# facebookresearch/PartDistillation

Measured on AMD Instinct MI355X. Metric: images/sec training step, R50 Mask2Former 1024² bs=2/GPU, 1/2/4/8 MI355X, higher is better.
Workload: dtype bf16

## Files before the change

### include/pd_gemm.h

```cpp
#ifndef PD_GEMM_H
#define PD_GEMM_H

#include <stdint.h>

#ifdef __cplusplus
extern "C" {
#endif

int pd_gemm_tn_f32(const float *A, const float *B, const float *bias, float *C, int M, int N, int K, int lda, int ldb,
                   int ldc, int relu, void *stream);

int pd_gemm_tn_f32x3(const float *A, const float *B, const float *bias, float *C, int M, int N, int K, int lda, int ldb,
                     int ldc, int relu, void *stream);

int pd_gemm_wgrad_f32(const float *dY, const float *X, float *dW, float *dB, int M, int N, int K, int ldy, int ldx,
                      int ldw, void *stream);

int pd_gemm_wgrad_acc_f32(const float *dY, const float *X, float *dW, float *dB, int M, int N, int K, int ldy, int ldx,
                          int ldw, void *stream);

int64_t pd_gemm_tn_f32x3_relu_bits_words(int M, int N);
int pd_split3_bf16(const float *W, int N, int K, int ldw, int transpose, void *planes, void *stream);
int pd_gemm_tn_f32x3_pre(const float *A, const void *Bplanes, const float *bias, float *C, uint32_t *bits, float *colsum, int M, int N, int K,
                         int lda, int ldc, int mode, void *stream);
// ... 16 lines not shown
} PdGemmWgradDesc;
int64_t pd_gemm_wgrad_f32x3_grouped_table_bytes(int max_count);
int64_t pd_gemm_wgrad_f32x3_grouped_ws_floats(const PdGemmWgradDesc *descs, int count);
int pd_gemm_wgrad_f32x3_grouped(const PdGemmWgradDesc *descs, int count, void *table_host_pinned, void *table_device, float *workspace,
                                int64_t workspace_floats, void *stream);

int pd_conv3x3_wgrad_nhwc_f32x3(const float *dY, const float *X, float *dWk, float *dB, float *workspace, int64_t workspace_floats, int B, int H,
                                int W, int Ci, int Co, void *stream);

int pd_conv3x3_nhwc_f32x3(const float *X, const float *Wk, const float *bias, float *Y, int B, int H, int W, int Ci, int Co,
                          void *stream);

int64_t pd_gemm_wgrad_f16x2_ws_floats(int N, int K);
int pd_gemm_wgrad_f16x2_takes_wide_tiles(int N, int K);
int64_t pd_gemm_wgrad_f16x2_grouped_ws_floats(const PdGemmWgradDesc *descs, int count);
int pd_gemm_wgrad_acc_f16x2_ws(const float *dY, const float *X, float *dW, float *dB, const float *y_amax, const float *x_amax,
                               float *workspace, int64_t workspace_floats, int M, int N, int K, int ldy, int ldx, int ldw, void *stream);
int pd_gemm_wgrad_f16x2_grouped(const PdGemmWgradDesc *descs, int count, void *table_host_pinned, void *table_device, float *workspace,
                                int64_t workspace_floats, void *stream);
int pd_conv3x3_wgrad_nhwc_f16x2(const float *dY, const float *X, float *dWk, float *dB, const float *y_amax, const float *x_amax,
                                float *workspace, int64_t workspace_floats, int B, int H, int W, int Ci, int Co, void *stream);
int pd_gemm_tn_f16x2_which(int M, int N, int K, int mode, int has_bits, int has_amax);

int pd_conv3x3_nhwc_f16x2(const float *X, const float *Wk, const float *bias, float *Y, const float *x_amax, const float *w_amax, float *y_amax,
                          int B, int H, int W, int Ci, int Co, void *stream);
int64_t pd_gemm_tn_f16x2_bits_words(int M, int N);
int pd_gemm_tn_f16x2(const float *A, const float *B, const float *bias, float *C, uint32_t *bits, float *colsum, const float *a_amax,
                     const float *b_amax, float *c_amax, int M, int N, int K, int lda, int ldb, int ldc, int mode, void *stream);
int pd_row_amax_f32(const float *X, int rows, int cols, int ld, float *out, void *stream);
int pd_gemm_tn_f16x2_bf16out(const float *A, const float *B, const float *bias, void *C_bf16, const float *a_amax, const float *b_amax, int M, int N,
                             int K, int lda, int ldb, int ldc, void *stream);
int pd_cast_bf16_f32_amax(const void *X_bf16, int rows, int cols, float *Y, float *row_amax, void *stream);

#ifdef __cplusplus
}
#endif
#endif
```

### partdistillation_amd/csrc/cmdbuf.hip

```cpp
#include <hip/hip_runtime.h>
#include <stdint.h>
#include <string.h>

#include <type_traits>
#include <utility>

#include "pd_common.h"
#include "pd_cmdbuf.h"
#include "pd_attention.h"
#include "pd_conv.h"
#include "pd_declayer.h"
#include "pd_criterion.h"
#include "pd_fused.h"
#include "pd_gemm.h"
#include "pd_grouping.h"
#include "pd_igemm.h"
#include "pd_input.h"
#include "pd_kmeans.h"
#include "pd_msda.h"
#include "pd_mx8.h"
#include "pd_optim.h"
#include "pd_poly.h"
#include "pd_rowwise.h"
#include "pd_smallgemm.h"
// ... 30 lines not shown
#define PD_E(f) {#f, &Thunk<&f>::call, Thunk<&f>::nargs}
const Entry kTable[] = {
  PD_E(pd_adamw_clipped),
  PD_E(pd_adamw_clipped_shadow),
  PD_E(pd_add_layernorm_bwd),
  PD_E(pd_add_layernorm_bwd_amax),
  PD_E(pd_add_layernorm_fwd),
  PD_E(pd_add_layernorm_fwd_amax),
  PD_E(pd_add_rows_amax_f32),
  PD_E(pd_affine_act_bwd2_bf16),
  PD_E(pd_affine_act_bwd_bf16),
  PD_E(pd_affine_act_fwd_bf16),
  PD_E(pd_attn_bwd_d32),
  PD_E(pd_attn_fwd_d32),
  PD_E(pd_attn_mask_u8),
  PD_E(pd_cast_bf16_f32_amax),
  PD_E(pd_colsum_acc),
  PD_E(pd_conv3x3_nhwc_f16x2),
  PD_E(pd_conv3x3_nhwc_f32x3),
  PD_E(pd_conv3x3_wgrad_nhwc_f16x2),
  PD_E(pd_conv3x3_wgrad_nhwc_f32x3),
  PD_E(pd_conv_bf16_dgrad),
  PD_E(pd_conv_bf16_fwd),
  PD_E(pd_conv_bf16_wgrad),
  PD_E(pd_conv_bf16_wgrad_grouped),
  PD_E(pd_dec_bwd_a),
  PD_E(pd_dec_bwd_b),
  PD_E(pd_dec_fwd_a),
  PD_E(pd_dec_fwd_b),
  PD_E(pd_dec_pack_grouped),
  PD_E(pd_decoder_head_bf16),
  PD_E(pd_filter_transpose_grouped),
  PD_E(pd_gemm_tn_f16x2),
  PD_E(pd_gemm_tn_f16x2_bf16out),
  PD_E(pd_gemm_tn_f32),
  PD_E(pd_gemm_tn_f32x3),
  PD_E(pd_gemm_tn_f32x3_pre),
  PD_E(pd_gemm_tn_f32x3_relu_bits),
  PD_E(pd_gemm_tn_f32x3_relumask),
  PD_E(pd_gemm_wgrad_acc_f16x2_ws),
  PD_E(pd_gemm_wgrad_acc_f32),
  PD_E(pd_gemm_wgrad_acc_f32x3),
  PD_E(pd_gemm_wgrad_acc_f32x3_ws),
  PD_E(pd_gemm_wgrad_f16x2_grouped),
  PD_E(pd_gemm_wgrad_f32),
  PD_E(pd_gemm_wgrad_f32x3_grouped),
  PD_E(pd_gn_coeffs_bwd),
  PD_E(pd_gn_coeffs_fwd),
  PD_E(pd_igemm_bf16),
  PD_E(pd_igemm_bf16_seq),
  PD_E(pd_kmeans_assign),
  PD_E(pd_kmeans_assign_bounded),
  PD_E(pd_kmeans_assign_partial),
  PD_E(pd_kmeans_reduce),
  PD_E(pd_kmeans_reduce_update),
  PD_E(pd_kmeans_reduce_update_shift),
  PD_E(pd_kmeans_update),
  PD_E(pd_layernorm_rows_f32_bwd),
  PD_E(pd_layernorm_rows_f32_fwd),
  PD_E(pd_loss_vectors_bwd),
  PD_E(pd_loss_vectors_fwd),
  PD_E(pd_lsa_batched),
  PD_E(pd_mask_assign),
  PD_E(pd_mask_point_losses_bwd),
  PD_E(pd_mask_point_losses_fwd),
  PD_E(pd_matcher_costs),
  PD_E(pd_copy_segments),
// ... 16 lines not shown
  PD_E(pd_msda_forward_amax),
  PD_E(pd_msda_fused_backward),
  PD_E(pd_msda_fused_forward),
  PD_E(pd_msda_prep_bwd),
  PD_E(pd_msda_prep_bwd_amax),
  PD_E(pd_msda_prep_fwd),
  PD_E(pd_multi_gather_sumsq),
  PD_E(pd_mx8_gemm),
  PD_E(pd_mx8_quantize_bf16),
  PD_E(pd_mx8_quantize_grouped),
  PD_E(pd_nc_affine2_amax_f32),
  PD_E(pd_nc_affine2_f32),
  PD_E(pd_nc_affine_amax_f32),
  PD_E(pd_nc_affine_f32),
  PD_E(pd_nc_sums_f32),
  PD_E(pd_normalize_u8_nhwc),
  PD_E(pd_pair_logits_bwd_rows),
  PD_E(pd_pair_logits_bwd_tok),
  PD_E(pd_pair_logits_fwd),
  PD_E(pd_point_sample_nhwc_f32),
  PD_E(pd_point_sample_nhwc_f32_bf16),
  PD_E(pd_point_sample_planar_bwd_f32),
  PD_E(pd_point_sample_planar_f32),
  PD_E(pd_point_sample_u8),
  PD_E(pd_poly_crossings_i32),
  PD_E(pd_relu_bwd_colsum),
  PD_E(pd_resample_cols_canvas_u8),
  PD_E(pd_resample_cols_u8),
  PD_E(pd_resample_rows_u8),
  PD_E(pd_resize_bilinear_nhwc_f32),
  PD_E(pd_rle_sample_groups_canvas_u8),
  PD_E(pd_rle_sample_groups_u8),
  PD_E(pd_rle_sample_u8),
  PD_E(pd_row_amax_f32),
  PD_E(pd_scores_argmax_u8),
  PD_E(pd_sgemm_nn_bf16),
  PD_E(pd_sgemm_nn_splitn_bf16),
  PD_E(pd_sgemm_tn_batched_bf16),
  PD_E(pd_sgemm_tn_bf16),
  PD_E(pd_sgemm_tn_multi_bf16),
  PD_E(pd_sgemm_tn_splitk_bf16),
  PD_E(pd_sgemm_wgrad_bf16),
  PD_E(pd_sgemm_wgrad_grouped_bf16),
  PD_E(pd_sgemm_wgrad_split_bf16),
  PD_E(pd_skinny_linear_bwd),
  PD_E(pd_skinny_linear_fwd),
  PD_E(pd_split3_bf16),
  PD_E(pd_stem7x7_fwd),
  PD_E(pd_stem7x7_wgrad),
  PD_E(pd_sum3_sum2_f32),
  PD_E(pd_sumsq_accumulate),
  PD_E(pd_swin_ln_bwd),
  PD_E(pd_swin_ln_fwd),
  PD_E(pd_transpose_batched_f32),
  PD_E(pd_uncertain_points),
  PD_E(pd_upsample2x_bwd_nhwc_f32),
  PD_E(pd_upsample_add_amax_nhwc_f32),
  PD_E(pd_upsample_add_nhwc_f32),
  PD_E(pd_wgrad_bf16),
  PD_E(pd_wgrad_bf16_seq),
  PD_E(pd_window_attn_bwd_w12),
  PD_E(pd_window_attn_fwd_w12),
};
constexpr int kCount = (int)(sizeof(kTable) / sizeof(kTable[0]));
}

extern "C" int pd_memset_async(void *dst, int value, int64_t bytes, void *stream)
// ... 42 lines not shown
```

### partdistillation_amd/csrc/common.hip

```cpp
#include <hip/hip_runtime.h>
#include <stdarg.h>
#include <stdio.h>
#include <string.h>

#include "pd_common.h"
#include "pd_msda.h"

namespace {
thread_local char g_err[512] = {0};
}

int pd_set_error(int code, const char *fmt, ...)
{
  va_list ap;
  va_start(ap, fmt);
  vsnprintf(g_err, sizeof(g_err), fmt, ap);
  va_end(ap);
  return code;
}

int pd_check_launch(const char *what)
{
  hipError_t e = hipGetLastError();
  if (e == hipSuccess) return PD_OK;
  return pd_set_error(PD_ERR_LAUNCH, "%s: %s", what, hipGetErrorString(e));
}

extern "C" const char *pd_last_error(void) { return g_err; }
extern "C" int pd_abi_version(void) { return 47; }

extern int g_pd_dbg_atomic_scope;
extern int g_pd_dbg_force_generic;
extern int g_pd_dbg_ablate;
extern int g_pd_dbg_x3_narrow;
extern int g_pd_dbg_f16x2;
extern int g_pd_dbg_wgrad_wide;
extern "C" void pd_dbg_set_wgrad_xcd(int v);
extern "C" void pd_dbg_set_wgrad_fast(int v);
extern int g_pd_dbg_bwd_variant;
extern int g_pd_dbg_msda_gate_pct;
extern int g_pd_dbg_wgrad_wgs;
extern int g_pd_dbg_bwd_threads;
extern int g_pd_dbg_attn_scalar;
extern int g_pd_dbg_wattn;
extern int g_pd_dbg_x3;
extern int g_pd_dbg_kmeans;
extern int g_pd_dbg_conv_group_rows;
extern int g_pd_dbg_conv_xcd_major;
extern int g_pd_dbg_sgemm_deep;
extern int g_ig_bn, g_ig_nst, g_ig_splits, g_ig_patch, g_ig_pcls;
extern int g_mx_bn, g_mx_nst;
extern int g_swin_ln_abl;
extern int g_ln_bwd_cap;
extern int g_crit_abl;
extern int g_attn_bwd_kc;
extern int g_wg_nst, g_wg_splits, g_wg_mode;
extern "C" int pd_debug_set(const char *key, int value)
{
  if (!key) return PD_ERR_INVALID_ARG;
  if (!strcmp(key, "msda_bwd_atomic_scope")) { g_pd_dbg_atomic_scope = value; return PD_OK; }
  if (!strcmp(key, "msda_ablate")) { g_pd_dbg_ablate = value; return PD_OK; }
  if (!strcmp(key, "msda_bwd_variant")) { g_pd_dbg_bwd_variant = value; return PD_OK; }
// ... 33 lines not shown
```

### partdistillation_amd/csrc/f16x2.h

```cpp
#ifndef PD_F16X2_H
#define PD_F16X2_H
#include <hip/hip_runtime.h>
#include <stdint.h>

namespace pdh2 {
typedef float f32x16 __attribute__((ext_vector_type(16)));
typedef float f32x2 __attribute__((ext_vector_type(2)));
typedef _Float16 h16x2 __attribute__((ext_vector_type(2)));
typedef _Float16 h16x8 __attribute__((ext_vector_type(8)));
typedef unsigned short h16_t;
__device__ __forceinline__ void row_scale(float amax, float &s, float &inv)
{
  int e = (int)((__float_as_uint(amax) >> 23) & 0xffu);
  e = e < 20 ? 20 : (e > 250 ? 250 : e);
  s = __uint_as_float((unsigned)(268 - e) << 23);
  inv = __uint_as_float((unsigned)(e - 14) << 23);
}

struct SplitH { uint2 hi, lo; };
__device__ __forceinline__ void split2h(float x0, float x1, unsigned &h, unsigned &l)
{
  const f32x2 x = {x0, x1};
  const h16x2 hh = __builtin_convertvector(x, h16x2);
  const f32x2 r = {x0 - (float)hh[0], x1 - (float)hh[1]};
  const h16x2 ll = __builtin_convertvector(r, h16x2);
  h = __builtin_bit_cast(unsigned, hh);
  l = __builtin_bit_cast(unsigned, ll);
}
__device__ __forceinline__ SplitH split4h_p(float4 v, float s)
{
  SplitH o;
  split2h(v.x * s, v.y * s, o.hi.x, o.lo.x);
  split2h(v.z * s, v.w * s, o.hi.y, o.lo.y);
  return o;
}
__device__ __forceinline__ float np_mul(float a, float b) { float r; asm("v_mul_f32 %0, %1, %2" : "=v"(r) : "v"(a), "v"(b)); return r; }
__device__ __forceinline__ float np_sub(float a, float b) { float r; asm("v_sub_f32 %0, %1, %2" : "=v"(r) : "v"(a), "v"(b)); return r; }
__device__ __forceinline__ void split2h_u(float x0, float x1, unsigned &h, unsigned &l)
{
  const f32x2 x = {x0, x1};
  const h16x2 hh = __builtin_convertvector(x, h16x2);
  const f32x2 r = {np_sub(x0, (float)hh[0]), np_sub(x1, (float)hh[1])};
  const h16x2 ll = __builtin_convertvector(r, h16x2);
  h = __builtin_bit_cast(unsigned, hh);
  l = __builtin_bit_cast(unsigned, ll);
}
__device__ __forceinline__ SplitH split4h_u(float4 v, float s)
{
  SplitH o;
  split2h_u(np_mul(v.x, s), np_mul(v.y, s), o.hi.x, o.lo.x);
  split2h_u(np_mul(v.z, s), np_mul(v.w, s), o.hi.y, o.lo.y);
  return o;
}
__device__ __forceinline__ SplitH split4h(float4 v, float s)
{
#ifdef PD_F16X2_UNPACKED_SPLIT
  return split4h_u(v, s);
#else
  return split4h_p(v, s);
#endif
}
__device__ __forceinline__ void mmah(f32x16 &c, h16x8 x, h16x8 y) { c = __builtin_amdgcn_mfma_f32_32x32x16_f16(x, y, c, 0, 0, 0); }

}
#endif
```

### partdistillation_amd/csrc/gemm_f16x2.hip

```cpp
#include <hip/hip_runtime.h>
#include <stdint.h>
#include <stdlib.h>
#include <type_traits>

#include "f16x2.h"
#include "pd_common.h"
#include "xcd.h"
#include "pd_gemm.h"
#include "pd_msda.h"

#ifndef PD_ABL
#define PD_ABL 0
#endif

namespace {
using namespace pdh2;
__device__ __forceinline__ int xcd_chunk(int bid, int nb) { return pd_xcd_chunk(bid, nb); }
__device__ __forceinline__ unsigned short f2bf_rne(float f)
{
  unsigned u = __float_as_uint(f);
  if ((u & 0x7fffffffu) > 0x7f800000u) return (unsigned short)((u >> 16) | 0x40u);
  u += 0x7fffu + ((u >> 16) & 1u);
  return (unsigned short)(u >> 16);
}

template <int TM, int TN, int WN, int BKK, int MODE, bool CONV = false, int NRS = 1, int FAST = 0>
__global__ __launch_bounds__((TM / 64) * (TN / WN) * 64, (TM == 256 ? 1 : 2))
void gemm_tn_f16x2(const float *__restrict__ A, const float *__restrict__ B, const float *__restrict__ bias, float *__restrict__ C,
                   int M, int N, int K, int lda, int ldb, int ldc, int ntiles_n, uint32_t *__restrict__ bits,
                   float *__restrict__ colsum, const float *__restrict__ a_amax, const float *__restrict__ b_amax,
                   unsigned *__restrict__ c_amax, int H, int W, int tap_minor)
{
  constexpr int WVN = TN / WN, NW = (TM / 64) * WVN, NTH = NW * 64, NJ = WN / 32;
  constexpr int TPR = BKK / 4, RPP = NTH / TPR, APASS = TM / RPP, BPASS = TN / RPP, NPAN = BKK / 8;
  static_assert(TM % RPP == 0 && TN % RPP == 0, "staging passes");
  constexpr int ASZ = 2 * NPAN * TM * 8, BSZ = 2 * NPAN * TN * 8;
  extern __shared__ __attribute__((aligned(16))) float sc[];
  h16_t *smem = reinterpret_cast<h16_t *>(sc + 2 * (TM + TN));
  auto As = [&](int buf, int pl, int pan, int r) -> h16_t * { return smem + buf * (ASZ + BSZ) + (((pl * NPAN + pan) * TM + r) << 3); };
  auto Bs = [&](int buf, int pl, int pan, int r) -> h16_t * { return smem + buf * (ASZ + BSZ) + ASZ + (((pl * NPAN + pan) * TN + r) << 3); };
  const int lb = xcd_chunk(blockIdx.x, gridDim.x);
  const int m0 = (lb / ntiles_n) * TM, n0 = (lb % ntiles_n) * TN;
  const int t = threadIdx.x, lane = t & 63, wave = t >> 6;
  const int wm = (wave / WVN) * 64, wn = (wave % WVN) * WN;
  const int lr = t / TPR, lk = (t % TPR) * 4;
  for (int r = t; r < TM + TN; r += NTH) {
    const bool isa = r < TM;
    const int g = isa ? m0 + r : n0 + r - TM;
    const float *am = isa ? a_amax : b_amax;
    float s = 1.f, inv = 1.f;
    if (!(PD_ABL & 32) && am && g < (isa ? M : N)) {
      float mx = am[g];
      if (CONV && isa) {
        const int pix = g % (H * W), y = pix / W, x = pix - y * W;
#pragma unroll
        for (int dy = -1; dy <= 1; ++dy)
#pragma unroll
          for (int dx = -1; dx <= 1; ++dx)
            if (y + dy >= 0 && y + dy < H && x + dx >= 0 && x + dx < W) mx = fmaxf(mx, am[g + dy * W + dx]);
      }
      row_scale(mx, s, inv);
    }
    sc[r] = s; sc[TM + TN + r] = inv;
  }
  __syncthreads();
  float sa[APASS], sb[BPASS];
#pragma unroll
  for (int j = 0; j < APASS; ++j) sa[j] = sc[lr + RPP * j];
#pragma unroll
  for (int j = 0; j < BPASS; ++j) sb[j] = sc[TM + lr + RPP * j];
  float4 ra[NRS][APASS], rb[NRS][BPASS];
  int py[APASS], px[APASS];
  if (CONV) {
#pragma unroll
    for (int j = 0; j < APASS; ++j) {
      const int pix = (m0 + lr + RPP * j) % (H * W);
      py[j] = pix / W;
      px[j] = pix - py[j] * W;
    }
  }
  auto gload = [&](int rs, int k0) {
    if (PD_ABL & 8) {
#pragma unroll
      for (int j = 0; j < APASS; ++j) ra[rs][j] = make_float4(1.f, 0.5f, 0.25f, (float)k0);
#pragma unroll
      for (int j = 0; j < BPASS; ++j) rb[rs][j] = make_float4(1.f, 0.5f, 0.25f, (float)k0);
      return;
    }
    const int k = k0 + lk;
    int dy = 0, dx = 0, kc = k, kb = k;
    if (CONV) {
      int tap;
      if (tap_minor) { const int s = k0 / BKK; const int cb = s / 9; tap = s - cb * 9; kc = cb * BKK + lk; kb = tap * lda + kc; }
      else { tap = k / lda; kc = k - tap * lda; }
      dy = tap / 3 - 1; dx = tap - (tap / 3) * 3 - 1;
    }
#pragma unroll
    for (int j = 0; j < APASS; ++j) {
      const int r = lr + RPP * j;
      if (CONV) {
        const int yy = py[j] + dy, xx = px[j] + dx;
        const bool ok = m0 + r < M && k < K && yy >= 0 && yy < H && xx >= 0 && xx < W;
        ra[rs][j] = ok ? *reinterpret_cast<const float4 *>(A + ((int64_t)(m0 + r) + dy * W + dx) * lda + kc) : make_float4(0, 0, 0, 0);
      } else {
        ra[rs][j] = (m0 + r < M && k < K) ? *reinterpret_cast<const float4 *>(A + (int64_t)(m0 + r) * lda + k) : make_float4(0, 0, 0, 0);
      }
    }
#pragma unroll
    for (int j = 0; j < BPASS; ++j) {
      const int r = lr + RPP * j;
      rb[rs][j] = (n0 + r < N && k < K) ? *reinterpret_cast<const float4 *>(B + (int64_t)(n0 + r) * ldb + kb) : make_float4(0, 0, 0, 0);
    }
  };
  auto lstore = [&](int rs, int buf) {
    if (PD_ABL & 4) {
#pragma unroll
      for (int j = 0; j < APASS; ++j) asm volatile("" ::"v"(ra[rs][j].x), "v"(ra[rs][j].y), "v"(ra[rs][j].z), "v"(ra[rs][j].w));
#pragma unroll
      for (int j = 0; j < BPASS; ++j) asm volatile("" ::"v"(rb[rs][j].x), "v"(rb[rs][j].y), "v"(rb[rs][j].z), "v"(rb[rs][j].w));
      return;
    }
#pragma unroll
    for (int j = 0; j < APASS; ++j) {
      const SplitH x = split4h(ra[rs][j], sa[j]);
      h16_t *p = As(buf, 0, lk >> 3, lr + RPP * j) + (lk & 7);
      *reinterpret_cast<uint2 *>(p) = x.hi; *reinterpret_cast<uint2 *>(p + NPAN * TM * 8) = x.lo;
    }
#pragma unroll
    for (int j = 0; j < BPASS; ++j) {
      const SplitH x = split4h(rb[rs][j], sb[j]);
      h16_t *p = Bs(buf, 0, lk >> 3, lr + RPP * j) + (lk & 7);
      *reinterpret_cast<uint2 *>(p) = x.hi; *reinterpret_cast<uint2 *>(p + NPAN * TN * 8) = x.lo;
    }
  };
  f32x16 acc[2][NJ];
#pragma unroll
  for (int i = 0; i < 2; ++i)
#pragma unroll
    for (int j = 0; j < NJ; ++j)
#pragma unroll
      for (int e = 0; e < 16; ++e) acc[i][j][e] = 0.f;
  const int KT = (K + BKK - 1) / BKK;
  gload(0, 0);
  lstore(0, 0);
  if (KT > 1) gload(NRS == 2 ? 1 : 0, BKK);
  if (NRS == 2 && KT > 2) gload(0, 2 * BKK);
  __syncthreads();
  const int fr = lane & 31, fh = lane >> 5;
  auto step = [&](int kt, int par) {
    if (kt + 1 < KT) {
      const int rs = NRS == 2 ? (par ^ 1) : 0;
      lstore(rs, par ^ 1);
      if (kt + 1 + NRS < KT) gload(rs, (kt + 1 + NRS) * BKK);
    }
#pragma unroll
    for (int ks = 0; ks < ((PD_ABL & 2) ? 0 : BKK / 16); ++ks) {
      h16x8 a[2][2];
#pragma unroll
      for (int pl = 0; pl < 2; ++pl)
#pragma unroll
        for (int i = 0; i < 2; ++i) a[pl][i] = *reinterpret_cast<const h16x8 *>(As(par, pl, 2 * ks + fh, wm + i * 32 + fr));
#pragma unroll
      for (int jp = 0; jp < NJ / 2; ++jp) {
        h16x8 b[2][2];
#pragma unroll
        for (int pl = 0; pl < 2; ++pl)
#pragma unroll
          for (int j = 0; j < 2; ++j) b[pl][j] = *reinterpret_cast<const h16x8 *>(Bs(par, pl, 2 * ks + fh, wn + (jp * 2 + j) * 32 + fr));
#if PD_ABL & 1
#define HTERM(PA, PB)                                                        \
  _Pragma("unroll") for (int i = 0; i < 2; ++i)                              \
      _Pragma("unroll") for (int j = 0; j < 2; ++j) asm volatile("" ::"v"(a[PA][i]), "v"(b[PB][j]));
#else
#define HTERM(PA, PB)                                                        \
  _Pragma("unroll") for (int i = 0; i < 2; ++i)                              \
      _Pragma("unroll") for (int j = 0; j < 2; ++j) mmah(acc[i][jp * 2 + j], a[PA][i], b[PB][j]);
#endif
        HTERM(1, 0)
        HTERM(0, 1)
        HTERM(0, 0)
#undef HTERM
      }
    }
    __syncthreads();
  };
  int kt0 = 0;
  if constexpr (FAST != 0 && BKK == 16) {
    if (m0 + TM <= M && n0 + TN <= N && (K % (2 * BKK)) == 0 && KT >= 4 && (!CONV || tap_minor)) {
      const float *pa[APASS], *pb[BPASS];
#pragma unroll
      for (int j = 0; j < APASS; ++j) pa[j] = A + (int64_t)(m0 + lr + RPP * j) * lda + lk;
#pragma unroll
      for (int j = 0; j < BPASS; ++j) pb[j] = B + (int64_t)(n0 + lr + RPP * j) * ldb + lk;
      auto fstep = [&](int kt, int par) {
        const int rs = NRS == 2 ? (par ^ 1) : 0;
        int kn = min((kt + 1 + NRS) * BKK, K - BKK), knb = kn, dy = 0, dx = 0;
        if (CONV) {
          const int sidx = kn / BKK, cb = sidx / 9, tap = sidx - cb * 9;
          dy = tap / 3 - 1; dx = tap - (tap / 3) * 3 - 1;
          kn = cb * BKK; knb = tap * lda + kn;
        }
        h16x8 a[2][2], b[2][NJ];
#pragma unroll
        for (int pl = 0; pl < 2; ++pl) {
#pragma unroll
          for (int i = 0; i < 2; ++i) a[pl][i] = *reinterpret_cast<const h16x8 *>(As(par, pl, fh, wm + i * 32 + fr));
#pragma unroll
          for (int j = 0; j < NJ; ++j) b[pl][j] = *reinterpret_cast<const h16x8 *>(Bs(par, pl, fh, wn + j * 32 + fr));
        }
#pragma unroll
        for (int j = 0; j < APASS; ++j) {
          const SplitH x = split4h(ra[rs][j], sa[j]);
          h16_t *p = As(par ^ 1, 0, lk >> 3, lr + RPP * j) + (lk & 7);
          *reinterpret_cast<uint2 *>(p) = x.hi; *reinterpret_cast<uint2 *>(p + NPAN * TM * 8) = x.lo;
          if (CONV) {
            const int yy = py[j] + dy, xx = px[j] + dx;
            const bool ok = yy >= 0 && yy < H && xx >= 0 && xx < W;
            const float4 v = *reinterpret_cast<const float4 *>(pa[j] + (ok ? (dy * W + dx) * lda : 0) + kn);
            ra[rs][j] = make_float4(ok ? v.x : 0.f, ok ? v.y : 0.f, ok ? v.z : 0.f, ok ? v.w : 0.f);
          } else {
            ra[rs][j] = *reinterpret_cast<const float4 *>(pa[j] + kn);
          }
        }
#pragma unroll
        for (int j = 0; j < BPASS; ++j) {
          const SplitH x = split4h(rb[rs][j], sb[j]);
          h16_t *p = Bs(par ^ 1, 0, lk >> 3, lr + RPP * j) + (lk & 7);
          *reinterpret_cast<uint2 *>(p) = x.hi; *reinterpret_cast<uint2 *>(p + NPAN * TN * 8) = x.lo;
          rb[rs][j] = *reinterpret_cast<const float4 *>(pb[j] + knb);
        }
#define FTERM(PA, PB)                                                        \
  _Pragma("unroll") for (int i = 0; i < 2; ++i)                              \
      _Pragma("unroll") for (int j = 0; j < NJ; ++j) mmah(acc[i][j], a[PA][i], b[PB][j]);
        FTERM(1, 0)
        FTERM(0, 1)
        FTERM(0, 0)
#undef FTERM
        if constexpr (FAST == 1) {
          constexpr int NM = 6 * NJ, NV = (12 * (APASS + BPASS) + 8 + NM - 1) / NM, EV = NM / (APASS + BPASS);
          __builtin_amdgcn_sched_group_barrier(0x100, 4 + 2 * NJ, 0);
#pragma unroll
          for (int g = 0; g < NM; ++g) {
            __builtin_amdgcn_sched_group_barrier(0x008, 1, 0);
            __builtin_amdgcn_sched_group_barrier(0x002, NV, 0);
            if (g % EV == EV - 1) {
              __builtin_amdgcn_sched_group_barrier(0x200, 1, 0);
              __builtin_amdgcn_sched_group_barrier(0x020, 1, 0);
            }
          }
        }
        __syncthreads();
      };
      for (; kt0 + 2 < KT; kt0 += 2) {
        fstep(kt0, 0);
        fstep(kt0 + 1, 1);
      }
    }
  }
  for (int kt = kt0; kt < KT; kt += 2) {
    step(kt, 0);
    if (kt + 1 < KT) step(kt + 1, 1);
  }
  float bv[NJ], ib[NJ], csum[NJ];
  uint32_t word[NJ];
  int64_t widx[NJ];
#pragma unroll
  for (int j = 0; j < NJ; ++j) {
    const int col = n0 + wn + j * 32 + (lane & 31);
    bv[j] = (bias && col < N) ? bias[col] : 0.f;
    ib[j] = sc[2 * TM + TN + wn + j * 32 + (lane & 31)];
    widx[j] = (((int64_t)lb * NW + wave) * 64 + lane) * NJ + j;
    word[j] = MODE == 2 ? bits[widx[j]] : 0u;
    csum[j] = 0.f;
// ... 23 lines not shown
          }
          if (PD_ABL & 16) { asm volatile("" ::"v"(v)); rm = fmaxf(rm, fabsf(v)); }
          else if (ok) {
            if (!CONV && (H & 1)) reinterpret_cast<unsigned short *>(C)[(int64_t)row * ldc + col] = f2bf_rne(v);
            else C[(int64_t)row * ldc + col] = v;
            rm = fmaxf(rm, fabsf(v));
          }
        }
        if (c_amax) red[rl * 33 + (lane & 31)] = rm;
      }
  };
  if (full) store_tile(std::false_type{});
  else store_tile(std::true_type{});
#pragma unroll
  for (int j = 0; j < NJ; ++j) {
    const int col = n0 + wn + j * 32 + (lane & 31);
    if (MODE == 1 && bits && col < N) bits[widx[j]] = word[j];
    if (MODE == 2) {
      float cs = csum[j];
      cs += __shfl_xor(cs, 32, 64);
      if (lane < 32 && cs != 0.f && col < N) unsafeAtomicAdd(colsum + col, cs);
    }
  }
  if (c_amax) {
    __builtin_amdgcn_wave_barrier();
    float v = 0.f;
#pragma unroll
    for (int c = 0; c < 32; ++c) v = fmaxf(v, red[lane * 33 + c]);
    const int row = m0 + wm + lane;
    if (row < M && v > 0.f) atomicMax(c_amax + row, __float_as_uint(v));
  }
}

__global__ __launch_bounds__(256) void row_amax_f32(const float *__restrict__ X, int rows, int cols, int ld, float *__restrict__ out)
{
  const int row = blockIdx.x * 4 + (threadIdx.x >> 6), lane = threadIdx.x & 63;
  if (row >= rows) return;
  const float *p = X + (int64_t)row * ld;
  float v = 0.f;
  if (!(cols & 3) && !(ld & 3) && !((uintptr_t)X & 15)) {
    for (int c = lane * 4; c < cols; c += 256) {
      const float4 x = *reinterpret_cast<const float4 *>(p + c);
      v = fmaxf(fmaxf(v, fmaxf(fabsf(x.x), fabsf(x.y))), fmaxf(fabsf(x.z), fabsf(x.w)));
    }
  } else {
    for (int c = lane; c < cols; c += 64) v = fmaxf(v, fabsf(p[c]));
  }
#pragma unroll
  for (int o = 32; o; o >>= 1) v = fmaxf(v, __shfl_xor(v, o, 64));
  if (lane == 0) out[row] = v;
}


__global__ __launch_bounds__(256) void cast_bf16_f32_amax(const unsigned short *__restrict__ X, int rows, int cols, float *__restrict__ Y,
                                                          float *__restrict__ out)
{
  const int row = blockIdx.x * 4 + (threadIdx.x >> 6), lane = threadIdx.x & 63;
  if (row >= rows) return;
  const unsigned short *p = X + (int64_t)row * cols;
  float *q = Y + (int64_t)row * cols;
  float v = 0.f;
  for (int c = lane * 8; c < cols; c += 512) {
    const uint4 u = *reinterpret_cast<const uint4 *>(p + c);
    float f[8];
    f[0] = __uint_as_float(u.x << 16); f[1] = __uint_as_float(u.x & 0xffff0000u); f[2] = __uint_as_float(u.y << 16); f[3] = __uint_as_float(u.y & 0xffff0000u);
    f[4] = __uint_as_float(u.z << 16); f[5] = __uint_as_float(u.z & 0xffff0000u); f[6] = __uint_as_float(u.w << 16); f[7] = __uint_as_float(u.w & 0xffff0000u);
#pragma unroll
    for (int k = 0; k < 8; ++k) v = fmaxf(v, fabsf(f[k]));
    *reinterpret_cast<float4 *>(q + c) = make_float4(f[0], f[1], f[2], f[3]);
    *reinterpret_cast<float4 *>(q + c + 4) = make_float4(f[4], f[5], f[6], f[7]);
  }
#pragma unroll
  for (int o = 32; o; o >>= 1) v = fmaxf(v, __shfl_xor(v, o, 64));
  if (lane == 0) out[row] = v;
}

constexpr int RS_PANEL = 528, RS_PLANE = 32 * RS_PANEL, RS_BUF = 2 * RS_PLANE;
typedef unsigned u32x4 __attribute__((ext_vector_type(4)));

#ifdef PD_ROWS_PACKED_SPLIT
#define ROWS_SPLIT split4h
#else
#define ROWS_SPLIT split4h_u
#endif
__device__ int g_rows_wstage = 1;
template <bool AM, int MODE = 0>
__global__ __launch_bounds__(512)
void gemm_rows_f16x2_k256(const float *__restrict__ A, const float *__restrict__ B, const float *__restrict__ bias, float *__restrict__ C,
                          int M, int npanels, int lda, int ldb, int ldc, const float *__restrict__ a_amax,
                          const float *__restrict__ b_amax, unsigned *__restrict__ c_amax, unsigned short *__restrict__ bits = nullptr,
                          float *__restrict__ colsum = nullptr)
{
  __shared__ __attribute__((aligned(16))) unsigned char lds0[RS_BUF], lds1[RS_BUF];
  __shared__ __attribute__((aligned(16))) float sinv0[32], sinv1[32], sdump[64];
  const int t = threadIdx.x, lane = t & 63, w = __builtin_amdgcn_readfirstlane(t >> 6), fr = lane & 31, fh = lane >> 5;
  const int x = blockIdx.x & 7, q = blockIdx.x >> 3;
  const int panel = q % npanels, rg = (q / npanels) * 8 + x, nrg = (gridDim.x / 8 / npanels) * 8;
  const int ntile = (M + 31) >> 5;
  const int t0 = (int)((int64_t)rg * ntile / nrg), t1 = (int)((int64_t)(rg + 1) * ntile / nrg), T = t1 - t0;
  if (T <= 0) return;
  const int n0 = panel * 256 + w * 32;

  float4 R[2][4];
  float am[2][4];
  auto gload = [&](int rs, int tile) {
    tile = min(tile, t1 - 1);
#pragma unroll
    for (int j = 0; j < 4; ++j) {
      const int row = min(tile * 32 + w + 8 * j, M - 1);
      if (PD_ABL & 8) R[rs][j] = make_float4(1.f, 0.5f, 0.25f, (float)row);
      else R[rs][j] = *reinterpret_cast<const float4 *>(A + (int64_t)row * lda + 4 * lane);
      am[rs][j] = AM ? a_amax[row] : 0.f;
    }
  };
  auto split_store = [&](int rs, int buf) {
    float invs[4];
#pragma unroll
    for (int j = 0; j < 4; ++j) {
      float s = 1.f;
      invs[j] = 1.f;
      if (AM) row_scale(am[rs][j], s, invs[j]);
      const SplitH v = ROWS_SPLIT(R[rs][j], s);
      unsigned char *p = (buf ? lds1 : lds0) + (lane >> 1) * RS_PANEL + (w + 8 * j) * 16 + (lane & 1) * 8;
      if (PD_ABL & 4) { asm volatile("" ::"v"(R[rs][j].x), "v"(R[rs][j].y), "v"(R[rs][j].z), "v"(R[rs][j].w)); continue; }
      *reinterpret_cast<uint2 *>(p) = v.hi;
      *reinterpret_cast<uint2 *>(p + RS_PLANE) = v.lo;
    }
    const unsigned l0 = -(unsigned)(lane == 0), l1 = -(unsigned)(lane == 1), l2 = -(unsigned)(lane == 2);
    const unsigned iv = (__float_as_uint(invs[0]) & l0) | (__float_as_uint(invs[1]) & l1) | (__float_as_uint(invs[2]) & l2) |
                        (__float_as_uint(invs[3]) & ~(l0 | l1 | l2));
    *reinterpret_cast<unsigned *>(lane < 4 ? (buf ? sinv1 : sinv0) + w + 8 * lane : sdump + lane) = iv;
  };
  gload(0, t0);
  gload(1, t0 + 1);
  h16x8 bh[16], bl[16];
  float ibv = 1.f;
  {
    float sbv = 1.f;
    if (AM) row_scale(b_amax[n0 + fr], sbv, ibv);
    if (g_rows_wstage) {
      constexpr int WP = 66;
      float *wl = reinterpret_cast<float *>(w < 4 ? lds0 : lds1) + (w & 3) * (32 * WP);
      const float *bsrc = B + (int64_t)(n0 + (lane >> 4)) * ldb + 4 * (lane & 15);
      float *wdst = wl + (lane >> 4) * WP + 4 * (lane & 15);
      const float *wsrc = wl + fr * WP + 8 * fh;
      float4 wa[8], wb[8];
#pragma unroll
      for (int i = 0; i < 8; ++i) wa[i] = *reinterpret_cast<const float4 *>(bsrc + (int64_t)(4 * i) * ldb);
#define PD_WPASS(R, CUR, NXT)                                                                                                  \
      {                                                                                                                        \
        if (R < 3) {                                                                                                           \
          _Pragma("unroll") for (int i = 0; i < 8; ++i) NXT[i] = *reinterpret_cast<const float4 *>(bsrc + (int64_t)(4 * i) * ldb + 64 * (R + 1)); \
        }                                                                                                                      \
        _Pragma("unroll") for (int i = 0; i < 8; ++i) {                                                                        \
          *reinterpret_cast<float2 *>(wdst + 4 * i * WP) = make_float2(CUR[i].x, CUR[i].y);                                    \
          *reinterpret_cast<float2 *>(wdst + 4 * i * WP + 2) = make_float2(CUR[i].z, CUR[i].w);                                \
// ... 8 lines not shown
        }                                                                                                                      \
        asm volatile("s_waitcnt lgkmcnt(0)" ::: "memory");        \
      }
      PD_WPASS(0, wa, wb) PD_WPASS(1, wb, wa) PD_WPASS(2, wa, wb) PD_WPASS(3, wb, wa)
#undef PD_WPASS
      __syncthreads();
    } else {
      const float *bp = B + (int64_t)(n0 + fr) * ldb + 8 * fh;
#pragma unroll
      for (int s = 0; s < 16; ++s) {
        const SplitH u = split4h((PD_ABL & 64) ? make_float4(1.f, 2.f, (float)s, sbv) : *reinterpret_cast<const float4 *>(bp + 16 * s), sbv),
                     v = split4h((PD_ABL & 64) ? make_float4(1.f, 2.f, (float)s, ibv) : *reinterpret_cast<const float4 *>(bp + 16 * s + 4), sbv);
        bh[s] = __builtin_bit_cast(h16x8, u32x4{u.hi.x, u.hi.y, v.hi.x, v.hi.y});
        bl[s] = __builtin_bit_cast(h16x8, u32x4{u.lo.x, u.lo.y, v.lo.x, v.lo.y});
      }
    }
  }
  const float bv = bias ? bias[n0 + fr] : 0.f;
  float csum = 0.f;
  split_store(0, 0);
  gload(0, t0 + 2);
  __syncthreads();

  auto iter = [&](int it, int par) {
    const unsigned char *base = (par ? lds1 : lds0) + fh * RS_PANEL + fr * 16;
    unsigned wbits = 0u;
    if (MODE == 2) wbits = (unsigned)bits[(((int64_t)(t0 + it) * npanels + panel) * 8 + w) * 64 + lane];
    f32x16 acc0, acc1;
#pragma unroll
    for (int e = 0; e < 16; ++e) { acc0[e] = 0.f; acc1[e] = 0.f; }
#pragma unroll
    for (int s = 0; s < ((PD_ABL & 1) ? 0 : 16); ++s) {
      const h16x8 ah = (PD_ABL & 2) ? bl[15 - s] : *reinterpret_cast<const h16x8 *>(base + 2 * s * RS_PANEL);
      const h16x8 al = (PD_ABL & 2) ? bh[15 - s] : *reinterpret_cast<const h16x8 *>(base + 2 * s * RS_PANEL + RS_PLANE);
#ifdef PD_ROWS_TWO_CHAINS
      if (s & 1) { mmah(acc1, al, bh[s]); mmah(acc0, ah, bl[s]); mmah(acc1, ah, bh[s]); }
      else       { mmah(acc0, al, bh[s]); mmah(acc1, ah, bl[s]); mmah(acc0, ah, bh[s]); }
#else
      mmah(acc0, al, bh[s]); mmah(acc0, ah, bl[s]); mmah(acc0, ah, bh[s]);
#endif
    }
    split_store(par ^ 1, par ^ 1);
    gload(par ^ 1, t0 + it + 3);
#pragma unroll
    for (int s = 0; s < 16; ++s) {
      __builtin_amdgcn_sched_group_barrier(0x008, 1, 0);
      __builtin_amdgcn_sched_group_barrier(0x002, 2, 0);
      __builtin_amdgcn_sched_group_barrier(0x008, 1, 0);
      __builtin_amdgcn_sched_group_barrier(0x002, 2, 0);
      __builtin_amdgcn_sched_group_barrier(0x008, 1, 0);
      __builtin_amdgcn_sched_group_barrier(0x002, 2, 0);
      if (s & 1) __builtin_amdgcn_sched_group_barrier(0x200, 1, 0);
      if ((s & 3) == 3) __builtin_amdgcn_sched_group_barrier(0x020, 1, 0);
    }
    __builtin_amdgcn_sched_barrier(0);
    const int row0 = (t0 + it) * 32;
    float o[16];
#pragma unroll
    for (int qd = 0; qd < 4; ++qd) {
      const float4 ia = *reinterpret_cast<const float4 *>((par ? sinv1 : sinv0) + 8 * qd + 4 * fh);
      o[4 * qd + 0] = (acc0[4 * qd + 0] + acc1[4 * qd + 0]) * (ia.x * ibv) + bv;
      o[4 * qd + 1] = (acc0[4 * qd + 1] + acc1[4 * qd + 1]) * (ia.y * ibv) + bv;
      o[4 * qd + 2] = (acc0[4 * qd + 2] + acc1[4 * qd + 2]) * (ia.z * ibv) + bv;
      o[4 * qd + 3] = (acc0[4 * qd + 3] + acc1[4 * qd + 3]) * (ia.w * ibv) + bv;
    }
    if (MODE != 0) {
      const int64_t widx = (((int64_t)(t0 + it) * npanels + panel) * 8 + w) * 64 + lane;
      unsigned word = 0u;
      if (MODE == 2) { asm volatile("" : "+v"(wbits)); word = wbits; }
#pragma unroll
      for (int e = 0; e < 16; ++e) {
        const int rl = (e & 3) + 8 * (e >> 2) + 4 * fh;
        if (MODE == 1) {
          o[e] = fmaxf(o[e], 0.f);
          word |= (o[e] > 0.f ? 1u : 0u) << e;
        } else {
          o[e] = ((word >> e) & 1u) ? o[e] : 0.f;
          if (row0 + rl < M) csum += o[e];
        }
      }
      if (MODE == 1 && bits) bits[widx] = (unsigned short)word;
    }
    float *cp = C + (int64_t)row0 * ldc + n0 + fr;
    if (PD_ABL & 16) {
// ... 33 lines not shown
    if (it + 1 < T) iter(it + 1, 1);
  }
  if (MODE == 2) {
    csum += __shfl_xor(csum, 32, 64);
    if (lane < 32 && csum != 0.f) unsafeAtomicAdd(colsum + n0 + fr, csum);
  }
}


constexpr int KR_RB = 192, KR_KC = 32;
constexpr int KR_APANEL = KR_RB * 16 + 16, KR_APLANE = (KR_KC / 8) * KR_APANEL, KR_ABUF = 2 * KR_APLANE;
constexpr int KR_BPANEL = 256 * 16 + 16, KR_BPLANE = (KR_KC / 8) * KR_BPANEL, KR_BBUF = 2 * KR_BPLANE;
#ifdef PD_PROBES
constexpr size_t KR_LDS = (size_t)2 * (KR_ABUF + KR_BBUF) + KR_RB * sizeof(float);
#endif

constexpr size_t KP_LDS = (size_t)2 * (KR_ABUF + KR_BBUF) + 2 * KR_RB * sizeof(float) + 4 * sizeof(int);

#ifdef PD_PROBES
#include "../../tools/probes/gemm_f16x2_optin.h"
#endif
__device__ unsigned long long g_kp_trace[2][64][8];
__device__ __forceinline__ void kp_stamp(int role, int chunk, int ev)
{
  if (chunk < 64) g_kp_trace[role][chunk][ev] = __builtin_readcyclecounter();
}

__device__ __forceinline__ void kp_wait_ge(int *p, int target)
{
  while (__hip_atomic_load(p, __ATOMIC_RELAXED, __HIP_MEMORY_SCOPE_WORKGROUP) < target) __builtin_amdgcn_s_sleep(1);
  asm volatile("" ::: "memory");
}

template <bool AM, int KABL = 0, bool BP = false, bool CONV = false>
__global__ __launch_bounds__(768)
void gemm_kpc_f16x2(const float *__restrict__ A, const float *__restrict__ B, const float *__restrict__ bias, float *__restrict__ C, int M, int K,
                    int lda, int ldb, int ldc, int npanels, const float *__restrict__ a_amax, const float *__restrict__ b_amax, int H = 0, int W = 0)
{
  auto conv_amax = [&](int row) -> float {
    float mx = a_amax[row];
    const int pix = row % (H * W), y = pix / W, x = pix - y * W;
#pragma unroll
    for (int dy = -1; dy <= 1; ++dy)
#pragma unroll
      for (int dx = -1; dx <= 1; ++dx)
        if (y + dy >= 0 && y + dy < H && x + dx >= 0 && x + dx < W) mx = fmaxf(mx, a_amax[row + dy * W + dx]);
    return mx;
  };
  extern __shared__ __attribute__((aligned(16))) unsigned char kp_lds[];
  unsigned char *const aimg = kp_lds, *const bimg = kp_lds + 2 * KR_ABUF;
  float *sinv = reinterpret_cast<float *>(kp_lds + 2 * (KR_ABUF + KR_BBUF));
  int *ctr = reinterpret_cast<int *>(sinv + 2 * KR_RB);
  const int t = threadIdx.x, lane = t & 63, w = __builtin_amdgcn_readfirstlane(t >> 6);
  const int nblk = (M + KR_RB - 1) / KR_RB, NC = K / KR_KC;
  if (t < 4) ctr[t] = 0;
  __syncthreads();
  if (w >= 8) {
    const int pt = t - 512, prow = pt >> 3, pc4 = pt & 7;
    int g0 = 0, seq = 0;
    for (int work = blockIdx.x; work < nblk * npanels; work += gridDim.x, g0 += NC, ++seq) {
      const int blk = work / npanels, panel = work - blk * npanels, row0 = blk * KR_RB, c0 = panel * 256;
      if (pt < KR_RB) {
        float sc = 1.f, inv = 1.f;
        if (AM) row_scale(CONV ? conv_amax(min(row0 + pt, M - 1)) : a_amax[min(row0 + pt, M - 1)], sc, inv);
        sinv[(seq & 1) * KR_RB + pt] = inv;
      }
      float sa[6], sb[8];
#pragma unroll
      for (int j = 0; j < 6; ++j) {
        float inv;
        sa[j] = 1.f;
        if (AM) row_scale(CONV ? conv_amax(min(row0 + prow + 32 * j, M - 1)) : a_amax[min(row0 + prow + 32 * j, M - 1)], sa[j], inv);
      }
#pragma unroll
      for (int j = 0; j < 8; ++j) {
        float inv;
        sb[j] = 1.f;
        if (AM) row_scale(b_amax[c0 + prow + 32 * j], sb[j], inv);
      }
      const __amdgpu_buffer_rsrc_t ra = __builtin_amdgcn_make_buffer_rsrc(const_cast<float *>(A), 0, (int)((int64_t)M * lda * 4), 0x00020000);
      const int64_t bbytes = BP ? (int64_t)2 * npanels * 256 * K * 2 : (int64_t)(c0 + 256) * ldb * 4;
      const __amdgpu_buffer_rsrc_t rbs = __builtin_amdgcn_make_buffer_rsrc(const_cast<float *>(B), 0, (int)bbytes, 0x00020000);
      unsigned oa[6], ob[8];
      unsigned pyx[6];
#pragma unroll
      for (int j = 0; j < 6; ++j) {
        const int row = row0 + prow + 32 * j;
        oa[j] = ((unsigned)row * (unsigned)lda + 4u * pc4) * 4u;
        pyx[j] = 0u;
        if (CONV && row < M) {
          const int pix = row % (H * W), y = pix / W, x = pix - y * W;
#pragma unroll
          for (int t9 = 0; t9 < 9; ++t9) {
            const int dy = t9 / 3 - 1, dx = t9 % 3 - 1;
            pyx[j] |= (unsigned)(y + dy >= 0 && y + dy < H && x + dx >= 0 && x + dx < W) << t9;
          }
        }
      }
#pragma unroll
      for (int j = 0; j < 8; ++j) {
        if (BP) {
          const int q = pt + 256 * (j & 3), h = j >> 2, plane = q >> 9, col = 128 * h + ((q & 511) >> 2), pan = q & 3;
          ob[j] = (unsigned)(((int64_t)plane * npanels * 256 + c0 + col) * K + 8 * pan) * 2u;
        } else {
          ob[j] = ((unsigned)(c0 + prow + 32 * j) * (unsigned)ldb + 4u * pc4) * 4u;
        }
      }
      float4 RA[3][3], RB[3][4];
      auto gload = [&](int rs, int u) {
        const int kcl = min(u >> 1, NC - 1), ko = kcl * (KR_KC * 4), h = u & 1;
        int tap = 0, shift = 0;
        if (CONV) {
          const int lcb = __builtin_ctz((unsigned)(lda / KR_KC));
          tap = kcl >> lcb;
          const int cb = kcl - (tap << lcb), t3 = (tap >= 3) + (tap >= 6), dy = t3 - 1, dx = tap - 3 * t3 - 1;
          shift = ((dy * W + dx) * lda + cb * KR_KC) * 4;
        }
#pragma unroll
        for (int j = 0; j < 3; ++j) {
          unsigned off = h ? oa[3 + j] : oa[j];
          if (CONV) off = (((h ? pyx[3 + j] : pyx[j]) >> tap) & 1u) ? off + (unsigned)shift : 0x80000000u;
          const u32x4 v = __builtin_amdgcn_raw_buffer_load_b128(ra, off, CONV ? 0 : ko, 0);
          RA[rs][j] = make_float4(__uint_as_float(v.x), __uint_as_float(v.y), __uint_as_float(v.z), __uint_as_float(v.w));
        }
#pragma unroll
        for (int j = 0; j < 4; ++j) {
          const u32x4 v = __builtin_amdgcn_raw_buffer_load_b128(rbs, h ? ob[4 + j] : ob[j], BP ? ko / 2 : ko, 0);
          RB[rs][j] = make_float4(__uint_as_float(v.x), __uint_as_float(v.y), __uint_as_float(v.z), __uint_as_float(v.w));
        }
      };
      auto split_store = [&](int rs, int buf, int h) {
        unsigned char *ab = aimg + buf * KR_ABUF + (pc4 >> 1) * KR_APANEL + (pc4 & 1) * 8;
        unsigned char *bb = bimg + buf * KR_BBUF + (pc4 >> 1) * KR_BPANEL + (pc4 & 1) * 8;
#pragma unroll
        for (int j = 0; j < 3; ++j) {
          const SplitH v = split4h_u(RA[rs][j], h ? sa[3 + j] : sa[j]);
          unsigned char *p = ab + (prow + 32 * (3 * h + j)) * 16;
          *reinterpret_cast<uint2 *>(p) = v.hi;
          *reinterpret_cast<uint2 *>(p + KR_APLANE) = v.lo;
        }
#pragma unroll
        for (int j = 0; j < 4; ++j) {
          if (BP) {
            const int q = pt + 256 * j, plane = q >> 9, col = 128 * h + ((q & 511) >> 2), pan = q & 3;
            *reinterpret_cast<float4 *>(bimg + buf * KR_BBUF + plane * KR_BPLANE + pan * KR_BPANEL + col * 16) = RB[rs][j];
          } else {
            const SplitH v = split4h_u(RB[rs][j], h ? sb[4 + j] : sb[j]);
            unsigned char *p = bb + (prow + 32 * (4 * h + j)) * 16;
            *reinterpret_cast<uint2 *>(p) = v.hi;
            *reinterpret_cast<uint2 *>(p + KR_BPLANE) = v.lo;
          }
        }
      };
      gload(0, 0);
      gload(1, 1);
      gload(2, 2);
      const int NH = 2 * NC;
      for (int u0 = 0; u0 < NH; u0 += 6) {
#pragma unroll
        for (int k6 = 0; k6 < 6; ++k6) {
          const int u = u0 + k6;
          if (u >= NH) break;
          const int cc = u >> 1, gc = g0 + cc, par = gc & 1, h = k6 & 1, rs = k6 % 3;
          const bool tr = (KABL & 16) && blockIdx.x == 0 && w == 8 && lane == 0 && seq == 0;
          if (h == 0) {
            if (tr) kp_stamp(1, cc, 0);
            kp_wait_ge(ctr + 2 + par, 8 * (gc >> 1));
            if (tr) kp_stamp(1, cc, 1);
          }
          if (KABL & 16) { asm volatile("s_waitcnt vmcnt(14)" ::: "memory"); if (tr) kp_stamp(1, cc, 2 + 2 * h); }
// ... 15 lines not shown
#pragma unroll
    for (int cb = 0; cb < 2; ++cb) {
      float sc = 1.f;
      if (AM) row_scale(b_amax[n0 + 32 * cb + fr], sc, ibv[cb]);
    }
    f32x16 acc[3][2];
#pragma unroll
    for (int ti = 0; ti < 3; ++ti)
#pragma unroll
      for (int cb = 0; cb < 2; ++cb)
#pragma unroll
        for (int e = 0; e < 16; ++e) acc[ti][cb][e] = 0.f;
    for (int c = 0; c < NC; c += 2) {
#pragma unroll
      for (int par0 = 0; par0 < 2; ++par0) {
        const int cc = c + par0, gc = g0 + cc, par = gc & 1;
        if (cc >= NC) break;
        const bool tr = (KABL & 16) && blockIdx.x == 0 && w == 0 && lane == 0 && seq == 0;
        if (tr) kp_stamp(0, cc, 0);
        kp_wait_ge(ctr + par, 4 * ((gc >> 1) + 1));
        if (tr) kp_stamp(0, cc, 1);
        const unsigned char *ab = aimg + par * KR_ABUF + fh * KR_APANEL + (96 * rgp + fr) * 16;
        const unsigned char *bb = bimg + par * KR_BBUF + fh * KR_BPANEL + (64 * cg + fr) * 16;
#pragma unroll
        for (int s = 0; s < KR_KC / 16; ++s) {
          h16x8 ah[3], al[3], bh[2], bl[2];
#pragma unroll
          for (int ti = 0; ti < 3; ++ti) {
            if (KABL & 4) {
              ah[ti] = __builtin_bit_cast(h16x8, u32x4{(unsigned)s, (unsigned)ti, 1u, (unsigned)cc});
              al[ti] = ah[ti];
            } else {
              ah[ti] = *reinterpret_cast<const h16x8 *>(ab + 2 * s * KR_APANEL + ti * 32 * 16);
              al[ti] = *reinterpret_cast<const h16x8 *>(ab + 2 * s * KR_APANEL + ti * 32 * 16 + KR_APLANE);
            }
          }
#pragma unroll
          for (int cb = 0; cb < 2; ++cb) {
            if (KABL & 4) {
              bh[cb] = __builtin_bit_cast(h16x8, u32x4{(unsigned)s, (unsigned)cb, 3u, (unsigned)cc});
              bl[cb] = bh[cb];
            } else {
              bh[cb] = *reinterpret_cast<const h16x8 *>(bb + 2 * s * KR_BPANEL + cb * 32 * 16);
              bl[cb] = *reinterpret_cast<const h16x8 *>(bb + 2 * s * KR_BPANEL + cb * 32 * 16 + KR_BPLANE);
            }
          }
          if (KABL & 2) {
#pragma unroll
            for (int ti = 0; ti < 3; ++ti)
#pragma unroll
              for (int cb = 0; cb < 2; ++cb) acc[ti][cb][0] += (float)ah[ti][0] * (float)bl[cb][1] + (float)al[ti][2] * (float)bh[cb][3];
            continue;
          }
          if (KABL & 16) { asm volatile("s_waitcnt lgkmcnt(0)" ::: "memory"); if (tr) kp_stamp(0, cc, 3 + s); }
#pragma unroll
          for (int ti = 0; ti < 3; ++ti)
#pragma unroll
            for (int cb = 0; cb < 2; ++cb) mmah(acc[ti][cb], al[ti], bh[cb]);
#pragma unroll
          for (int ti = 0; ti < 3; ++ti)
#pragma unroll
            for (int cb = 0; cb < 2; ++cb) mmah(acc[ti][cb], ah[ti], bl[cb]);
#pragma unroll
          for (int ti = 0; ti < 3; ++ti)
#pragma unroll
            for (int cb = 0; cb < 2; ++cb) mmah(acc[ti][cb], ah[ti], bh[cb]);
        }
        if (tr) kp_stamp(0, cc, 2);
        if (lane == 0) __hip_atomic_fetch_add(ctr + 2 + par, 1, __ATOMIC_RELEASE, __HIP_MEMORY_SCOPE_WORKGROUP);
      }
    }
#pragma unroll
    for (int ti = 0; ti < 3; ++ti) {
      const int rl0 = 96 * rgp + 32 * ti;
#pragma unroll
      for (int cb = 0; cb < 2; ++cb) {
        const int col = n0 + 32 * cb + fr;
        const float bv = bias ? bias[col] : 0.f;
        float *cp = C + (int64_t)(row0 + rl0) * ldc + col;
#pragma unroll
        for (int e = 0; e < 16; ++e) {
          const int rl = (e & 3) + 8 * (e >> 2) + 4 * fh;
          if (row0 + rl0 + rl < M) cp[(int64_t)rl * ldc] = acc[ti][cb][e] * (sinv_it[rl0 + rl] * ibv[cb]) + bv;
        }
      }
    }
  }
}
}

static const bool g_rows_relu = []() { const char *e = getenv("PD_H2_ROWS_RELU"); return !e || e[0] != '0'; }();
// ... 234 lines not shown
{
  const int dbg = g_pd_dbg_f16x2;
  static const bool rows_k256 = []() { const char *e = getenv("PD_H2_ROWS_K256"); return !e || e[0] != '0'; }();
  if ((dbg == 61 || (rows_k256 && dbg == 0)) && mode == 0 && K == 256 && (N % 256) == 0 && M >= 8192) return 2;
#ifdef PD_PROBES
  if ((dbg == 90 || (dbg >= 100 && dbg < 132)) && mode == 0 && K == 256 && M >= 4096 && (N % 32) == 0 && N >= 96 && ((N % 128) == 0 || (N % 96) == 0)) return 3;
#endif
  if (dbg != 62 && dbg != 3 && dbg != 13 && dbg != 70 && (mode == 1 || mode == 2) && has_bits && K == 256 && (N % 256) == 0 && N >= 512 && M >= 8192 && has_amax && g_rows_relu) return 2;
  static const bool kpc_env = []() { const char *e = getenv("PD_H2_KPC"); return !e || e[0] != '0'; }();
  if (((kpc_env && dbg == 0) || dbg == 92 || dbg == 93) && mode == 0 && !has_bits && K >= 512 && (K % KR_KC) == 0 && (N % 256) == 0 && N <= 512 && M >= 8192 && kpc_items_ok(M, N)) return 5;
#ifdef PD_PROBES
  static const bool kres_env = []() { const char *e = getenv("PD_H2_KRES"); return e && e[0] == '1'; }();
  if (((kres_env && dbg == 0) || dbg == 91) && mode == 0 && !has_bits && K >= 512 && (K % KR_KC) == 0 && (N % 256) == 0 && N <= 512 && M >= 8192) return 4;
#endif
  const bool wide_ok = (N % 256) == 0 && M >= 1024;
  const bool by_shape = dbg == 0 || dbg == 61 || dbg == 70 || dbg == 80 || dbg == 62;
  static const bool wide_deepk = []() { const char *e = getenv("PD_H2_WIDE_DEEPK"); return e && e[0] == '1'; }();
  const bool wide = has_bits || dbg == 3 || dbg == 13 || (by_shape && wide_ok && (int64_t)((M + 255) / 256) * (N / 256) >= 128 && (N >= 1024 || (K >= 512 && wide_deepk)));
  return wide ? 1 : 0;
}

extern "C" int pd_gemm_tn_f16x2(const float *A, const float *B, const float *bias, float *C, uint32_t *bits, float *colsum, const float *a_amax,
                                const float *b_amax, float *c_amax, int M, int N, int K, int lda, int ldb, int ldc, int mode, void *stream_)
{
  return gemm_tn_f16x2_impl(A, B, bias, C, bits, colsum, a_amax, b_amax, c_amax, M, N, K, lda, ldb, ldc, mode, stream_, 0);
}

extern "C" int pd_gemm_tn_f16x2_bf16out(const float *A, const float *B, const float *bias, void *C_bf16, const float *a_amax, const float *b_amax,
                                        int M, int N, int K, int lda, int ldb, int ldc, void *stream_)
{
  return gemm_tn_f16x2_impl(A, B, bias, reinterpret_cast<float *>(C_bf16), nullptr, nullptr, a_amax, b_amax, nullptr, M, N, K, lda, ldb, ldc, 0, stream_, 1);
}

extern "C" int pd_cast_bf16_f32_amax(const void *X_bf16, int rows, int cols, float *Y, float *row_amax, void *stream_)
{
  if (rows < 0 || cols <= 0 || (cols & 7)) return pd_set_error(PD_ERR_INVALID_ARG, "pd_cast_bf16_f32_amax: rows=%d cols=%d (a multiple of 8)", rows, cols);
  if (rows == 0) return PD_OK;
  if (!X_bf16 || !Y || !row_amax || ((uintptr_t)X_bf16 & 15) || ((uintptr_t)Y & 15)) return pd_set_error(PD_ERR_INVALID_ARG, "pd_cast_bf16_f32_amax: null / misaligned pointer");
  hipLaunchKernelGGL(cast_bf16_f32_amax, dim3((unsigned)((rows + 3) / 4)), dim3(256), 0, (hipStream_t)stream_, (const unsigned short *)X_bf16, rows, cols, Y,
                     row_amax);
  return pd_check_launch("pd_cast_bf16_f32_amax");
}

extern "C" int pd_conv3x3_nhwc_f16x2(const float *X, const float *Wk, const float *bias, float *Y, const float *x_amax, const float *w_amax,
                                     float *y_amax, int B, int H, int W, int Ci, int Co, void *stream_)
{
  if (B < 0 || H <= 0 || W <= 0 || Ci <= 0 || Co <= 0 || (Ci & 15))
    return pd_set_error(PD_ERR_INVALID_ARG, "pd_conv3x3_nhwc_f16x2: B=%d H=%d W=%d Ci=%d (%% 16) Co=%d", B, H, W, Ci, Co);
  if (B == 0) return PD_OK;
  if (!X || !Wk || !Y || ((uintptr_t)X & 15) || ((uintptr_t)Wk & 15)) return pd_set_error(PD_ERR_INVALID_ARG, "pd_conv3x3_nhwc_f16x2: null / misaligned pointer");
  const int64_t M = (int64_t)B * H * W;
  if (M > 0x7fffffffLL - 4096) return pd_set_error(PD_ERR_INVALID_ARG, "pd_conv3x3_nhwc_f16x2: too many pixels");
  hipStream_t st = (hipStream_t)stream_;
#ifdef PD_PROBES
  static const bool kpc_conv = []() { const char *e = getenv("PD_H2_KPC_CONV"); return e && e[0] == '1'; }();
  if (((kpc_conv && g_pd_dbg_f16x2 == 0) || g_pd_dbg_f16x2 == 92 || g_pd_dbg_f16x2 == 234) && x_amax && w_amax && !y_amax && (Co % 256) == 0 && (Ci % KR_KC) == 0 && ((Ci / KR_KC) & (Ci / KR_KC - 1)) == 0 && M >= 8192 &&
      H < 65536 && W < 65536 && M * Ci * 4 < (1ll << 31) && (int64_t)Co * 9 * Ci * 4 < (1ll << 31)) {
    static int ncu5 = 0;
    if (!ncu5) { int dev = 0; (void)hipGetDevice(&dev); if (hipDeviceGetAttribute(&ncu5, hipDeviceAttributeMultiprocessorCount, dev) != hipSuccess || ncu5 < 8) ncu5 = 256; }
    const int np = Co / 256, nwork = (int)((M + KR_RB - 1) / KR_RB) * np, G = nwork < ncu5 ? nwork : ncu5;
    static bool cattr = false;
    if (!cattr) {
      (void)hipFuncSetAttribute((const void *)(gemm_kpc_f16x2<true, 0, false, true>), hipFuncAttributeMaxDynamicSharedMemorySize, (int)KP_LDS);
      cattr = true;
    }
    if (g_pd_dbg_f16x2 == 234) {
      (void)hipFuncSetAttribute((const void *)(gemm_kpc_f16x2<true, 16, false, true>), hipFuncAttributeMaxDynamicSharedMemorySize, (int)KP_LDS);
      hipLaunchKernelGGL((gemm_kpc_f16x2<true, 16, false, true>), dim3((unsigned)G), dim3(768), KP_LDS, st, X, Wk, bias, Y, (int)M, 9 * Ci, Ci, 9 * Ci, Co, np, x_amax,
                         w_amax, H, W);
      return pd_check_launch("pd_conv3x3_nhwc_f16x2 (producer / consumer wavefronts, stamps)");
    }
    hipLaunchKernelGGL((gemm_kpc_f16x2<true, 0, false, true>), dim3((unsigned)G), dim3(768), KP_LDS, st, X, Wk, bias, Y, (int)M, 9 * Ci, Ci, 9 * Ci, Co, np, x_amax,
                       w_amax, H, W);
    return pd_check_launch("pd_conv3x3_nhwc_f16x2 (producer / consumer wavefronts)");
  }
#endif
  const bool wide = g_pd_dbg_f16x2 == 3 || (g_pd_dbg_f16x2 != 4 && (Co % 256) == 0 && M >= 65536);
  if (g_pd_dbg_f16x2 == 70 || g_pd_dbg_f16x2 == 21) {
    if (wide) return launch_f16x2<256, 256, 128, 16, true>(X, Wk, bias, Y, (int)M, Co, 9 * Ci, Ci, 9 * Ci, Co, 0, nullptr, nullptr, x_amax, w_amax, y_amax, st, H, W);
    return launch_f16x2<128, 128, 64, 16, true>(X, Wk, bias, Y, (int)M, Co, 9 * Ci, Ci, 9 * Ci, Co, 0, nullptr, nullptr, x_amax, w_amax, y_amax, st, H, W);
  }
  if (wide) return launch_f16x2<256, 256, 128, 16, true, 1, 1>(X, Wk, bias, Y, (int)M, Co, 9 * Ci, Ci, 9 * Ci, Co, 0, nullptr, nullptr, x_amax, w_amax, y_amax, st, H, W);
  return launch_f16x2<128, 128, 64, 16, true, 1, 1>(X, Wk, bias, Y, (int)M, Co, 9 * Ci, Ci, 9 * Ci, Co, 0, nullptr, nullptr, x_amax, w_amax, y_amax, st, H, W);
}

extern "C" int pd_row_amax_f32(const float *X, int rows, int cols, int ld, float *out, void *stream_)
{
  if (rows < 0 || cols < 0) return pd_set_error(PD_ERR_INVALID_ARG, "pd_row_amax_f32: negative size");
  if (rows == 0) return PD_OK;
  if (!X || !out) return pd_set_error(PD_ERR_INVALID_ARG, "pd_row_amax_f32: null pointer");
  hipLaunchKernelGGL(row_amax_f32, dim3((unsigned)((rows + 3) / 4)), dim3(256), 0, (hipStream_t)stream_, X, rows, cols, ld, out);
  return pd_check_launch("pd_row_amax_f32");
}

extern "C" int pd_debug_read_kpc_trace(unsigned long long *dst)
{
  return hipMemcpyFromSymbol(dst, HIP_SYMBOL(g_kp_trace), sizeof(unsigned long long) * 2 * 64 * 8) == hipSuccess ? PD_OK : PD_ERR_LAUNCH;
}
```

### partdistillation_amd/csrc/gemm_x3.hip

```cpp
#include <hip/hip_runtime.h>
#include <stdint.h>
#include <type_traits>

#include "f16x2.h"
#include "mfma_bf16.h"
#include "pd_common.h"
#include "xcd.h"
#include "pd_gemm.h"
#include "pd_msda.h"

namespace {
using namespace pdmfma;

constexpr int BM = 128, BN = 128, BK = 16, PITCH = BK + 4;

struct Split4 { uint2 hi, mid, lo; };

__device__ __forceinline__ void split2(float x0, float x1, unsigned &h, unsigned &m, unsigned &l)
{
  h = pk_bf16(x0, x1);
  const float r0 = x0 - bf_lo(h), r1 = x1 - bf_hi(h);
  m = pk_bf16(r0, r1);
  l = pk_bf16(r0 - bf_lo(m), r1 - bf_hi(m));
}
// ... 382 lines not shown
    if (st + 2 < steps) gload(par, mb + (st + 2) * WS);
    __syncthreads();
  };
  for (int st = 0; st < steps; st += 2) {
    step(st, 0);
    if (st + 1 < steps) step(st + 1, 1);
  }
  if (do_bias && ycol_ok) unsafeAtomicAdd(dB + n0 + col, bsum);
#pragma unroll
  for (int j = 0; j < 2; ++j) {
    const int c = k0 + wk + j * 32 + (lane & 31);
    if (c >= K) continue;
#pragma unroll
    for (int i = 0; i < 2; ++i)
#pragma unroll
      for (int e = 0; e < 16; ++e) {
        const int row = n0 + wn + i * 32 + (e & 3) + 8 * (e >> 2) + 4 * (lane >> 5);
        if (row < N) unsafeAtomicAdd(dW + (int64_t)row * ldw + c, acc[i][j][e]);
      }
  }
}

constexpr int TWS = 16, TP = 160;
typedef short v4s16 __attribute__((ext_vector_type(4)));
__device__ __forceinline__ hwbf16x8 frag_tr(const bf16_t *p)
{
  typedef __attribute__((address_space(3))) v4s16 *lp;
  union { v4s16 h[2]; hwbf16x8 v; } u;
  u.h[0] = __builtin_amdgcn_ds_read_tr16_b64_v4i16((lp)(p));
  u.h[1] = __builtin_amdgcn_ds_read_tr16_b64_v4i16((lp)(p + 4 * TP));
  return u.v;
}

template <int ABL, bool CONV, bool H2 = false>
__device__ __forceinline__ void wgrad_tr_body(const float *__restrict__ dY, const float *__restrict__ X, float *__restrict__ dW,
                                              float *__restrict__ dB, float *__restrict__ ws, int M, int N, int K, int ldy, int ldx,
                                              int ldw, int tiles_k, int tiles, int m_chunk, int H, int W, int bid, int64_t ws_tile0,
                                              const float *__restrict__ y_amax = nullptr, const float *__restrict__ x_amax = nullptr)
{
  constexpr int NP = H2 ? 2 : 3;
  __shared__ __attribute__((aligned(16))) bf16_t S[2][2][NP][TWS][TP];
  const int tile = bid % tiles, split = bid / tiles;
  const int n0 = (tile / tiles_k) * BN, k0 = (tile % tiles_k) * BM;
  const int mb = split * m_chunk, me = min(M, mb + m_chunk);
  const int t = threadIdx.x, lane = t & 63, wave = t >> 6;
  const int wn = (wave >> 1) * 64, wk = (wave & 1) * 64;
  const int sr = t >> 5, sc = (t & 31) * 4;
  const bool ycol_ok = n0 + sc < N, xcol_ok = k0 + sc < K;
  float sy = 1.f, sx = 1.f, inv_yx = 1.f;
  if (H2 && (y_amax || x_amax)) {
    float my = 0.f, mx = 0.f;
    if (y_amax) for (int r = mb + t; r < me; r += 256) my = fmaxf(my, y_amax[r]);
    const int xlo = CONV ? max(0, mb - W - 1) : mb, xhi = CONV ? min(M, me + W + 1) : me;
    if (x_amax) for (int r = xlo + t; r < xhi; r += 256) mx = fmaxf(mx, x_amax[r]);
#pragma unroll
    for (int o = 32; o; o >>= 1) { my = fmaxf(my, __shfl_xor(my, o, 64)); mx = fmaxf(mx, __shfl_xor(mx, o, 64)); }
    float *red = reinterpret_cast<float *>(&S[0][0][0][0][0]);
    if (lane == 0) { red[wave] = my; red[4 + wave] = mx; }
    __syncthreads();
    my = fmaxf(fmaxf(red[0], red[1]), fmaxf(red[2], red[3]));
    mx = fmaxf(fmaxf(red[4], red[5]), fmaxf(red[6], red[7]));
    __syncthreads();
    float iy = 1.f, ix = 1.f;
    if (y_amax) pdh2::row_scale(my, sy, iy);
    if (x_amax) pdh2::row_scale(mx, sx, ix);
    inv_yx = iy * ix;
  }
  float4 ry[2][2], rx[2][2];
  int cpy[2] = {0, 0}, cpx[2] = {0, 0}, tdy = 0, tdx = 0, xoff = k0 + sc;
  if (CONV) {
    const int tap = k0 / ldx;
    tdy = tap / 3 - 1; tdx = tap - (tap / 3) * 3 - 1;
    xoff = k0 - tap * ldx + sc;
#pragma unroll
    for (int j = 0; j < 2; ++j) {
      const int pix = (mb + sr + 8 * j) % (H * W);
      cpy[j] = pix / W; cpx[j] = pix - cpy[j] * W;
    }
  }
  auto gload = [&](int s, int m) {
#pragma unroll
    for (int j = 0; j < 2; ++j) {
      const int r = m + sr + 8 * j;
      ry[s][j] = (r < me && ycol_ok) ? *reinterpret_cast<const float4 *>(dY + (int64_t)r * ldy + n0 + sc) : make_float4(0, 0, 0, 0);
      if (CONV) {
        const int yy = cpy[j] + tdy, xx = cpx[j] + tdx;
        const bool ok = r < me && xcol_ok && yy >= 0 && yy < H && xx >= 0 && xx < W;
        rx[s][j] = ok ? *reinterpret_cast<const float4 *>(X + ((int64_t)r + tdy * W + tdx) * ldx + xoff) : make_float4(0, 0, 0, 0);
        cpx[j] += TWS;
        while (cpx[j] >= W) { cpx[j] -= W; if (++cpy[j] == H) cpy[j] = 0; }
      } else {
        rx[s][j] = (r < me && xcol_ok) ? *reinterpret_cast<const float4 *>(X + (int64_t)r * ldx + k0 + sc) : make_float4(0, 0, 0, 0);
      }
    }
  };
  const bool do_bias = dB != nullptr && k0 == 0;
  float4 bsum = make_float4(0, 0, 0, 0);
  auto lstore = [&](int s, int buf) {
#pragma unroll
    for (int j = 0; j < 2; ++j) {
      const int r = sr + 8 * j;
      if constexpr (H2) {
        const pdh2::SplitH y = pdh2::split4h(ry[s][j], sy), x = pdh2::split4h(rx[s][j], sx);
        *reinterpret_cast<uint2 *>(&S[buf][0][0][r][sc]) = y.hi; *reinterpret_cast<uint2 *>(&S[buf][0][1][r][sc]) = y.lo;
        *reinterpret_cast<uint2 *>(&S[buf][1][0][r][sc]) = x.hi; *reinterpret_cast<uint2 *>(&S[buf][1][1][r][sc]) = x.lo;
      } else {
        const Split4 y = split4(ry[s][j]), x = split4(rx[s][j]);
        *reinterpret_cast<uint2 *>(&S[buf][0][0][r][sc]) = y.hi; *reinterpret_cast<uint2 *>(&S[buf][0][1][r][sc]) = y.mid;
        *reinterpret_cast<uint2 *>(&S[buf][0][NP - 1][r][sc]) = y.lo;
        *reinterpret_cast<uint2 *>(&S[buf][1][0][r][sc]) = x.hi; *reinterpret_cast<uint2 *>(&S[buf][1][1][r][sc]) = x.mid;
        *reinterpret_cast<uint2 *>(&S[buf][1][NP - 1][r][sc]) = x.lo;
      }
      if (do_bias) { bsum.x += ry[s][j].x; bsum.y += ry[s][j].y; bsum.z += ry[s][j].z; bsum.w += ry[s][j].w; }
    }
  };
  f32x16 acc[2][2];
#pragma unroll
  for (int i = 0; i < 2; ++i)
#pragma unroll
    for (int j = 0; j < 2; ++j)
#pragma unroll
      for (int e = 0; e < 16; ++e) acc[i][j][e] = 0.f;
  const int steps = (me - mb + TWS - 1) / TWS;
  if (steps > 0) {
    gload(0, mb);
    if (steps > 1) gload(1, mb + TWS);
    lstore(0, 0);
  }
  __syncthreads();
  const int grp = lane >> 4, sl = lane & 15;
  const int frow = 8 * (grp >> 1) + (sl >> 2), fcol = 16 * (grp & 1) + 4 * (sl & 3);
  auto step = [&](int st, int par) {
    if (st + 2 < steps) gload(par, mb + (st + 2) * TWS);
    hwbf16x8 a[NP][2], b[NP][2];
#pragma unroll
    for (int p = 0; p < NP; ++p)
#pragma unroll
      for (int i = 0; i < 2; ++i) {
        a[p][i] = frag_tr(&S[par][0][p][frow][wn + i * 32 + fcol]);
        b[p][i] = frag_tr(&S[par][1][p][frow][wk + i * 32 + fcol]);
      }
#define TERM(PA, PB)                                                         \
  _Pragma("unroll") for (int i = 0; i < 2; ++i)                              \
      _Pragma("unroll") for (int j = 0; j < 2; ++j) {                        \
        if constexpr (H2) pdh2::mmah(acc[i][j], __builtin_bit_cast(pdh2::h16x8, a[PA][i]), __builtin_bit_cast(pdh2::h16x8, b[PB][j])); \
        else mma16k(acc[i][j], a[PA][i], b[PB][j]);                          \
      }
    if constexpr (H2) { TERM(1, 0) TERM(0, 1) TERM(0, 0) }
    else if (ABL != 2) { TERM(NP - 1, 0) TERM(0, NP - 1) TERM(1, 1) TERM(1, 0) TERM(0, 1) TERM(0, 0) }
    else { _Pragma("unroll") for (int p = 0; p < NP; ++p) _Pragma("unroll") for (int i = 0; i < 2; ++i) { acc[i][0][p] += (float)a[p][i][0]; acc[i][1][p] += (float)b[p][i][0]; } }
#undef TERM
    if (st + 1 < steps) lstore(par ^ 1, par ^ 1);
    __syncthreads();
  };
  for (int st = 0; st < steps; st += 2) {
    step(st, 0);
    if (st + 1 < steps) step(st + 1, 1);
  }
  if (do_bias) {
    float *red = reinterpret_cast<float *>(&S[0][0][0][0][0]);
    *reinterpret_cast<float4 *>(red + sr * BN + sc) = bsum;
    __syncthreads();
    if (t < BN && n0 + t < N) {
      float v = 0.f;
#pragma unroll
      for (int r = 0; r < 8; ++r) v += red[r * BN + t];
      unsafeAtomicAdd(dB + n0 + t, v);
    }
  }
  if (ws) {
    float *w = ws + (ws_tile0 + (int64_t)split * tiles + tile) * (BN * BM) + t;
#pragma unroll
    for (int i = 0; i < 2; ++i)
#pragma unroll
      for (int j = 0; j < 2; ++j)
#pragma unroll
        for (int e = 0; e < 16; ++e) w[((i * 2 + j) * 16 + e) * 256] = H2 ? acc[i][j][e] * inv_yx : acc[i][j][e];
    return;
  }
#pragma unroll
  for (int j = 0; j < 2; ++j) {
    const int c = k0 + wk + j * 32 + (lane & 31);
    if (c >= K) continue;
#pragma unroll
    for (int i = 0; i < 2; ++i)
#pragma unroll
      for (int e = 0; e < 16; ++e) {
        const int row = n0 + wn + i * 32 + (e & 3) + 8 * (e >> 2) + 4 * (lane >> 5);
        if (row < N) unsafeAtomicAdd(dW + (int64_t)row * ldw + c, H2 ? acc[i][j][e] * inv_yx : acc[i][j][e]);
      }
  }
}

template <int ABL, bool CONV, bool H2 = false>
__global__ __launch_bounds__(256, 2) void gemm_wgrad_f32x3_tr(const float *__restrict__ dY, const float *__restrict__ X,
                                                               float *__restrict__ dW, float *__restrict__ dB, float *__restrict__ ws,
                                                               int M, int N, int K, int ldy, int ldx, int ldw, int tiles_k, int tiles,
                                                               int m_chunk, int H, int W, const float *__restrict__ y_amax,
                                                               const float *__restrict__ x_amax)
{
  const int lb = g_wgrad_xcd ? xcd_chunk((int)blockIdx.x, (int)gridDim.x) : (int)blockIdx.x;
  wgrad_tr_body<ABL, CONV, H2>(dY, X, dW, dB, ws, M, N, K, ldy, ldx, ldw, tiles_k, tiles, m_chunk, H, W, lb, 0, y_amax, x_amax);
}

constexpr int WTD = 256, WTP = 288, WNT = 512;
__device__ __forceinline__ hwbf16x8 frag_trw(const bf16_t *p)
{
  typedef __attribute__((address_space(3))) v4s16 *lp;
  union { v4s16 h[2]; hwbf16x8 v; } u;
  u.h[0] = __builtin_amdgcn_ds_read_tr16_b64_v4i16((lp)(p));
  u.h[1] = __builtin_amdgcn_ds_read_tr16_b64_v4i16((lp)(p + 4 * WTP));
  return u.v;
}

template <bool CONV>
__device__ __forceinline__ void wgrad_h2w_body(const float *__restrict__ dY, const float *__restrict__ X, float *__restrict__ dW,
                                               float *__restrict__ dB, float *__restrict__ ws, int M, int N, int K, int ldy, int ldx,
                                               int ldw, int tiles_k, int tiles, int m_chunk, int H, int W, int bid, int64_t ws_tile0,
                                               const float *__restrict__ y_amax, const float *__restrict__ x_amax)
{
  extern __shared__ __attribute__((aligned(16))) bf16_t Sw[];
  auto S = [&](int buf, int op, int pl, int r) -> bf16_t * { return Sw + ((((buf * 2 + op) * 2 + pl) * TWS + r) * WTP); };
  const int tile = bid % tiles, split = bid / tiles;
  const int n0 = (tile / tiles_k) * WTD, k0 = (tile % tiles_k) * WTD;
  const int mb = split * m_chunk, me = min(M, mb + m_chunk);
  const int t = threadIdx.x, lane = t & 63, wave = t >> 6;
  const int wn = (wave >> 1) * 64, wk = (wave & 1) * 128;
  const int sr = t >> 6, sc = (t & 63) * 4;
  const bool ycol_ok = n0 + sc < N, xcol_ok = k0 + sc < K;
  float sy = 1.f, sx = 1.f, inv_yx = 1.f;
  if (y_amax || x_amax) {
    float my = 0.f, mx = 0.f;
    if (y_amax) for (int r = mb + t; r < me; r += WNT) my = fmaxf(my, y_amax[r]);
    const int xlo = CONV ? max(0, mb - W - 1) : mb, xhi = CONV ? min(M, me + W + 1) : me;
    if (x_amax) for (int r = xlo + t; r < xhi; r += WNT) mx = fmaxf(mx, x_amax[r]);
#pragma unroll
    for (int o = 32; o; o >>= 1) { my = fmaxf(my, __shfl_xor(my, o, 64)); mx = fmaxf(mx, __shfl_xor(mx, o, 64)); }
    float *red = reinterpret_cast<float *>(Sw);
    if (lane == 0) { red[wave] = my; red[8 + wave] = mx; }
    __syncthreads();
    my = mx = 0.f;
#pragma unroll
    for (int i = 0; i < 8; ++i) { my = fmaxf(my, red[i]); mx = fmaxf(mx, red[8 + i]); }
    __syncthreads();
    float iy = 1.f, ix = 1.f;
    if (y_amax) pdh2::row_scale(my, sy, iy);
    if (x_amax) pdh2::row_scale(mx, sx, ix);
    inv_yx = iy * ix;
  }
  float4 ry[2][2], rx[2][2];
  int cpy[2] = {0, 0}, cpx[2] = {0, 0}, tdy = 0, tdx = 0, xoff = k0 + sc;
  if (CONV) {
    const int tap = k0 / ldx;
    tdy = tap / 3 - 1; tdx = tap - (tap / 3) * 3 - 1;
    xoff = k0 - tap * ldx + sc;
#pragma unroll
    for (int j = 0; j < 2; ++j) {
      const int pix = (mb + sr + 8 * j) % (H * W);
      cpy[j] = pix / W; cpx[j] = pix - cpy[j] * W;
    }
  }
  auto gload = [&](int s, int m) {
#pragma unroll
    for (int j = 0; j < 2; ++j) {
      const int r = m + sr + 8 * j;
      ry[s][j] = (r < me && ycol_ok) ? *reinterpret_cast<const float4 *>(dY + (int64_t)r * ldy + n0 + sc) : make_float4(0, 0, 0, 0);
      if (CONV) {
        const int yy = cpy[j] + tdy, xx = cpx[j] + tdx;
        const bool ok = r < me && xcol_ok && yy >= 0 && yy < H && xx >= 0 && xx < W;
        rx[s][j] = ok ? *reinterpret_cast<const float4 *>(X + ((int64_t)r + tdy * W + tdx) * ldx + xoff) : make_float4(0, 0, 0, 0);
        cpx[j] += TWS;
        while (cpx[j] >= W) { cpx[j] -= W; if (++cpy[j] == H) cpy[j] = 0; }
      } else {
        rx[s][j] = (r < me && xcol_ok) ? *reinterpret_cast<const float4 *>(X + (int64_t)r * ldx + k0 + sc) : make_float4(0, 0, 0, 0);
      }
    }
  };
  const bool do_bias = dB != nullptr && k0 == 0;
  float4 bsum = make_float4(0, 0, 0, 0);
  auto lstore = [&](int s, int buf) {
#pragma unroll
    for (int j = 0; j < 2; ++j) {
      const int r = sr + 8 * j;
      const pdh2::SplitH y = pdh2::split4h(ry[s][j], sy), x = pdh2::split4h(rx[s][j], sx);
      *reinterpret_cast<uint2 *>(S(buf, 0, 0, r) + sc) = y.hi; *reinterpret_cast<uint2 *>(S(buf, 0, 1, r) + sc) = y.lo;
      *reinterpret_cast<uint2 *>(S(buf, 1, 0, r) + sc) = x.hi; *reinterpret_cast<uint2 *>(S(buf, 1, 1, r) + sc) = x.lo;
      if (do_bias) { bsum.x += ry[s][j].x; bsum.y += ry[s][j].y; bsum.z += ry[s][j].z; bsum.w += ry[s][j].w; }
    }
  };
  f32x16 acc[2][4];
#pragma unroll
  for (int i = 0; i < 2; ++i)
#pragma unroll
    for (int j = 0; j < 4; ++j)
#pragma unroll
      for (int e = 0; e < 16; ++e) acc[i][j][e] = 0.f;
  const int steps = (me - mb + TWS - 1) / TWS;
  if (steps > 0) {
    gload(0, mb);
    if (steps > 1) gload(1, mb + TWS);
    lstore(0, 0);
  }
  __syncthreads();
  const int grp = lane >> 4, sl = lane & 15;
  const int frow = 8 * (grp >> 1) + (sl >> 2), fcol = 16 * (grp & 1) + 4 * (sl & 3);
  auto step = [&](int st, int par) {
    if (st + 2 < steps) gload(par, mb + (st + 2) * TWS);
    hwbf16x8 a[2][2];
#pragma unroll
    for (int p = 0; p < 2; ++p)
#pragma unroll
      for (int i = 0; i < 2; ++i) a[p][i] = frag_trw(S(par, 0, p, frow) + wn + i * 32 + fcol);
#pragma unroll
    for (int jp = 0; jp < 2; ++jp) {
      hwbf16x8 b[2][2];
#pragma unroll
      for (int p = 0; p < 2; ++p)
#pragma unroll
        for (int j = 0; j < 2; ++j) b[p][j] = frag_trw(S(par, 1, p, frow) + wk + (jp * 2 + j) * 32 + fcol);
#define WTERM(PA, PB)                                                        \
  _Pragma("unroll") for (int i = 0; i < 2; ++i)                              \
      _Pragma("unroll") for (int j = 0; j < 2; ++j)                          \
        pdh2::mmah(acc[i][jp * 2 + j], __builtin_bit_cast(pdh2::h16x8, a[PA][i]), __builtin_bit_cast(pdh2::h16x8, b[PB][j]));
      WTERM(1, 0) WTERM(0, 1) WTERM(0, 0)
#undef WTERM
    }
    if (st + 1 < steps) lstore(par ^ 1, par ^ 1);
    __syncthreads();
  };
  int st0 = 0;
  if (g_wgrad_fast && n0 + WTD <= N && k0 + WTD <= K && ((me - mb) % TWS) == 0 && steps >= 4 && (!CONV || W >= TWS)) {
    const float *py0 = dY + (int64_t)(mb + sr) * ldy + n0 + sc, *px0 = X + (int64_t)(mb + sr) * ldx + (CONV ? xoff : k0 + sc);
    auto fstep = [&](int st, int par) {
      const int64_t m = (int64_t)(st + 2) * TWS;
#pragma unroll
      for (int j = 0; j < 2; ++j) {
        ry[par][j] = *reinterpret_cast<const float4 *>(py0 + (m + 8 * j) * ldy);
        if (CONV) {
          const int yy = cpy[j] + tdy, xx = cpx[j] + tdx;
          const bool ok = yy >= 0 && yy < H && xx >= 0 && xx < W;
          const float4 v = *reinterpret_cast<const float4 *>(px0 + (m + 8 * j + (ok ? tdy * W + tdx : 0)) * ldx);
          rx[par][j] = make_float4(ok ? v.x : 0.f, ok ? v.y : 0.f, ok ? v.z : 0.f, ok ? v.w : 0.f);
          cpx[j] += TWS;
          const bool wrap = cpx[j] >= W;
          cpx[j] -= wrap ? W : 0;
          cpy[j] = wrap ? (cpy[j] + 1 == H ? 0 : cpy[j] + 1) : cpy[j];
        } else {
          rx[par][j] = *reinterpret_cast<const float4 *>(px0 + (m + 8 * j) * ldx);
        }
      }
      hwbf16x8 a[2][2], b[2][4];
#pragma unroll
      for (int p = 0; p < 2; ++p) {
#pragma unroll
        for (int i = 0; i < 2; ++i) a[p][i] = frag_trw(S(par, 0, p, frow) + wn + i * 32 + fcol);
#pragma unroll
        for (int j = 0; j < 4; ++j) b[p][j] = frag_trw(S(par, 1, p, frow) + wk + j * 32 + fcol);
      }
#pragma unroll
      for (int j = 0; j < 2; ++j) {
        const int r = sr + 8 * j;
        const pdh2::SplitH y = pdh2::split4h(ry[par ^ 1][j], sy), x = pdh2::split4h(rx[par ^ 1][j], sx);
        *reinterpret_cast<uint2 *>(S(par ^ 1, 0, 0, r) + sc) = y.hi; *reinterpret_cast<uint2 *>(S(par ^ 1, 0, 1, r) + sc) = y.lo;
        *reinterpret_cast<uint2 *>(S(par ^ 1, 1, 0, r) + sc) = x.hi; *reinterpret_cast<uint2 *>(S(par ^ 1, 1, 1, r) + sc) = x.lo;
        bsum.x += ry[par ^ 1][j].x; bsum.y += ry[par ^ 1][j].y; bsum.z += ry[par ^ 1][j].z; bsum.w += ry[par ^ 1][j].w;
      }
#define WFTERM(PA, PB)                                                       \
  _Pragma("unroll") for (int i = 0; i < 2; ++i)                              \
      _Pragma("unroll") for (int j = 0; j < 4; ++j)                          \
        pdh2::mmah(acc[i][j], __builtin_bit_cast(pdh2::h16x8, a[PA][i]), __builtin_bit_cast(pdh2::h16x8, b[PB][j]));
      WFTERM(1, 0) WFTERM(0, 1) WFTERM(0, 0)
#undef WFTERM
      __builtin_amdgcn_sched_group_barrier(0x100, 24, 0);
#pragma unroll
      for (int g = 0; g < 24; ++g) {
        __builtin_amdgcn_sched_group_barrier(0x008, 1, 0);
        __builtin_amdgcn_sched_group_barrier(0x002, 3, 0);
        if (g % 3 == 2) __builtin_amdgcn_sched_group_barrier(0x200, 1, 0);
        if (g % 6 == 5) __builtin_amdgcn_sched_group_barrier(0x020, 1, 0);
      }
      __syncthreads();
    };
    for (; st0 + 3 < steps; st0 += 2) {
      fstep(st0, 0);
      fstep(st0 + 1, 1);
    }
  }
  for (int st = st0; st < steps; st += 2) {
    step(st, 0);
    if (st + 1 < steps) step(st + 1, 1);
  }
  if (do_bias) {
    float *red = reinterpret_cast<float *>(Sw);
    *reinterpret_cast<float4 *>(red + sr * WTD + sc) = bsum;
    __syncthreads();
    if (t < WTD && n0 + t < N) {
      float v = 0.f;
#pragma unroll
      for (int r = 0; r < 8; ++r) v += red[r * WTD + t];
      unsafeAtomicAdd(dB + n0 + t, v);
    }
  }
  if (ws) {
    float *w = ws + (ws_tile0 + (int64_t)split * tiles + tile) * (WTD * WTD) + t;
#pragma unroll
    for (int i = 0; i < 2; ++i)
#pragma unroll
      for (int j = 0; j < 4; ++j)
#pragma unroll
        for (int e = 0; e < 16; ++e) w[((i * 4 + j) * 16 + e) * WNT] = acc[i][j][e] * inv_yx;
    return;
  }
#pragma unroll
  for (int j = 0; j < 4; ++j) {
    const int c = k0 + wk + j * 32 + (lane & 31);
    if (c >= K) continue;
#pragma unroll
    for (int i = 0; i < 2; ++i)
#pragma unroll
      for (int e = 0; e < 16; ++e) {
        const int row = n0 + wn + i * 32 + (e & 3) + 8 * (e >> 2) + 4 * (lane >> 5);
        if (row < N) unsafeAtomicAdd(dW + (int64_t)row * ldw + c, acc[i][j][e] * inv_yx);
      }
  }
}

template <bool CONV>
__global__ __launch_bounds__(512, 1) void gemm_wgrad_f16x2_wide(const float *__restrict__ dY, const float *__restrict__ X, float *__restrict__ dW,
                                                                float *__restrict__ dB, float *__restrict__ ws, int M, int N, int K, int ldy, int ldx,
                                                                int ldw, int tiles_k, int tiles, int m_chunk, int H, int W,
                                                                const float *__restrict__ y_amax, const float *__restrict__ x_amax)
{
  wgrad_h2w_body<CONV>(dY, X, dW, dB, ws, M, N, K, ldy, ldx, ldw, tiles_k, tiles, m_chunk, H, W, xcd_chunk((int)blockIdx.x, (int)gridDim.x), 0,
                       y_amax, x_amax);
}

__device__ __forceinline__ void h2w_coord(int q, int t, int &row, int &col)
{
  const int lane = t & 63, wave = t >> 6, ij = q >> 4, e = q & 15, i = ij >> 2, j = ij & 3;
  row = (wave >> 1) * 64 + i * 32 + (e & 3) + 8 * (e >> 2) + 4 * (lane >> 5);
  col = (wave & 1) * 128 + j * 32 + (lane & 31);
}

__global__ __launch_bounds__(512) void wgrad_h2w_reduce(const float *__restrict__ ws, float *__restrict__ dW, int N, int K, int ldw, int tiles_k,
                                                        int tiles, int splits)
{
  const int tile = blockIdx.x >> 7, q = blockIdx.x & 127, t = threadIdx.x;
  const int n0 = (tile / tiles_k) * WTD, k0 = (tile % tiles_k) * WTD;
  const float *p = ws + (int64_t)tile * (WTD * WTD) + q * WNT + t;
  const int64_t stride = (int64_t)tiles * (WTD * WTD);
  float s0 = 0.f, s1 = 0.f;
  int sp = blockIdx.y;
  const int G = gridDim.y;
  for (; sp + 7 * G < splits; sp += 8 * G) {
    float v[8];
#pragma unroll
    for (int u = 0; u < 8; ++u) v[u] = p[(int64_t)(sp + u * G) * stride];
#pragma unroll
    for (int u = 0; u < 8; u += 2) { s0 += v[u]; s1 += v[u + 1]; }
  }
  for (; sp < splits; sp += G) s0 += p[(int64_t)sp * stride];
  int row, col;
  h2w_coord(q, t, row, col);
  if (k0 + col < K && n0 + row < N) {
    float *d = dW + (int64_t)(n0 + row) * ldw + k0 + col;
    if (G == 1) *d += s0 + s1; else unsafeAtomicAdd(d, s0 + s1);
  }
// ... 227 lines not shown
  static bool attr = false;
  if (!attr) { (void)hipFuncSetAttribute((const void *)gemm_tn_f32x3_wide<true>, hipFuncAttributeMaxDynamicSharedMemorySize, (int)lds); attr = true; }
  hipLaunchKernelGGL(gemm_tn_f32x3_wide<true>, dim3((unsigned)((int64_t)wtm * wtn)), dim3(512), lds, (hipStream_t)stream_, A, B, bias, C, M, N, K,
                     lda, ldb, ldc, wtn, bits, (float *)nullptr);
  return pd_check_launch("pd_gemm_tn_f32x3_relu_bits");
}

extern "C" int pd_gemm_tn_f32x3_relumask(const float *A, const float *B, const uint32_t *bits, float *C, float *colsum, int M, int N, int K,
                                         int lda, int ldb, int ldc, void *stream_)
{
  if (M < 0 || N < 0 || K < 0) return pd_set_error(PD_ERR_INVALID_ARG, "pd_gemm_tn_f32x3_relumask: negative size");
  if (M == 0 || N == 0) return PD_OK;
  if (!A || !B || !C || !bits || !colsum) return pd_set_error(PD_ERR_INVALID_ARG, "pd_gemm_tn_f32x3_relumask: null pointer");
  if ((K & 3) || (lda & 3) || (ldb & 3) || ((uintptr_t)A & 15) || ((uintptr_t)B & 15) || (N % WBN) || M < 4 * WBM)
    return pd_set_error(PD_ERR_INVALID_ARG, "pd_gemm_tn_f32x3_relumask: K, lda, ldb multiples of 4, N a multiple of 256, M >= 1024, A, B 16-byte aligned");
  const int wtn = N / WBN, wtm = (M + WBM - 1) / WBM;
  const size_t lds = (size_t)2 * 3 * 2 * (WBM + WBN) * 8 * sizeof(bf16_t);
  static bool attr = false;
  if (!attr) { (void)hipFuncSetAttribute((const void *)gemm_tn_f32x3_wide<false, 0, true>, hipFuncAttributeMaxDynamicSharedMemorySize, (int)lds); attr = true; }
  hipLaunchKernelGGL((gemm_tn_f32x3_wide<false, 0, true>), dim3((unsigned)((int64_t)wtm * wtn)), dim3(512), lds, (hipStream_t)stream_, A, B,
                     (const float *)nullptr, C, M, N, K, lda, ldb, ldc, wtn, const_cast<uint32_t *>(bits), colsum);
  return pd_check_launch("pd_gemm_tn_f32x3_relumask");
}

int g_pd_dbg_wgrad_wide = 1;
static bool wgrad_wide_ok(int N, int K, int conv_ci)
{
  return g_pd_dbg_wgrad_wide && N > 128 && K > 128 && (N >= 1024 || K >= 1024) && (conv_ci == 0 || conv_ci % WTD == 0);
}
extern "C" int pd_gemm_wgrad_f16x2_takes_wide_tiles(int N, int K) { return wgrad_wide_ok(N, K, 0) ? 1 : 0; }

static int wgrad_x3_launch(const float *dY, const float *X, float *dW, float *dB, float *ws, int64_t ws_floats, int M, int N, int K, int ldy,
                           int ldx, int ldw, hipStream_t st, const char *who, int convH = 0, int convW = 0, bool h2 = false,
                           const float *y_amax = nullptr, const float *x_amax = nullptr)
{
  if (M < 0 || N < 0 || K < 0) return pd_set_error(PD_ERR_INVALID_ARG, "%s: negative size", who);
  if (N == 0 || K == 0 || M == 0) return PD_OK;
  if (!dW || !dY || !X) return pd_set_error(PD_ERR_INVALID_ARG, "%s: null pointer", who);
  const int tk = (K + BM - 1) / BM, tn = (N + BN - 1) / BN, tiles = tk * tn;
  int splits;
  if (g_pd_dbg_x3 == 22) { const int target = tiles <= 4 ? 256 : 1024; splits = (target + tiles - 1) / tiles; }
  else splits = tiles >= 512 ? 1 : (512 + tiles / 2) / tiles;
  int m_chunk = ((M + splits - 1) / splits + WS - 1) / WS * WS;
  if (m_chunk < 4 * WS) m_chunk = 4 * WS;
  splits = (M + m_chunk - 1) / m_chunk;
  const bool vec = !(N & 3) && !(K & 3) && !(ldy & 3) && !(ldx & 3) && !((uintptr_t)dY & 15) && !((uintptr_t)X & 15) && g_pd_dbg_x3 != 21;
  if (convH && !vec) return pd_set_error(PD_ERR_INVALID_ARG, "%s: channel counts must be multiples of 4 and the tensors 16-byte aligned", who);
  if (h2 && !vec) return pd_set_error(PD_ERR_INVALID_ARG, "%s: N, K, ldy, ldx must be multiples of 4 and dY, X 16-byte aligned", who);
  if (!vec) {
    hipLaunchKernelGGL(gemm_wgrad_f32x3, dim3((unsigned)(tiles * splits)), dim3(256), 0, st, dY, X, dW, dB, M, N, K, ldy, ldx, ldw, tk, tiles,
                       m_chunk);
    return pd_check_launch(who);
  }
  if (h2 && wgrad_wide_ok(N, K, convH ? ldx : 0)) {
    const int wtk = (K + WTD - 1) / WTD, wtn = (N + WTD - 1) / WTD, wtiles = wtk * wtn;
    int wsplits = wtiles >= 256 ? 1 : (256 + wtiles / 2) / wtiles;
    int mc = ((M + wsplits - 1) / wsplits + TWS - 1) / TWS * TWS;
    if (mc < 4 * TWS) mc = 4 * TWS;
    wsplits = (M + mc - 1) / mc;
    if (ws && (ws_floats < (int64_t)wtiles * wsplits * WTD * WTD || wsplits < 2)) ws = nullptr;
    constexpr size_t lds = (size_t)2 * 2 * 2 * TWS * WTP * sizeof(bf16_t);
    static bool attr = false;
    if (!attr) {
      (void)hipFuncSetAttribute((const void *)gemm_wgrad_f16x2_wide<false>, hipFuncAttributeMaxDynamicSharedMemorySize, (int)lds);
      (void)hipFuncSetAttribute((const void *)gemm_wgrad_f16x2_wide<true>, hipFuncAttributeMaxDynamicSharedMemorySize, (int)lds);
      attr = true;
    }
    auto kw = convH ? gemm_wgrad_f16x2_wide<true> : gemm_wgrad_f16x2_wide<false>;
    hipLaunchKernelGGL(kw, dim3((unsigned)(wtiles * wsplits)), dim3(WNT), lds, st, dY, X, dW, dB, ws, M, N, K, ldy, ldx, ldw, wtk, wtiles, mc, convH, convW,
                       y_amax, x_amax);
    const int wgroups = wtiles * 128 >= 2048 ? 1 : wsplits >= 64 ? 8 : wsplits >= 16 ? 4 : 1;
    if (ws) hipLaunchKernelGGL(wgrad_h2w_reduce, dim3((unsigned)(wtiles * 128), wgroups), dim3(WNT), 0, st, (const float *)ws, dW, N, K, ldw, wtk, wtiles, wsplits);
    return pd_check_launch(who);
  }
  if (ws && (ws_floats < (int64_t)tiles * splits * BN * BM || splits < 2 || g_pd_dbg_x3 == 25)) ws = nullptr;
  auto kfn = h2 ? (convH ? gemm_wgrad_f32x3_tr<0, true, true> : gemm_wgrad_f32x3_tr<0, false, true>)
                 : convH ? gemm_wgrad_f32x3_tr<0, true> : g_pd_dbg_x3 == 24 ? gemm_wgrad_f32x3_tr<2, false> : gemm_wgrad_f32x3_tr<0, false>;
  hipLaunchKernelGGL(kfn, dim3((unsigned)(tiles * splits)), dim3(256), 0, st, dY, X, dW, dB, ws, M, N, K, ldy, ldx, ldw, tk, tiles, m_chunk,
                     convH, convW, y_amax, x_amax);
  const int groups = tiles * 64 >= 2048 ? 1 : splits >= 64 ? 8 : splits >= 16 ? 4 : 1;
  if (ws) hipLaunchKernelGGL(wgrad_tr_reduce, dim3((unsigned)(tiles * 64), groups), dim3(256), 0, st, (const float *)ws, dW, N, K, ldw, tk, tiles,
                             splits);
  return pd_check_launch(who);
}


extern "C" int64_t pd_gemm_wgrad_f32x3_grouped_table_bytes(int max_count) { return (int64_t)(max_count > 0 ? max_count : 0) * (int64_t)sizeof(WgradX3Problem); }

static bool grouped_wide(const PdGemmWgradDesc *d, int count)
{
  for (int i = 0; i < count; ++i) if (!wgrad_wide_ok(d[i].N, d[i].K, 0)) return false;
  return count > 0;
}

static int grouped_plan(const PdGemmWgradDesc *d, int count, WgradX3Problem *tab, int64_t *ws_tiles, int *blocks, int TD = BM)
{
  int64_t total_tiles = 0;
  for (int i = 0; i < count; ++i) {
    if (d[i].M <= 0 || d[i].N <= 0 || d[i].K <= 0 || !d[i].dY || !d[i].X || !d[i].dW) return 1;
    if ((d[i].N & 3) || (d[i].K & 3) || (d[i].ldy & 3) || (d[i].ldx & 3) || ((uintptr_t)d[i].dY & 15) || ((uintptr_t)d[i].X & 15)) return 1;
    total_tiles += (int64_t)((d[i].K + TD - 1) / TD) * ((d[i].N + TD - 1) / TD);
  }
  int splits = (int)((6 * (TD == BM ? 512 : 256)) / (total_tiles > 0 ? total_tiles : 1));
  if (splits < 1) splits = 1;
  int64_t wt = 0; int b0 = 0;
  for (int i = 0; i < count; ++i) {
    WgradX3Problem &q = tab[i];
    q.dY = d[i].dY; q.X = d[i].X; q.dW = d[i].dW; q.dB = d[i].dB;
    q.M = d[i].M; q.N = d[i].N; q.K = d[i].K; q.ldy = d[i].ldy; q.ldx = d[i].ldx; q.ldw = d[i].ldw;
// ... 59 lines not shown

extern "C" int pd_gemm_wgrad_f16x2_grouped(const PdGemmWgradDesc *descs, int count, void *table_host_pinned, void *table_device,
                                           float *workspace, int64_t workspace_floats, void *stream_)
{
  return wgrad_grouped(descs, count, table_host_pinned, table_device, workspace, workspace_floats, stream_, true);
}

extern "C" int64_t pd_gemm_wgrad_f16x2_ws_floats(int N, int K)
{
  const int64_t narrow = pd_gemm_wgrad_f32x3_ws_floats(N, K);
  if (N <= 0 || K <= 0) return narrow;
  const int64_t wt = (int64_t)((K + WTD - 1) / WTD) * ((N + WTD - 1) / WTD);
  const int64_t wide = wt >= 256 ? 0 : (256 + wt / 2) / wt * wt * WTD * WTD;
  return wide > narrow ? wide : narrow;
}

extern "C" int64_t pd_gemm_wgrad_f16x2_grouped_ws_floats(const PdGemmWgradDesc *descs, int count)
{
  if (count <= 0 || count > 256 || !descs) return 0;
  WgradX3Problem tab[256];
  int64_t wt = 0; int blocks = 0;
  const int TD = grouped_wide(descs, count) ? WTD : BM;
  if (grouped_plan(descs, count, tab, &wt, &blocks, TD)) return -1;
  return wt * TD * TD;
}

extern "C" int pd_gemm_wgrad_acc_f16x2_ws(const float *dY, const float *X, float *dW, float *dB, const float *y_amax, const float *x_amax,
                                          float *workspace, int64_t workspace_floats, int M, int N, int K, int ldy, int ldx, int ldw, void *stream_)
{
  return wgrad_x3_launch(dY, X, dW, dB, workspace, workspace_floats, M, N, K, ldy, ldx, ldw, (hipStream_t)stream_, "pd_gemm_wgrad_acc_f16x2_ws", 0, 0,
                         true, y_amax, x_amax);
}

extern "C" int pd_conv3x3_wgrad_nhwc_f16x2(const float *dY, const float *X, float *dWk, float *dB, const float *y_amax, const float *x_amax,
                                           float *workspace, int64_t workspace_floats, int B, int H, int W, int Ci, int Co, void *stream_)
{
  if (B < 0 || H <= 0 || W <= 0 || Ci <= 0 || Co <= 0 || (Ci % BM) || (Co & 3))
    return pd_set_error(PD_ERR_INVALID_ARG, "pd_conv3x3_wgrad_nhwc_f16x2: B=%d H=%d W=%d Ci=%d (%% 128) Co=%d (%% 4)", B, H, W, Ci, Co);
  const int64_t M = (int64_t)B * H * W;
  if (M > 0x7fffffffLL - 4096) return pd_set_error(PD_ERR_INVALID_ARG, "pd_conv3x3_wgrad_nhwc_f16x2: too many pixels");
  return wgrad_x3_launch(dY, X, dWk, dB, workspace, workspace_floats, (int)M, Co, 9 * Ci, Co, Ci, 9 * Ci, (hipStream_t)stream_,
                         "pd_conv3x3_wgrad_nhwc_f16x2", H, W, true, y_amax, x_amax);
}

extern "C" int pd_gemm_wgrad_acc_f32x3(const float *dY, const float *X, float *dW, float *dB, int M, int N, int K, int ldy, int ldx,
                                       int ldw, void *stream_)
{
  return wgrad_x3_launch(dY, X, dW, dB, nullptr, 0, M, N, K, ldy, ldx, ldw, (hipStream_t)stream_, "pd_gemm_wgrad_acc_f32x3");
}

extern "C" int64_t pd_gemm_wgrad_f32x3_ws_floats(int N, int K)
{
  const int64_t tiles = (int64_t)((K + BM - 1) / BM) * ((N + BN - 1) / BN);
  return tiles >= 512 ? 0 : (512 + tiles / 2) / tiles * tiles * BN * BM;
}

extern "C" int pd_gemm_wgrad_acc_f32x3_ws(const float *dY, const float *X, float *dW, float *dB, float *workspace, int64_t workspace_floats,
                                          int M, int N, int K, int ldy, int ldx, int ldw, void *stream_)
{
  return wgrad_x3_launch(dY, X, dW, dB, workspace, workspace_floats, M, N, K, ldy, ldx, ldw, (hipStream_t)stream_, "pd_gemm_wgrad_acc_f32x3_ws");
}

extern "C" int pd_conv3x3_wgrad_nhwc_f32x3(const float *dY, const float *X, float *dWk, float *dB, float *workspace, int64_t workspace_floats,
                                           int B, int H, int W, int Ci, int Co, void *stream_)
{
  if (B < 0 || H <= 0 || W <= 0 || Ci <= 0 || Co <= 0 || (Ci % BM) || (Co & 3))
// ... 24 lines not shown
```

### partdistillation_amd/functions/conv_x3.py

```python
import torch
from torch.autograd import Function

from .. import lib as _lib


H2 = __import__("os").environ.get("PD_H2_CONV", "1") != "0"
H2_1X1 = __import__("os").environ.get("PD_H2_1X1", "1") != "0"
WGRAD_X3 = True


def supported(x, conv):
    return (x.is_cuda and x.dtype == torch.float32 and x.dim() == 4 and conv.weight.dtype == torch.float32
            and tuple(conv.kernel_size) == (3, 3) and tuple(conv.stride) == (1, 1) and tuple(conv.padding) == (1, 1)
            and tuple(conv.dilation) == (1, 1) and conv.groups == 1 and x.shape[1] % 16 == 0 and conv.weight.shape[0] % 16 == 0
            and x.is_contiguous(memory_format=torch.channels_last))


def _pixel_amax(x):
    from . import amax_cache
    from .gemm import row_amax
    am = amax_cache.get(x)
    return am if am is not None else row_amax(x.permute(0, 2, 3, 1).reshape(-1, x.shape[1]))


def _raw(x, wk, bias, co, x_amax=None):
    B, ci, H, W = x.shape
    y = torch.empty((B, co, H, W), dtype=torch.float32, device=x.device, memory_format=torch.channels_last)
    from .gemm import _timed_fwd, row_amax
    if x_amax is not None:
        w_amax = row_amax(wk.view(co, -1))
        with _timed_fwd(2.0 * B * H * W * 9 * ci * co, "gemm_tn_f16x2<256, 256, 128, 16, 0, conv 3x3>", 4.0 * (B * H * W * (ci + co) + 9 * ci * co)):
            _lib.check(_lib.load().pd_conv3x3_nhwc_f16x2(x.data_ptr(), wk.data_ptr(), bias.data_ptr() if bias is not None else None, y.data_ptr(),
                                                         x_amax.data_ptr(), w_amax.data_ptr(), None, B, H, W, ci, co, _lib.current_stream()))
        return y
    with _timed_fwd(2.0 * B * H * W * 9 * ci * co, "gemm_tn_f32x3<conv 3x3>"):
        _lib.check(_lib.load().pd_conv3x3_nhwc_f32x3(x.data_ptr(), wk.data_ptr(), bias.data_ptr() if bias is not None else None, y.data_ptr(),
                                                     B, H, W, ci, co, _lib.current_stream()))
    return y


# ... 24 lines not shown
            from .gemm import _wgrad_workspace
            L = _lib.load()
            B, _, H, W = x.shape
            buf = torch.zeros(co * 9 * ci + co, dtype=torch.float32, device=x.device)
            dwk, dbv = buf[:co * 9 * ci].view(co, 3, 3, ci), buf[co * 9 * ci:]
            ws = _wgrad_workspace(x.device, int((L.pd_gemm_wgrad_f16x2_ws_floats if x_am is not None else L.pd_gemm_wgrad_f32x3_ws_floats)(co, 9 * ci)))
            if x_am is not None:
                _lib.check(L.pd_conv3x3_wgrad_nhwc_f16x2(dy.data_ptr(), x.data_ptr(), dwk.data_ptr(), dbv.data_ptr() if want_b else None,
                                                         dy_am.data_ptr(), x_am.data_ptr(), ws.data_ptr() if ws is not None else None,
                                                         ws.numel() if ws is not None else 0, B, H, W, ci, co, _lib.current_stream()))
            else:
                _lib.check(L.pd_conv3x3_wgrad_nhwc_f32x3(dy.data_ptr(), x.data_ptr(), dwk.data_ptr(), dbv.data_ptr() if want_b else None,
                                                         ws.data_ptr() if ws is not None else None, ws.numel() if ws is not None else 0,
                                                         B, H, W, ci, co, _lib.current_stream()))
            dw = dwk.permute(0, 3, 1, 2) if want_w else None
            db = dbv if want_b else None
        elif want_w or want_b:
            _, dw, db = torch.ops.aten.convolution_backward(dy, x, weight, [co] if ctx.has_bias else None, [1, 1], [1, 1], [1, 1], False,
                                                            [0, 0], 1, [False, True, ctx.has_bias])
        return dx, dw, db


def conv3x3(x, weight, bias=None):
    return Conv3x3X3.apply(x, weight, bias)


class Conv1x1OwnWgrad(Function):

    @staticmethod
    def forward(ctx, x, weight, bias):
        ctx.has_bias = bias is not None
        ctx.x_bf16 = x.dtype == torch.bfloat16
        if H2 and H2_1X1 and x.is_contiguous(memory_format=torch.channels_last):
            from .gemm import cast_rows_amax, gemm_tn_h2, row_amax
            B, ci, Hh, Ww = x.shape
            co = weight.shape[0]
            if ctx.x_bf16:
                x2, x_am = cast_rows_amax(x.permute(0, 2, 3, 1).reshape(-1, ci))
                x = x2.view(B, Hh, Ww, ci).permute(0, 3, 1, 2)
            else:
                x_am = _pixel_amax(x)
            w2 = weight.reshape(co, ci)
            y = gemm_tn_h2(x.permute(0, 2, 3, 1).reshape(-1, ci), w2, bias, a_amax=x_am, b_amax=row_amax(w2))
            ctx.save_for_backward(x, weight, x_am)
            return y.view(B, Hh, Ww, co).permute(0, 3, 1, 2)
        if ctx.x_bf16:
            x = x.float()
        ctx.save_for_backward(x, weight, None)
        return torch.ops.aten.convolution(x, weight, bias, [1, 1], [0, 0], [1, 1], False, [0, 0], 1)

    @staticmethod
    def backward(ctx, dy):
        from .gemm import gemm_tn_h2, gemm_tn_h2_bf16out, gemm_wgrad_acc, row_amax
        x, weight, x_am = ctx.saved_tensors
        dy = dy.contiguous(memory_format=torch.channels_last)
        co, ci = weight.shape[0], weight.shape[1]
        dx = dw = db = None
        rows = lambda t: t.permute(0, 2, 3, 1).reshape(-1, t.shape[1])
        h2 = x_am is not None
        dy_am = _pixel_amax(dy) if h2 else None
        if ctx.needs_input_grad[0]:
            if h2:
                wt = weight.reshape(co, ci).t().contiguous()
                B, _, Hh, Ww = x.shape
                mm = gemm_tn_h2_bf16out if ctx.x_bf16 else gemm_tn_h2
                dx = mm(rows(dy), wt, None, a_amax=dy_am, b_amax=row_amax(wt)).view(B, Hh, Ww, ci).permute(0, 3, 1, 2)
            else:
                dx = torch.ops.aten.convolution_backward(dy, x, weight, None, [1, 1], [0, 0], [1, 1], False, [0, 0], 1, [True, False, False])[0]
                dx = dx.to(torch.bfloat16) if ctx.x_bf16 else dx
        want_w, want_b = ctx.needs_input_grad[1], ctx.has_bias and ctx.needs_input_grad[2]
        if want_w or want_b:
            buf = torch.zeros(co * ci + co, dtype=torch.float32, device=x.device)
            dw2, dbv = buf[:co * ci].view(co, ci), buf[co * ci:]
            if h2:
                gemm_wgrad_acc(rows(dy), rows(x), dw2, dbv if want_b else None, h2=True, y_amax=dy_am, x_amax=x_am)
            else:
                gemm_wgrad_acc(rows(dy), rows(x), dw2, dbv if want_b else None, x3=True)
            dw = dw2.view(co, ci, 1, 1).as_strided(weight.shape, weight.stride()) if want_w else None
            db = dbv if want_b else None
        return dx, dw, db


def conv1x1_supported(x, conv):
    return (WGRAD_X3 and x.is_cuda and (x.dtype == torch.float32 or (x.dtype == torch.bfloat16 and H2 and H2_1X1 and x.shape[1] % 8 == 0))
            and x.dim() == 4 and conv.weight.dtype == torch.float32
            and tuple(conv.kernel_size) == (1, 1) and tuple(conv.stride) == (1, 1) and tuple(conv.padding) == (0, 0)
            and tuple(conv.dilation) == (1, 1) and conv.groups == 1 and x.shape[1] % 4 == 0 and conv.weight.shape[0] % 4 == 0
            and x.is_contiguous(memory_format=torch.channels_last) and torch.is_grad_enabled())


def conv1x1(x, weight, bias=None):
    return Conv1x1OwnWgrad.apply(x, weight, bias)
```

### partdistillation_amd/functions/gemm.py

```python
import ctypes

import torch
from torch.autograd import Function

from .. import lib as _lib


def _stream():
    return _lib.current_stream()


def gemm_tn(a, b, bias=None, relu=False):
    if not a.is_cuda:
        raise RuntimeError("pd_gemm_tn_f32 runs on the GPU only (no CPU fallback in partdistillation_amd)")
    assert a.dtype == torch.float32 and b.dtype == torch.float32 and a.stride(1) == 1 and b.stride(1) == 1
    M, K = a.shape
    N = b.shape[0]
    c = torch.empty((M, N), dtype=torch.float32, device=a.device)
    with torch.cuda.device(a.device):
        rc = _lib.load().pd_gemm_tn_f32(a.data_ptr(), b.data_ptr(), bias.data_ptr() if bias is not None else None,
                                        c.data_ptr(), M, N, K, a.stride(0), b.stride(0), N, int(relu), _stream())
    _lib.check(rc)
    return c

# ... 13 lines not shown

    def __exit__(self, *exc):
        if _TIMING["on"]:
            self.b.record()
            _TIMING["fwd"].append((self.a, self.b, (self.flops, self.label, self.nbytes)))


def gemm_tn_x3(a, b, bias=None, relu=False):
    if not a.is_cuda:
        raise RuntimeError("pd_gemm_tn_f32x3 runs on the GPU only (no CPU fallback in partdistillation_amd)")
    assert a.dtype == torch.float32 and b.dtype == torch.float32 and a.stride(1) == 1 and b.stride(1) == 1
    M, K = a.shape
    N = b.shape[0]
    c = torch.empty((M, N), dtype=torch.float32, device=a.device)
    with _timed_fwd(2.0 * M * N * K, "gemm_tn_f32x3(_wide)"):
        _lib.check(_lib.load().pd_gemm_tn_f32x3(a.data_ptr(), b.data_ptr(), bias.data_ptr() if bias is not None else None, c.data_ptr(),
                                                M, N, K, a.stride(0), b.stride(0), N, int(relu), _stream()))
    return c


def row_amax(x):
    assert x.is_cuda and x.dtype == torch.float32 and x.dim() == 2 and x.stride(1) == 1
    out = torch.empty(x.shape[0], dtype=torch.float32, device=x.device)
    _lib.check(_lib.load().pd_row_amax_f32(x.data_ptr(), x.shape[0], x.shape[1], x.stride(0), out.data_ptr(), _stream()))
    return out


def cast_rows_amax(x):
    assert x.is_cuda and x.dtype == torch.bfloat16 and x.dim() == 2 and x.is_contiguous() and x.shape[1] % 8 == 0
    y = torch.empty(x.shape, dtype=torch.float32, device=x.device)
    am = torch.empty(x.shape[0], dtype=torch.float32, device=x.device)
    _lib.check(_lib.load().pd_cast_bf16_f32_amax(x.data_ptr(), x.shape[0], x.shape[1], y.data_ptr(), am.data_ptr(), _stream()))
    return y, am


def gemm_tn_h2_bf16out(a, b, bias=None, a_amax=None, b_amax=None):
    if not a.is_cuda:
        raise RuntimeError("pd_gemm_tn_f16x2_bf16out runs on the GPU only (no CPU fallback in partdistillation_amd)")
    assert a.dtype == torch.float32 and b.dtype == torch.float32 and a.stride(1) == 1 and b.stride(1) == 1 and b.shape[1] == a.shape[1]
    M, K = a.shape
    N = b.shape[0]
    c = torch.empty((M, N), dtype=torch.bfloat16, device=a.device)
    p = lambda t: t.data_ptr() if t is not None else None
    _lib.check(_lib.load().pd_gemm_tn_f16x2_bf16out(a.data_ptr(), b.data_ptr(), p(bias), c.data_ptr(), p(a_amax), p(b_amax), M, N, K, a.stride(0),
                                                    b.stride(0), N, _stream()))
    return c


def h2_bits_supported(M, N):
    return N % 256 == 0 and M >= 1024


def gemm_tn_h2(a, b, bias=None, mode=0, bits=None, colsum=None, a_amax=None, b_amax=None, c_amax=None, want_bits=False):
    if not a.is_cuda:
        raise RuntimeError("pd_gemm_tn_f16x2 runs on the GPU only (no CPU fallback in partdistillation_amd)")
    assert a.dtype == torch.float32 and b.dtype == torch.float32 and a.stride(1) == 1 and b.stride(1) == 1
    M, K = a.shape
    N = b.shape[0]
    assert b.shape[1] == K
    for v, n in ((a_amax, M), (b_amax, N), (c_amax, M)):
        assert v is None or (v.dtype == torch.float32 and v.is_contiguous() and v.numel() == n)
    L = _lib.load()
    c = torch.empty((M, N), dtype=torch.float32, device=a.device)
    if mode == 1 and want_bits:
        bits = torch.empty(int(L.pd_gemm_tn_f16x2_bits_words(M, N)), dtype=torch.int32, device=a.device)
    p = lambda t: t.data_ptr() if t is not None else None
# ... 68 lines not shown
                                                         M, N, K, a.stride(0), b.stride(0), N, _stream()))
    return c


def enable_timing(on=True):
    _TIMING["on"] = on
    _TIMING["wgrad"].clear()
    _TIMING["fwd"].clear()


def timing(which="wgrad"):
    return [(a.elapsed_time(b), f) for a, b, f in _TIMING[which]]


WGRAD_X3 = True


_WGRAD_WS = {}


def _wgrad_workspace(device, need):
    if need <= 0:
        return None
    key = (str(device), torch.cuda.current_stream(device).cuda_stream)
    ws = _WGRAD_WS.get(key)
    if ws is None or ws.numel() < need:
        ws = _WGRAD_WS[key] = torch.empty(max(need, 8912896), dtype=torch.float32, device=device)
    return ws


def gemm_wgrad_acc(dy, x, dw, db=None, x3=None, h2=False, y_amax=None, x_amax=None):
    M, N = dy.shape
    K = x.shape[1]
    assert dw.shape == (N, K) and dw.is_contiguous() and (db is None or db.numel() == N)
    assert dy.dtype == torch.float32 and x.dtype == torch.float32 and dy.stride(1) == 1 and x.stride(1) == 1
    if _TIMING["on"]:
        a, b = torch.cuda.Event(enable_timing=True), torch.cuda.Event(enable_timing=True)
        a.record()
    L = _lib.load()
    if h2:
        ws = _wgrad_workspace(dy.device, int(L.pd_gemm_wgrad_f16x2_ws_floats(N, K)))
        _lib.check(L.pd_gemm_wgrad_acc_f16x2_ws(dy.data_ptr(), x.data_ptr(), dw.data_ptr(), db.data_ptr() if db is not None else None,
                                                y_amax.data_ptr() if y_amax is not None else None, x_amax.data_ptr() if x_amax is not None else None,
                                                ws.data_ptr() if ws is not None else None, ws.numel() if ws is not None else 0,
                                                M, N, K, dy.stride(0), x.stride(0), K, _stream()))
    elif WGRAD_X3 if x3 is None else x3:
        ws = _wgrad_workspace(dy.device, int(L.pd_gemm_wgrad_f32x3_ws_floats(N, K)))
        _lib.check(L.pd_gemm_wgrad_acc_f32x3_ws(dy.data_ptr(), x.data_ptr(), dw.data_ptr(), db.data_ptr() if db is not None else None,
                                                ws.data_ptr() if ws is not None else None, ws.numel() if ws is not None else 0,
                                                M, N, K, dy.stride(0), x.stride(0), K, _stream()))
    else:
        _lib.check(L.pd_gemm_wgrad_acc_f32(dy.data_ptr(), x.data_ptr(), dw.data_ptr(), db.data_ptr() if db is not None else None,
                                           M, N, K, dy.stride(0), x.stride(0), K, _stream()))
    if _TIMING["on"]:
        b.record()
        _TIMING["wgrad"].append((a, b, (2.0 * M * N * K, 4.0 * (M * N + M * K + N * K), "h2" if h2 else "x3")))


class _WgradDesc(ctypes.Structure):
    _fields_ = [("dY", ctypes.c_void_p), ("X", ctypes.c_void_p), ("dW", ctypes.c_void_p), ("dB", ctypes.c_void_p)] + \
               [(n, ctypes.c_int32) for n in ("M", "N", "K", "ldy", "ldx", "ldw")] + [("y_amax", ctypes.c_void_p), ("x_amax", ctypes.c_void_p)]


class WgradQueue:
    MAXP = 256
    _ring = None
    _table_dev = {}
    _ws = {}

    def __init__(self, h2=False):
        self.items = []
        self.h2 = h2

    def add(self, dy, x, dw, db=None, y_amax=None, x_amax=None):
        M, N = dy.shape
# ... 131 lines not shown
```

### partdistillation_amd/lib.py

```python
import ctypes
import os
import subprocess

_HERE = os.path.dirname(os.path.abspath(__file__))
LIB_PATH = os.environ.get("PD_LIB_PATH") or os.path.join(_HERE, "libpd_hip.so")
CSRC = os.path.join(_HERE, "csrc")

PD_F32, PD_F64, PD_BF16 = 0, 1, 2
ABI_VERSION = 47

_c_int, _c_vp = ctypes.c_int, ctypes.c_void_p

SIGNATURES = {
    "pd_msda_forward": (_c_int, [_c_vp] * 6 + [_c_int] * 9 + [_c_vp]),
    "pd_msda_backward": (_c_int, [_c_vp] * 9 + [_c_int] * 9 + [_c_vp]),
    "pd_msda_backward_last_gate": (_c_int, [_c_vp]),
    "pd_stem7x7_fwd": (_c_int, [_c_vp, _c_int] + [_c_vp] * 4 + [_c_int] * 4 + [_c_vp]),
    "pd_stem_wgrad_workspace_floats": (ctypes.c_int64, []),
    "pd_stem7x7_wgrad": (_c_int, [_c_vp, _c_int] + [_c_vp] * 4 + [_c_int, _c_vp] + [_c_int] * 4 + [_c_vp]),
    "pd_msda_fused_supported": (_c_int, [_c_int] * 7),
    "pd_msda_fused_forward": (_c_int, [_c_vp] * 4 + [_c_int] + [_c_vp] * 4 + [_c_int] * 7 + [_c_vp]),
    "pd_msda_fused_backward": (_c_int, [_c_vp] * 4 + [_c_int] + [_c_vp] * 6 + [_c_int, _c_vp, _c_vp] + [_c_int] * 7 + [_c_vp]),
    "pd_lsa_batched": (_c_int, [_c_vp] * 4 + [_c_int] * 3 + [_c_vp]),
    "pd_sumsq_accumulate": (_c_int, [_c_vp, ctypes.c_int64, _c_int, _c_vp, _c_vp]),
    "pd_adamw_clipped": (_c_int, [_c_vp] * 4 + [ctypes.c_int64, _c_int] + [ctypes.c_double] * 5 + [_c_int, _c_vp, ctypes.c_double, _c_vp, _c_vp]),
    "pd_gemm_tn_f32": (_c_int, [_c_vp] * 4 + [_c_int] * 7 + [_c_vp]),
    "pd_gemm_tn_f32x3": (_c_int, [_c_vp] * 4 + [_c_int] * 7 + [_c_vp]),
    "pd_gemm_wgrad_f16x2_takes_wide_tiles": (_c_int, [_c_int] * 2),
    "pd_gemm_wgrad_f16x2_ws_floats": (ctypes.c_int64, [_c_int] * 2),
    "pd_gemm_wgrad_f16x2_grouped_ws_floats": (ctypes.c_int64, [_c_vp, _c_int]),
    "pd_gemm_wgrad_acc_f16x2_ws": (_c_int, [_c_vp] * 7 + [ctypes.c_int64] + [_c_int] * 6 + [_c_vp]),
    "pd_gemm_wgrad_f16x2_grouped": (_c_int, [_c_vp, _c_int, _c_vp, _c_vp, _c_vp, ctypes.c_int64, _c_vp]),
    "pd_conv3x3_wgrad_nhwc_f16x2": (_c_int, [_c_vp] * 7 + [ctypes.c_int64] + [_c_int] * 5 + [_c_vp]),
    "pd_conv3x3_nhwc_f16x2": (_c_int, [_c_vp] * 7 + [_c_int] * 5 + [_c_vp]),
    "pd_gemm_tn_f16x2_which": (_c_int, [_c_int] * 6),
    "pd_gemm_tn_f16x2_bits_words": (ctypes.c_int64, [_c_int] * 2),
    "pd_gemm_tn_f16x2": (_c_int, [_c_vp] * 9 + [_c_int] * 7 + [_c_vp]),
    "pd_gemm_tn_f16x2_bf16out": (_c_int, [_c_vp] * 6 + [_c_int] * 6 + [_c_vp]),
    "pd_cast_bf16_f32_amax": (_c_int, [_c_vp, _c_int, _c_int, _c_vp, _c_vp, _c_vp]),
    "pd_row_amax_f32": (_c_int, [_c_vp, _c_int, _c_int, _c_int, _c_vp, _c_vp]),
    "pd_gemm_tn_f32x3_relumask": (_c_int, [_c_vp] * 5 + [_c_int] * 6 + [_c_vp]),
    "pd_gemm_tn_f32x3_relu_bits": (_c_int, [_c_vp] * 5 + [_c_int] * 6 + [_c_vp]),
    "pd_gemm_tn_f32x3_relu_bits_words": (ctypes.c_int64, [_c_int] * 2),
    "pd_split3_bf16": (_c_int, [_c_vp, _c_int, _c_int, _c_int, _c_int, _c_vp, _c_vp]),
    "pd_gemm_tn_f32x3_pre": (_c_int, [_c_vp] * 6 + [_c_int] * 6 + [_c_vp]),
    "pd_gemm_wgrad_f32": (_c_int, [_c_vp] * 4 + [_c_int] * 6 + [_c_vp]),
    "pd_gemm_wgrad_acc_f32": (_c_int, [_c_vp] * 4 + [_c_int] * 6 + [_c_vp]),
    "pd_conv3x3_nhwc_f32x3": (_c_int, [_c_vp] * 4 + [_c_int] * 5 + [_c_vp]),
    "pd_gemm_wgrad_acc_f32x3": (_c_int, [_c_vp] * 4 + [_c_int] * 6 + [_c_vp]),
    "pd_conv3x3_wgrad_nhwc_f32x3": (_c_int, [_c_vp] * 5 + [ctypes.c_int64] + [_c_int] * 5 + [_c_vp]),
    "pd_gemm_wgrad_f32x3_ws_floats": (ctypes.c_int64, [_c_int] * 2),
    "pd_gemm_wgrad_f32x3_grouped_table_bytes": (ctypes.c_int64, [_c_int]),
    "pd_gemm_wgrad_f32x3_grouped_ws_floats": (ctypes.c_int64, [_c_vp, _c_int]),
    "pd_gemm_wgrad_f32x3_grouped": (_c_int, [_c_vp, _c_int, _c_vp, _c_vp, _c_vp, ctypes.c_int64, _c_vp]),
    "pd_gemm_wgrad_acc_f32x3_ws": (_c_int, [_c_vp] * 5 + [ctypes.c_int64] + [_c_int] * 6 + [_c_vp]),
    "pd_adamw_clipped_shadow": (_c_int, [_c_vp] * 5 + [ctypes.c_int64] + [ctypes.c_double] * 5 + [_c_int, _c_vp, ctypes.c_double, _c_vp, _c_vp]),
    "pd_conv_bf16_supported": (_c_int, [_c_int] * 5),
    "pd_conv_bf16_fwd": (_c_int, [_c_vp] * 6 + [_c_int] * 11 + [_c_vp]),
    "pd_conv_bf16_wgrad_workspace_floats": (ctypes.c_int64, [_c_int] * 6),
    "pd_conv_bf16_wgrad": (_c_int, [_c_vp] * 4 + [ctypes.c_int64] + [_c_int] * 10 + [_c_vp]),
    "pd_conv_bf16_wgrad_grouped_table_bytes": (ctypes.c_int64, [_c_int]),
    "pd_conv_bf16_wgrad_grouped_workspace_floats": (ctypes.c_int64, [_c_vp, _c_int]),
    "pd_conv_bf16_wgrad_grouped": (_c_int, [_c_vp, _c_int, _c_vp, _c_vp, _c_vp, ctypes.c_int64, _c_vp]),
    "pd_conv_bf16_dgrad": (_c_int, [_c_vp] * 4 + [_c_int] * 10 + [_c_vp]),
    "pd_maxpool3s2_fwd_bf16": (_c_int, [_c_vp] * 3 + [_c_int] * 4 + [_c_vp]),
    "pd_maxpool3s2_bwd_bf16": (_c_int, [_c_vp] * 3 + [_c_int] * 4 + [_c_vp]),
    "pd_affine_act_fwd_bf16": (_c_int, [_c_vp] * 5 + [ctypes.c_int64, _c_int, _c_int, _c_vp]),
    "pd_affine_act_bwd_bf16": (_c_int, [_c_vp] * 5 + [ctypes.c_int64, _c_int, _c_int, _c_vp]),
    "pd_affine_act_bwd2_bf16": (_c_int, [_c_vp] * 6 + [ctypes.c_int64, _c_int, _c_int, _c_vp]),
    "pd_multi_gather_sumsq": (_c_int, [_c_vp] * 8 + [_c_int, _c_int, _c_vp]),
    "pd_attn_workspace_floats": (ctypes.c_int64, [_c_int] * 4),
    "pd_attn_fwd_d32": (_c_int, [_c_vp] * 7 + [_c_int] * 4 + [ctypes.c_float, _c_int, _c_vp]),
    "pd_attn_bwd_d32": (_c_int, [_c_vp] * 11 + [_c_int] * 4 + [ctypes.c_float, _c_int, _c_vp]),
# ... 213 lines not shown
```

Baseline: 110.0.

## Feed bf16 activations directly into f16x2 GEMMs and fuse weight operand prep

```diff
diff --git a/include/pd_gemm.h b/include/pd_gemm.h
--- a/include/pd_gemm.h
+++ b/include/pd_gemm.h
@@ -72,6 +72,16 @@
                              int K, int lda, int ldb, int ldc, void *stream);
 int pd_cast_bf16_f32_amax(const void *X_bf16, int rows, int cols, float *Y, float *row_amax, void *stream);
 
+
+int pd_row_amax_bf16(const void *X_bf16, int rows, int cols, int ld, float *out, void *stream);
+int pd_gemm_tn_f16x2_a16_supported(int M, int N, int K);
+int pd_gemm_tn_f16x2_a16_which(int M, int N, int K);
+int pd_gemm_tn_f16x2_a16(const void *A_bf16, const float *B, const float *bias, float *C, const float *a_amax, const float *b_amax, int M, int N, int K, int lda,
+                         int ldb, int ldc, void *stream);
+int pd_gemm_wgrad_acc_f16x2_x16_ws(const float *dY, const void *X_bf16, float *dW, float *dB, const float *y_amax, const float *x_amax, float *workspace,
+                                   int64_t workspace_floats, int M, int N, int K, int ldy, int ldx, int ldw, void *stream);
+int pd_weight_operands_f32(const float *W, int co, int ci, int ldw, float *w_amax, float *Wt, float *wt_amax, void *stream);
+
 #ifdef __cplusplus
 }
 #endif
diff --git a/partdistillation_amd/csrc/cmdbuf.hip b/partdistillation_amd/csrc/cmdbuf.hip
--- a/partdistillation_amd/csrc/cmdbuf.hip
+++ b/partdistillation_amd/csrc/cmdbuf.hip
@@ -86,7 +86,9 @@
   PD_E(pd_decoder_head_bf16),
   PD_E(pd_filter_transpose_grouped),
   PD_E(pd_gemm_tn_f16x2),
+  PD_E(pd_gemm_tn_f16x2_a16),
   PD_E(pd_gemm_tn_f16x2_bf16out),
+  PD_E(pd_gemm_wgrad_acc_f16x2_x16_ws),
   PD_E(pd_gemm_tn_f32),
   PD_E(pd_gemm_tn_f32x3),
   PD_E(pd_gemm_tn_f32x3_pre),
@@ -169,7 +171,9 @@
   PD_E(pd_rle_sample_groups_canvas_u8),
   PD_E(pd_rle_sample_groups_u8),
   PD_E(pd_rle_sample_u8),
+  PD_E(pd_row_amax_bf16),
   PD_E(pd_row_amax_f32),
+  PD_E(pd_weight_operands_f32),
   PD_E(pd_scores_argmax_u8),
   PD_E(pd_sgemm_nn_bf16),
   PD_E(pd_sgemm_nn_splitn_bf16),
diff --git a/partdistillation_amd/csrc/common.hip b/partdistillation_amd/csrc/common.hip
--- a/partdistillation_amd/csrc/common.hip
+++ b/partdistillation_amd/csrc/common.hip
@@ -27,7 +27,7 @@
 }
 
 extern "C" const char *pd_last_error(void) { return g_err; }
-extern "C" int pd_abi_version(void) { return 47; }
+extern "C" int pd_abi_version(void) { return 48; }
 
 extern int g_pd_dbg_atomic_scope;
 extern int g_pd_dbg_force_generic;
diff --git a/partdistillation_amd/csrc/f16x2.h b/partdistillation_amd/csrc/f16x2.h
--- a/partdistillation_amd/csrc/f16x2.h
+++ b/partdistillation_amd/csrc/f16x2.h
@@ -12,7 +12,7 @@
 __device__ __forceinline__ void row_scale(float amax, float &s, float &inv)
 {
   int e = (int)((__float_as_uint(amax) >> 23) & 0xffu);
-  e = e < 20 ? 20 : (e > 250 ? 250 : e);
+  e = e < 20 ? 20 : (e > 254 ? 254 : e);
   s = __uint_as_float((unsigned)(268 - e) << 23);
   inv = __uint_as_float((unsigned)(e - 14) << 23);
 }
@@ -60,6 +60,18 @@
   return split4h_p(v, s);
 #endif
 }
+__device__ __forceinline__ uint2 cvt4h_bf16(uint2 v, float s)
+{
+  const f32x2 a = {__uint_as_float(v.x << 16) * s, __uint_as_float(v.x & 0xffff0000u) * s};
+  const f32x2 b = {__uint_as_float(v.y << 16) * s, __uint_as_float(v.y & 0xffff0000u) * s};
+  return make_uint2(__builtin_bit_cast(unsigned, __builtin_convertvector(a, h16x2)), __builtin_bit_cast(unsigned, __builtin_convertvector(b, h16x2)));
+}
+__device__ __forceinline__ uint2 cvt4h_bf16_u(uint2 v, float s)
+{
+  const f32x2 a = {np_mul(__uint_as_float(v.x << 16), s), np_mul(__uint_as_float(v.x & 0xffff0000u), s)};
+  const f32x2 b = {np_mul(__uint_as_float(v.y << 16), s), np_mul(__uint_as_float(v.y & 0xffff0000u), s)};
+  return make_uint2(__builtin_bit_cast(unsigned, __builtin_convertvector(a, h16x2)), __builtin_bit_cast(unsigned, __builtin_convertvector(b, h16x2)));
+}
 __device__ __forceinline__ void mmah(f32x16 &c, h16x8 x, h16x8 y) { c = __builtin_amdgcn_mfma_f32_32x32x16_f16(x, y, c, 0, 0, 0); }
 
 }
diff --git a/partdistillation_amd/csrc/gemm_f16x2.hip b/partdistillation_amd/csrc/gemm_f16x2.hip
--- a/partdistillation_amd/csrc/gemm_f16x2.hip
+++ b/partdistillation_amd/csrc/gemm_f16x2.hip
@@ -24,7 +24,7 @@
   return (unsigned short)(u >> 16);
 }
 
-template <int TM, int TN, int WN, int BKK, int MODE, bool CONV = false, int NRS = 1, int FAST = 0>
+template <int TM, int TN, int WN, int BKK, int MODE, bool CONV = false, int NRS = 1, int FAST = 0, bool A16 = false>
 __global__ __launch_bounds__((TM / 64) * (TN / WN) * 64, (TM == 256 ? 1 : 2))
 void gemm_tn_f16x2(const float *__restrict__ A, const float *__restrict__ B, const float *__restrict__ bias, float *__restrict__ C,
                    int M, int N, int K, int lda, int ldb, int ldc, int ntiles_n, uint32_t *__restrict__ bits,
@@ -70,6 +70,9 @@
 #pragma unroll
   for (int j = 0; j < BPASS; ++j) sb[j] = sc[TM + lr + RPP * j];
   float4 ra[NRS][APASS], rb[NRS][BPASS];
+  uint2 ra16[NRS][APASS];
+  static_assert(!A16 || !CONV, "the bf16-A form is a plain GEMM");
+  const unsigned short *A16p = reinterpret_cast<const unsigned short *>(A);
   int py[APASS], px[APASS];
   if (CONV) {
 #pragma unroll
@@ -102,6 +105,8 @@
         const int yy = py[j] + dy, xx = px[j] + dx;
         const bool ok = m0 + r < M && k < K && yy >= 0 && yy < H && xx >= 0 && xx < W;
         ra[rs][j] = ok ? *reinterpret_cast<const float4 *>(A + ((int64_t)(m0 + r) + dy * W + dx) * lda + kc) : make_float4(0, 0, 0, 0);
+      } else if (A16) {
+        ra16[rs][j] = (m0 + r < M && k < K) ? *reinterpret_cast<const uint2 *>(A16p + (int64_t)(m0 + r) * lda + k) : make_uint2(0u, 0u);
       } else {
         ra[rs][j] = (m0 + r < M && k < K) ? *reinterpret_cast<const float4 *>(A + (int64_t)(m0 + r) * lda + k) : make_float4(0, 0, 0, 0);
       }
@@ -122,8 +127,9 @@
     }
 #pragma unroll
     for (int j = 0; j < APASS; ++j) {
+      h16_t *p = As(buf, 0, lk >> 3, lr + RPP * j) + (lk & 7);
+      if constexpr (A16) { *reinterpret_cast<uint2 *>(p) = cvt4h_bf16(ra16[rs][j], sa[j]); continue; }
       const SplitH x = split4h(ra[rs][j], sa[j]);
-      h16_t *p = As(buf, 0, lk >> 3, lr + RPP * j) + (lk & 7);
       *reinterpret_cast<uint2 *>(p) = x.hi; *reinterpret_cast<uint2 *>(p + NPAN * TM * 8) = x.lo;
     }
 #pragma unroll
@@ -157,7 +163,7 @@
     for (int ks = 0; ks < ((PD_ABL & 2) ? 0 : BKK / 16); ++ks) {
       h16x8 a[2][2];
 #pragma unroll
-      for (int pl = 0; pl < 2; ++pl)
+      for (int pl = 0; pl < (A16 ? 1 : 2); ++pl)
 #pragma unroll
         for (int i = 0; i < 2; ++i) a[pl][i] = *reinterpret_cast<const h16x8 *>(As(par, pl, 2 * ks + fh, wm + i * 32 + fr));
 #pragma unroll
@@ -176,7 +182,7 @@
   _Pragma("unroll") for (int i = 0; i < 2; ++i)                              \
       _Pragma("unroll") for (int j = 0; j < 2; ++j) mmah(acc[i][jp * 2 + j], a[PA][i], b[PB][j]);
 #endif
-        HTERM(1, 0)
+        if constexpr (!A16) { HTERM(1, 0) }
         HTERM(0, 1)
         HTERM(0, 0)
 #undef HTERM
@@ -188,8 +194,9 @@
   if constexpr (FAST != 0 && BKK == 16) {
     if (m0 + TM <= M && n0 + TN <= N && (K % (2 * BKK)) == 0 && KT >= 4 && (!CONV || tap_minor)) {
       const float *pa[APASS], *pb[BPASS];
-#pragma unroll
-      for (int j = 0; j < APASS; ++j) pa[j] = A + (int64_t)(m0 + lr + RPP * j) * lda + lk;
+      const unsigned short *pa16[APASS];
+#pragma unroll
+      for (int j = 0; j < APASS; ++j) { pa[j] = A + (int64_t)(m0 + lr + RPP * j) * lda + lk; pa16[j] = A16p + (int64_t)(m0 + lr + RPP * j) * lda + lk; }
 #pragma unroll
       for (int j = 0; j < BPASS; ++j) pb[j] = B + (int64_t)(n0 + lr + RPP * j) * ldb + lk;
       auto fstep = [&](int kt, int par) {
@@ -204,14 +211,19 @@
 #pragma unroll
         for (int pl = 0; pl < 2; ++pl) {
 #pragma unroll
-          for (int i = 0; i < 2; ++i) a[pl][i] = *reinterpret_cast<const h16x8 *>(As(par, pl, fh, wm + i * 32 + fr));
+          for (int i = 0; i < 2; ++i) if (!A16 || pl == 0) a[pl][i] = *reinterpret_cast<const h16x8 *>(As(par, pl, fh, wm + i * 32 + fr));
 #pragma unroll
           for (int j = 0; j < NJ; ++j) b[pl][j] = *reinterpret_cast<const h16x8 *>(Bs(par, pl, fh, wn + j * 32 + fr));
         }
 #pragma unroll
         for (int j = 0; j < APASS; ++j) {
+          h16_t *p = As(par ^ 1, 0, lk >> 3, lr + RPP * j) + (lk & 7);
+          if constexpr (A16) {
+            *reinterpret_cast<uint2 *>(p) = cvt4h_bf16(ra16[rs][j], sa[j]);
+            ra16[rs][j] = *reinterpret_cast<const uint2 *>(pa16[j] + kn);
+            continue;
+          }
           const SplitH x = split4h(ra[rs][j], sa[j]);
-          h16_t *p = As(par ^ 1, 0, lk >> 3, lr + RPP * j) + (lk & 7);
           *reinterpret_cast<uint2 *>(p) = x.hi; *reinterpret_cast<uint2 *>(p + NPAN * TM * 8) = x.lo;
           if (CONV) {
             const int yy = py[j] + dy, xx = px[j] + dx;
@@ -232,13 +244,13 @@
 #define FTERM(PA, PB)                                                        \
   _Pragma("unroll") for (int i = 0; i < 2; ++i)                              \
       _Pragma("unroll") for (int j = 0; j < NJ; ++j) mmah(acc[i][j], a[PA][i], b[PB][j]);
-        FTERM(1, 0)
+        if constexpr (!A16) { FTERM(1, 0) }
         FTERM(0, 1)
         FTERM(0, 0)
 #undef FTERM
         if constexpr (FAST == 1) {
-          constexpr int NM = 6 * NJ, NV = (12 * (APASS + BPASS) + 8 + NM - 1) / NM, EV = NM / (APASS + BPASS);
-          __builtin_amdgcn_sched_group_barrier(0x100, 4 + 2 * NJ, 0);
+          constexpr int NM = (A16 ? 4 : 6) * NJ, NV = (12 * (APASS + BPASS) + 8 + NM - 1) / NM, EV = NM / (APASS + BPASS);
+          __builtin_amdgcn_sched_group_barrier(0x100, (A16 ? 2 : 4) + 2 * NJ, 0);
 #pragma unroll
           for (int g = 0; g < NM; ++g) {
             __builtin_amdgcn_sched_group_barrier(0x008, 1, 0);
@@ -328,13 +340,22 @@
   }
 }
 
+template <bool BF16 = false>
 __global__ __launch_bounds__(256) void row_amax_f32(const float *__restrict__ X, int rows, int cols, int ld, float *__restrict__ out)
 {
   const int row = blockIdx.x * 4 + (threadIdx.x >> 6), lane = threadIdx.x & 63;
   if (row >= rows) return;
   const float *p = X + (int64_t)row * ld;
   float v = 0.f;
-  if (!(cols & 3) && !(ld & 3) && !((uintptr_t)X & 15)) {
+  if constexpr (BF16) {
+    const unsigned short *q = reinterpret_cast<const unsigned short *>(X) + (int64_t)row * ld;
+    for (int c = lane * 8; c < cols; c += 512) {
+      const uint4 u = *reinterpret_cast<const uint4 *>(q + c);
+      const unsigned w[4] = {u.x, u.y, u.z, u.w};
+#pragma unroll
+      for (int k = 0; k < 4; ++k) v = fmaxf(v, fmaxf(fabsf(__uint_as_float(w[k] << 16)), fabsf(__uint_as_float(w[k] & 0xffff0000u))));
+    }
+  } else if (!(cols & 3) && !(ld & 3) && !((uintptr_t)X & 15)) {
     for (int c = lane * 4; c < cols; c += 256) {
       const float4 x = *reinterpret_cast<const float4 *>(p + c);
       v = fmaxf(fmaxf(v, fmaxf(fabsf(x.x), fabsf(x.y))), fmaxf(fabsf(x.z), fabsf(x.w)));
@@ -347,6 +368,63 @@
   if (lane == 0) out[row] = v;
 }
 
+
+__global__ __launch_bounds__(256) void row_amax_f32_wt(const float *__restrict__ W, int co, int ci, int ldw, float *__restrict__ w_amax, float *__restrict__ Wt,
+                                                       float *__restrict__ wt_amax, int tiles, int tiles_c, int cblocks)
+{
+  __shared__ float tile[32][33];
+  const int t = threadIdx.x, lane = t & 63, wave = t >> 6;
+  int b = blockIdx.x;
+  if (b < tiles) {
+    const int c0 = (b % tiles_c) * 32, r0 = (b / tiles_c) * 32, tx = t & 31, ty = t >> 5;
+#pragma unroll
+    for (int j = 0; j < 4; ++j) {
+      const int r = r0 + ty + 8 * j, c = c0 + tx;
+      tile[ty + 8 * j][tx] = (r < co && c < ci) ? W[(int64_t)r * ldw + c] : 0.f;
+    }
+    __syncthreads();
+#pragma unroll
+    for (int j = 0; j < 4; ++j) {
+      const int c = c0 + ty + 8 * j, r = r0 + tx;
+      if (c < ci && r < co) Wt[(int64_t)c * co + r] = tile[tx][ty + 8 * j];
+    }
+    return;
+  }
+  b -= tiles;
+  if (b < cblocks) {
+    const int c = b * 64 + lane;
+    float v = 0.f;
+    if (c < ci) {
+      int r = wave;
+      for (; r + 12 < co; r += 16) {
+        const float x0 = W[(int64_t)r * ldw + c], x1 = W[(int64_t)(r + 4) * ldw + c], x2 = W[(int64_t)(r + 8) * ldw + c], x3 = W[(int64_t)(r + 12) * ldw + c];
+        v = fmaxf(fmaxf(v, fmaxf(fabsf(x0), fabsf(x1))), fmaxf(fabsf(x2), fabsf(x3)));
+      }
+      for (; r < co; r += 4) v = fmaxf(v, fabsf(W[(int64_t)r * ldw + c]));
+    }
+    float *cm = &tile[0][0];
+    cm[wave * 64 + lane] = v;
+    __syncthreads();
+    if (t < 64 && c < ci) wt_amax[c] = fmaxf(fmaxf(cm[t], cm[64 + t]), fmaxf(cm[128 + t], cm[192 + t]));
+    return;
+  }
+  b -= cblocks;
+  const int row = b * 4 + wave;
+  if (row >= co) return;
+  const float *p = W + (int64_t)row * ldw;
+  float v = 0.f;
+  if (!(ci & 3) && !(ldw & 3) && !((uintptr_t)W & 15)) {
+    for (int c = lane * 4; c < ci; c += 256) {
+      const float4 x = *reinterpret_cast<const float4 *>(p + c);
+      v = fmaxf(fmaxf(v, fmaxf(fabsf(x.x), fabsf(x.y))), fmaxf(fabsf(x.z), fabsf(x.w)));
+    }
+  } else {
+    for (int c = lane; c < ci; c += 64) v = fmaxf(v, fabsf(p[c]));
+  }
+#pragma unroll
+  for (int o = 32; o; o >>= 1) v = fmaxf(v, __shfl_xor(v, o, 64));
+  if (lane == 0) w_amax[row] = v;
+}
 
 __global__ __launch_bounds__(256) void cast_bf16_f32_amax(const unsigned short *__restrict__ X, int rows, int cols, float *__restrict__ Y,
                                                           float *__restrict__ out)
@@ -373,6 +451,7 @@
 
 constexpr int RS_PANEL = 528, RS_PLANE = 32 * RS_PANEL, RS_BUF = 2 * RS_PLANE;
 typedef unsigned u32x4 __attribute__((ext_vector_type(4)));
+typedef unsigned u32x2 __attribute__((ext_vector_type(2)));
 
 #ifdef PD_ROWS_PACKED_SPLIT
 #define ROWS_SPLIT split4h
@@ -380,7 +459,7 @@
 #define ROWS_SPLIT split4h_u
 #endif
 __device__ int g_rows_wstage = 1;
-template <bool AM, int MODE = 0>
+template <bool AM, int MODE = 0, bool A16 = false>
 __global__ __launch_bounds__(512)
 void gemm_rows_f16x2_k256(const float *__restrict__ A, const float *__restrict__ B, const float *__restrict__ bias, float *__restrict__ C,
                           int M, int npanels, int lda, int ldb, int ldc, const float *__restrict__ a_amax,
@@ -398,13 +477,15 @@
   const int n0 = panel * 256 + w * 32;
 
   float4 R[2][4];
+  uint2 R16[2][4];
   float am[2][4];
   auto gload = [&](int rs, int tile) {
     tile = min(tile, t1 - 1);
 #pragma unroll
     for (int j = 0; j < 4; ++j) {
       const int row = min(tile * 32 + w + 8 * j, M - 1);
-      if (PD_ABL & 8) R[rs][j] = make_float4(1.f, 0.5f, 0.25f, (float)row);
+      if (A16) R16[rs][j] = *reinterpret_cast<const uint2 *>(reinterpret_cast<const unsigned short *>(A) + (int64_t)row * lda + 4 * lane);
+      else if (PD_ABL & 8) R[rs][j] = make_float4(1.f, 0.5f, 0.25f, (float)row);
       else R[rs][j] = *reinterpret_cast<const float4 *>(A + (int64_t)row * lda + 4 * lane);
       am[rs][j] = AM ? a_amax[row] : 0.f;
     }
@@ -416,8 +497,9 @@
       float s = 1.f;
       invs[j] = 1.f;
       if (AM) row_scale(am[rs][j], s, invs[j]);
+      unsigned char *p = (buf ? lds1 : lds0) + (lane >> 1) * RS_PANEL + (w + 8 * j) * 16 + (lane & 1) * 8;
+      if constexpr (A16) { *reinterpret_cast<uint2 *>(p) = cvt4h_bf16_u(R16[rs][j], s); continue; }
       const SplitH v = ROWS_SPLIT(R[rs][j], s);
-      unsigned char *p = (buf ? lds1 : lds0) + (lane >> 1) * RS_PANEL + (w + 8 * j) * 16 + (lane & 1) * 8;
       if (PD_ABL & 4) { asm volatile("" ::"v"(R[rs][j].x), "v"(R[rs][j].y), "v"(R[rs][j].z), "v"(R[rs][j].w)); continue; }
       *reinterpret_cast<uint2 *>(p) = v.hi;
       *reinterpret_cast<uint2 *>(p + RS_PLANE) = v.lo;
@@ -492,6 +574,7 @@
 #pragma unroll
     for (int s = 0; s < ((PD_ABL & 1) ? 0 : 16); ++s) {
       const h16x8 ah = (PD_ABL & 2) ? bl[15 - s] : *reinterpret_cast<const h16x8 *>(base + 2 * s * RS_PANEL);
+      if constexpr (A16) { mmah(acc0, ah, bl[s]); mmah(acc0, ah, bh[s]); continue; }
       const h16x8 al = (PD_ABL & 2) ? bh[15 - s] : *reinterpret_cast<const h16x8 *>(base + 2 * s * RS_PANEL + RS_PLANE);
 #ifdef PD_ROWS_TWO_CHAINS
       if (s & 1) { mmah(acc1, al, bh[s]); mmah(acc0, ah, bl[s]); mmah(acc1, ah, bh[s]); }
@@ -508,8 +591,10 @@
       __builtin_amdgcn_sched_group_barrier(0x002, 2, 0);
       __builtin_amdgcn_sched_group_barrier(0x008, 1, 0);
       __builtin_amdgcn_sched_group_barrier(0x002, 2, 0);
-      __builtin_amdgcn_sched_group_barrier(0x008, 1, 0);
-      __builtin_amdgcn_sched_group_barrier(0x002, 2, 0);
+      if (!A16) {
+        __builtin_amdgcn_sched_group_barrier(0x008, 1, 0);
+        __builtin_amdgcn_sched_group_barrier(0x002, 2, 0);
+      }
       if (s & 1) __builtin_amdgcn_sched_group_barrier(0x200, 1, 0);
       if ((s & 3) == 3) __builtin_amdgcn_sched_group_barrier(0x020, 1, 0);
     }
@@ -609,7 +694,7 @@
   asm volatile("" ::: "memory");
 }
 
-template <bool AM, int KABL = 0, bool BP = false, bool CONV = false>
+template <bool AM, int KABL = 0, bool BP = false, bool CONV = false, bool A16 = false>
 __global__ __launch_bounds__(768)
 void gemm_kpc_f16x2(const float *__restrict__ A, const float *__restrict__ B, const float *__restrict__ bias, float *__restrict__ C, int M, int K,
                     int lda, int ldb, int ldc, int npanels, const float *__restrict__ a_amax, const float *__restrict__ b_amax, int H = 0, int W = 0)
@@ -655,7 +740,7 @@
         sb[j] = 1.f;
         if (AM) row_scale(b_amax[c0 + prow + 32 * j], sb[j], inv);
       }
-      const __amdgpu_buffer_rsrc_t ra = __builtin_amdgcn_make_buffer_rsrc(const_cast<float *>(A), 0, (int)((int64_t)M * lda * 4), 0x00020000);
+      const __amdgpu_buffer_rsrc_t ra = __builtin_amdgcn_make_buffer_rsrc(const_cast<float *>(A), 0, (int)((int64_t)M * lda * (A16 ? 2 : 4)), 0x00020000);
       const int64_t bbytes = BP ? (int64_t)2 * npanels * 256 * K * 2 : (int64_t)(c0 + 256) * ldb * 4;
       const __amdgpu_buffer_rsrc_t rbs = __builtin_amdgcn_make_buffer_rsrc(const_cast<float *>(B), 0, (int)bbytes, 0x00020000);
       unsigned oa[6], ob[8];
@@ -663,7 +748,7 @@
 #pragma unroll
       for (int j = 0; j < 6; ++j) {
         const int row = row0 + prow + 32 * j;
-        oa[j] = ((unsigned)row * (unsigned)lda + 4u * pc4) * 4u;
+        oa[j] = ((unsigned)row * (unsigned)lda + 4u * pc4) * (A16 ? 2u : 4u);
         pyx[j] = 0u;
         if (CONV && row < M) {
           const int pix = row % (H * W), y = pix / W, x = pix - y * W;
@@ -684,6 +769,8 @@
         }
       }
       float4 RA[3][3], RB[3][4];
+      uint2 RA16[3][3];
+      static_assert(!A16 || !CONV, "the bf16-A form is a plain GEMM");
       auto gload = [&](int rs, int u) {
         const int kcl = min(u >> 1, NC - 1), ko = kcl * (KR_KC * 4), h = u & 1;
         int tap = 0, shift = 0;
@@ -697,6 +784,11 @@
         for (int j = 0; j < 3; ++j) {
           unsigned off = h ? oa[3 + j] : oa[j];
           if (CONV) off = (((h ? pyx[3 + j] : pyx[j]) >> tap) & 1u) ? off + (unsigned)shift : 0x80000000u;
+          if constexpr (A16) {
+            const u32x2 v2 = __builtin_amdgcn_raw_buffer_load_b64(ra, off, ko / 2, 0);
+            RA16[rs][j] = make_uint2(v2.x, v2.y);
+            continue;
+          }
           const u32x4 v = __builtin_amdgcn_raw_buffer_load_b128(ra, off, CONV ? 0 : ko, 0);
           RA[rs][j] = make_float4(__uint_as_float(v.x), __uint_as_float(v.y), __uint_as_float(v.z), __uint_as_float(v.w));
         }
@@ -711,8 +803,9 @@
         unsigned char *bb = bimg + buf * KR_BBUF + (pc4 >> 1) * KR_BPANEL + (pc4 & 1) * 8;
 #pragma unroll
         for (int j = 0; j < 3; ++j) {
+          unsigned char *p = ab + (prow + 32 * (3 * h + j)) * 16;
+          if constexpr (A16) { *reinterpret_cast<uint2 *>(p) = cvt4h_bf16_u(RA16[rs][j], h ? sa[3 + j] : sa[j]); continue; }
           const SplitH v = split4h_u(RA[rs][j], h ? sa[3 + j] : sa[j]);
-          unsigned char *p = ab + (prow + 32 * (3 * h + j)) * 16;
           *reinterpret_cast<uint2 *>(p) = v.hi;
           *reinterpret_cast<uint2 *>(p + KR_APLANE) = v.lo;
         }
@@ -794,7 +887,7 @@
               al[ti] = ah[ti];
             } else {
               ah[ti] = *reinterpret_cast<const h16x8 *>(ab + 2 * s * KR_APANEL + ti * 32 * 16);
-              al[ti] = *reinterpret_cast<const h16x8 *>(ab + 2 * s * KR_APANEL + ti * 32 * 16 + KR_APLANE);
+              if (!A16) al[ti] = *reinterpret_cast<const h16x8 *>(ab + 2 * s * KR_APANEL + ti * 32 * 16 + KR_APLANE);
             }
           }
 #pragma unroll
@@ -815,10 +908,12 @@
             continue;
           }
           if (KABL & 16) { asm volatile("s_waitcnt lgkmcnt(0)" ::: "memory"); if (tr) kp_stamp(0, cc, 3 + s); }
-#pragma unroll
-          for (int ti = 0; ti < 3; ++ti)
-#pragma unroll
-            for (int cb = 0; cb < 2; ++cb) mmah(acc[ti][cb], al[ti], bh[cb]);
+          if constexpr (!A16) {
+#pragma unroll
+            for (int ti = 0; ti < 3; ++ti)
+#pragma unroll
+              for (int cb = 0; cb < 2; ++cb) mmah(acc[ti][cb], al[ti], bh[cb]);
+          }
 #pragma unroll
           for (int ti = 0; ti < 3; ++ti)
 #pragma unroll
@@ -1119,6 +1214,65 @@
   return gemm_tn_f16x2_impl(A, B, bias, reinterpret_cast<float *>(C_bf16), nullptr, nullptr, a_amax, b_amax, nullptr, M, N, K, lda, ldb, ldc, 0, stream_, 1);
 }
 
+static int ncu_of_device()
+{
+  static int ncu = 0;
+  if (!ncu) { int dev = 0; (void)hipGetDevice(&dev); if (hipDeviceGetAttribute(&ncu, hipDeviceAttributeMultiprocessorCount, dev) != hipSuccess || ncu < 8) ncu = 256; }
+  return ncu;
+}
+
+extern "C" int pd_gemm_tn_f16x2_a16_which(int M, int N, int K)
+{
+  if (M <= 0 || N <= 0 || K <= 0 || (K % 64)) return -1;
+  const int which = pd_gemm_tn_f16x2_which(M, N, K, 0, 0, 1);
+  if (which == 2 && N / 256 > 32) return 0;
+  if (which == 5 && ((int64_t)M * K * 4 >= (1ll << 31) || (int64_t)N * K * 4 >= (1ll << 31))) return 0;
+  return (which == 0 || which == 2 || which == 5) ? which : -1;
+}
+
+extern "C" int pd_gemm_tn_f16x2_a16_supported(int M, int N, int K) { return pd_gemm_tn_f16x2_a16_which(M, N, K) >= 0 ? 1 : 0; }
+
+extern "C" int pd_gemm_tn_f16x2_a16(const void *A_bf16, const float *B, const float *bias, float *C, const float *a_amax, const float *b_amax, int M, int N,
+                                    int K, int lda, int ldb, int ldc, void *stream_)
+{
+  if (M < 0 || N < 0 || K < 0) return pd_set_error(PD_ERR_INVALID_ARG, "pd_gemm_tn_f16x2_a16: negative size");
+  if (M == 0 || N == 0) return PD_OK;
+  if (!A_bf16 || !B || !C || !a_amax || !b_amax) return pd_set_error(PD_ERR_INVALID_ARG, "pd_gemm_tn_f16x2_a16: null pointer (both operands come with row maxima)");
+  if ((K % 64) || (lda & 7) || (ldb & 3) || lda < K || ldb < K || ldc < N || ((uintptr_t)A_bf16 & 15) || ((uintptr_t)B & 15))
+    return pd_set_error(PD_ERR_INVALID_ARG, "pd_gemm_tn_f16x2_a16: K=%d must be a multiple of 64, lda %% 8 == 0, ldb %% 4 == 0, A and B 16-byte aligned", K);
+  int which = pd_gemm_tn_f16x2_a16_which(M, N, K);
+  if (which < 0) return pd_set_error(PD_ERR_INVALID_ARG, "pd_gemm_tn_f16x2_a16: M=%d N=%d K=%d has no bf16-A kernel (pd_gemm_tn_f16x2_a16_supported)", M, N, K);
+  if (which == 5 && ((int64_t)M * lda * 4 >= (1ll << 31) || (int64_t)N * ldb * 4 >= (1ll << 31))) which = 0;
+  hipStream_t st = (hipStream_t)stream_;
+  const float *A = reinterpret_cast<const float *>(A_bf16);
+  const int np = N / 256;
+  if (which == 2) {
+    const int G = (ncu_of_device() / (8 * np)) * 8 * np;
+    hipLaunchKernelGGL((gemm_rows_f16x2_k256<true, 0, true>), dim3((unsigned)G), dim3(512), 0, st, A, B, bias, C, M, np, lda, ldb, ldc, a_amax, b_amax,
+                       (unsigned *)nullptr, (unsigned short *)nullptr, (float *)nullptr);
+    return pd_check_launch("pd_gemm_tn_f16x2_a16 (row stream)");
+  }
+  if (which == 5) {
+    const int nwork = ((M + KR_RB - 1) / KR_RB) * np, ncu = ncu_of_device(), G = nwork < ncu ? nwork : ncu;
+    static bool pattr = false;
+    if (!pattr) { (void)hipFuncSetAttribute((const void *)(gemm_kpc_f16x2<true, 0, false, false, true>), hipFuncAttributeMaxDynamicSharedMemorySize, (int)KP_LDS); pattr = true; }
+    hipLaunchKernelGGL((gemm_kpc_f16x2<true, 0, false, false, true>), dim3((unsigned)G), dim3(768), KP_LDS, st, A, B, bias, C, M, K, lda, ldb, ldc, np, a_amax, b_amax, 0, 0);
+    return pd_check_launch("pd_gemm_tn_f16x2_a16 (producer / consumer wavefronts)");
+  }
+  {
+    constexpr int TM = 128, TN = 128, WN = 64, NTH = (TM / 64) * (TN / WN) * 64;
+    constexpr size_t stage = (size_t)2 * 2 * (TM + TN) * 16 * sizeof(h16_t), red = (size_t)(NTH / 64) * 64 * 33 * sizeof(float);
+    constexpr size_t lds = (stage > red ? stage : red) + (size_t)2 * (TM + TN) * sizeof(float);
+    const int tn = (N + TN - 1) / TN, tm = (M + TM - 1) / TM;
+    auto k = gemm_tn_f16x2<TM, TN, WN, 16, 0, false, 2, 1, true>;
+    static bool attr = false;
+    if (!attr) { (void)hipFuncSetAttribute((const void *)k, hipFuncAttributeMaxDynamicSharedMemorySize, (int)lds); attr = true; }
+    hipLaunchKernelGGL(k, dim3((unsigned)((int64_t)tm * tn)), dim3(NTH), lds, st, A, B, bias, C, M, N, K, lda, ldb, ldc, tn, (uint32_t *)nullptr, (float *)nullptr,
+                       a_amax, b_amax, (unsigned *)nullptr, 0, 0, 1);
+    return pd_check_launch("pd_gemm_tn_f16x2_a16");
+  }
+}
+
 extern "C" int pd_cast_bf16_f32_amax(const void *X_bf16, int rows, int cols, float *Y, float *row_amax, void *stream_)
 {
   if (rows < 0 || cols <= 0 || (cols & 7)) return pd_set_error(PD_ERR_INVALID_ARG, "pd_cast_bf16_f32_amax: rows=%d cols=%d (a multiple of 8)", rows, cols);
@@ -1176,10 +1330,31 @@
   if (rows < 0 || cols < 0) return pd_set_error(PD_ERR_INVALID_ARG, "pd_row_amax_f32: negative size");
   if (rows == 0) return PD_OK;
   if (!X || !out) return pd_set_error(PD_ERR_INVALID_ARG, "pd_row_amax_f32: null pointer");
-  hipLaunchKernelGGL(row_amax_f32, dim3((unsigned)((rows + 3) / 4)), dim3(256), 0, (hipStream_t)stream_, X, rows, cols, ld, out);
+  hipLaunchKernelGGL(row_amax_f32<false>, dim3((unsigned)((rows + 3) / 4)), dim3(256), 0, (hipStream_t)stream_, X, rows, cols, ld, out);
   return pd_check_launch("pd_row_amax_f32");
 }
 
+extern "C" int pd_weight_operands_f32(const float *W, int co, int ci, int ldw, float *w_amax, float *Wt, float *wt_amax, void *stream_)
+{
+  if (co < 0 || ci < 0 || ldw < ci) return pd_set_error(PD_ERR_INVALID_ARG, "pd_weight_operands_f32: co=%d ci=%d ldw=%d", co, ci, ldw);
+  if (co == 0 || ci == 0) return PD_OK;
+  if (!W || !w_amax || ((Wt == nullptr) != (wt_amax == nullptr))) return pd_set_error(PD_ERR_INVALID_ARG, "pd_weight_operands_f32: null pointer (Wt and wt_amax come together)");
+  const int tiles_c = (ci + 31) / 32, tiles = Wt ? tiles_c * ((co + 31) / 32) : 0, cblocks = Wt ? (ci + 63) / 64 : 0;
+  hipLaunchKernelGGL(row_amax_f32_wt, dim3((unsigned)(tiles + cblocks + (co + 3) / 4)), dim3(256), 0, (hipStream_t)stream_, W, co, ci, ldw, w_amax, Wt, wt_amax, tiles,
+                     tiles_c, cblocks);
+  return pd_check_launch("pd_weight_operands_f32");
+}
+
+extern "C" int pd_row_amax_bf16(const void *X_bf16, int rows, int cols, int ld, float *out, void *stream_)
+{
+  if (rows < 0 || cols <= 0 || (cols & 7) || (ld & 7) || ld < cols) return pd_set_error(PD_ERR_INVALID_ARG, "pd_row_amax_bf16: rows=%d cols=%d ld=%d (multiples of 8)", rows, cols, ld);
+  if (rows == 0) return PD_OK;
+  if (!X_bf16 || !out || ((uintptr_t)X_bf16 & 15)) return pd_set_error(PD_ERR_INVALID_ARG, "pd_row_amax_bf16: null / misaligned pointer");
+  hipLaunchKernelGGL(row_amax_f32<true>, dim3((unsigned)((rows + 3) / 4)), dim3(256), 0, (hipStream_t)stream_, reinterpret_cast<const float *>(X_bf16), rows, cols,
+                     ld, out);
+  return pd_check_launch("pd_row_amax_bf16");
+}
+
 extern "C" int pd_debug_read_kpc_trace(unsigned long long *dst)
 {
   return hipMemcpyFromSymbol(dst, HIP_SYMBOL(g_kp_trace), sizeof(unsigned long long) * 2 * 64 * 8) == hipSuccess ? PD_OK : PD_ERR_LAUNCH;
diff --git a/partdistillation_amd/csrc/gemm_x3.hip b/partdistillation_amd/csrc/gemm_x3.hip
--- a/partdistillation_amd/csrc/gemm_x3.hip
+++ b/partdistillation_amd/csrc/gemm_x3.hip
@@ -438,7 +438,7 @@
   return u.v;
 }
 
-template <int ABL, bool CONV, bool H2 = false>
+template <int ABL, bool CONV, bool H2 = false, bool X16 = false>
 __device__ __forceinline__ void wgrad_tr_body(const float *__restrict__ dY, const float *__restrict__ X, float *__restrict__ dW,
                                               float *__restrict__ dB, float *__restrict__ ws, int M, int N, int K, int ldy, int ldx,
                                               int ldw, int tiles_k, int tiles, int m_chunk, int H, int W, int bid, int64_t ws_tile0,
@@ -473,6 +473,9 @@
     inv_yx = iy * ix;
   }
   float4 ry[2][2], rx[2][2];
+  uint2 rx16[2][2];
+  static_assert(!X16 || (H2 && !CONV), "the bf16-X form is the plain two-plane weight gradient");
+  const unsigned short *X16p = reinterpret_cast<const unsigned short *>(X);
   int cpy[2] = {0, 0}, cpx[2] = {0, 0}, tdy = 0, tdx = 0, xoff = k0 + sc;
   if (CONV) {
     const int tap = k0 / ldx;
@@ -495,6 +498,8 @@
         rx[s][j] = ok ? *reinterpret_cast<const float4 *>(X + ((int64_t)r + tdy * W + tdx) * ldx + xoff) : make_float4(0, 0, 0, 0);
         cpx[j] += TWS;
         while (cpx[j] >= W) { cpx[j] -= W; if (++cpy[j] == H) cpy[j] = 0; }
+      } else if (X16) {
+        rx16[s][j] = (r < me && xcol_ok) ? *reinterpret_cast<const uint2 *>(X16p + (int64_t)r * ldx + k0 + sc) : make_uint2(0u, 0u);
       } else {
         rx[s][j] = (r < me && xcol_ok) ? *reinterpret_cast<const float4 *>(X + (int64_t)r * ldx + k0 + sc) : make_float4(0, 0, 0, 0);
       }
@@ -506,7 +511,11 @@
 #pragma unroll
     for (int j = 0; j < 2; ++j) {
       const int r = sr + 8 * j;
-      if constexpr (H2) {
+      if constexpr (X16) {
+        const pdh2::SplitH y = pdh2::split4h(ry[s][j], sy);
+        *reinterpret_cast<uint2 *>(&S[buf][0][0][r][sc]) = y.hi; *reinterpret_cast<uint2 *>(&S[buf][0][1][r][sc]) = y.lo;
+        *reinterpret_cast<uint2 *>(&S[buf][1][0][r][sc]) = pdh2::cvt4h_bf16(rx16[s][j], sx);
+      } else if constexpr (H2) {
         const pdh2::SplitH y = pdh2::split4h(ry[s][j], sy), x = pdh2::split4h(rx[s][j], sx);
         *reinterpret_cast<uint2 *>(&S[buf][0][0][r][sc]) = y.hi; *reinterpret_cast<uint2 *>(&S[buf][0][1][r][sc]) = y.lo;
         *reinterpret_cast<uint2 *>(&S[buf][1][0][r][sc]) = x.hi; *reinterpret_cast<uint2 *>(&S[buf][1][1][r][sc]) = x.lo;
@@ -544,7 +553,7 @@
 #pragma unroll
       for (int i = 0; i < 2; ++i) {
         a[p][i] = frag_tr(&S[par][0][p][frow][wn + i * 32 + fcol]);
-        b[p][i] = frag_tr(&S[par][1][p][frow][wk + i * 32 + fcol]);
+        if (!X16 || p == 0) b[p][i] = frag_tr(&S[par][1][p][frow][wk + i * 32 + fcol]);
       }
 #define TERM(PA, PB)                                                         \
   _Pragma("unroll") for (int i = 0; i < 2; ++i)                              \
@@ -552,7 +561,8 @@
         if constexpr (H2) pdh2::mmah(acc[i][j], __builtin_bit_cast(pdh2::h16x8, a[PA][i]), __builtin_bit_cast(pdh2::h16x8, b[PB][j])); \
         else mma16k(acc[i][j], a[PA][i], b[PB][j]);                          \
       }
-    if constexpr (H2) { TERM(1, 0) TERM(0, 1) TERM(0, 0) }
+    if constexpr (X16) { TERM(1, 0) TERM(0, 0) }
+    else if constexpr (H2) { TERM(1, 0) TERM(0, 1) TERM(0, 0) }
     else if (ABL != 2) { TERM(NP - 1, 0) TERM(0, NP - 1) TERM(1, 1) TERM(1, 0) TERM(0, 1) TERM(0, 0) }
     else { _Pragma("unroll") for (int p = 0; p < NP; ++p) _Pragma("unroll") for (int i = 0; i < 2; ++i) { acc[i][0][p] += (float)a[p][i][0]; acc[i][1][p] += (float)b[p][i][0]; } }
 #undef TERM
@@ -598,7 +608,7 @@
   }
 }
 
-template <int ABL, bool CONV, bool H2 = false>
+template <int ABL, bool CONV, bool H2 = false, bool X16 = false>
 __global__ __launch_bounds__(256, 2) void gemm_wgrad_f32x3_tr(const float *__restrict__ dY, const float *__restrict__ X,
                                                                float *__restrict__ dW, float *__restrict__ dB, float *__restrict__ ws,
                                                                int M, int N, int K, int ldy, int ldx, int ldw, int tiles_k, int tiles,
@@ -606,7 +616,7 @@
                                                                const float *__restrict__ x_amax)
 {
   const int lb = g_wgrad_xcd ? xcd_chunk((int)blockIdx.x, (int)gridDim.x) : (int)blockIdx.x;
-  wgrad_tr_body<ABL, CONV, H2>(dY, X, dW, dB, ws, M, N, K, ldy, ldx, ldw, tiles_k, tiles, m_chunk, H, W, lb, 0, y_amax, x_amax);
+  wgrad_tr_body<ABL, CONV, H2, X16>(dY, X, dW, dB, ws, M, N, K, ldy, ldx, ldw, tiles_k, tiles, m_chunk, H, W, lb, 0, y_amax, x_amax);
 }
 
 constexpr int WTD = 256, WTP = 288, WNT = 512;
@@ -619,7 +629,7 @@
   return u.v;
 }
 
-template <bool CONV>
+template <bool CONV, bool X16 = false>
 __device__ __forceinline__ void wgrad_h2w_body(const float *__restrict__ dY, const float *__restrict__ X, float *__restrict__ dW,
                                                float *__restrict__ dB, float *__restrict__ ws, int M, int N, int K, int ldy, int ldx,
                                                int ldw, int tiles_k, int tiles, int m_chunk, int H, int W, int bid, int64_t ws_tile0,
@@ -655,6 +665,9 @@
     inv_yx = iy * ix;
   }
   float4 ry[2][2], rx[2][2];
+  uint2 rx16[2][2];
+  static_assert(!X16 || !CONV, "the bf16-X form is the plain two-plane weight gradient");
+  const unsigned short *X16p = reinterpret_cast<const unsigned short *>(X);
   int cpy[2] = {0, 0}, cpx[2] = {0, 0}, tdy = 0, tdx = 0, xoff = k0 + sc;
   if (CONV) {
     const int tap = k0 / ldx;
@@ -677,6 +690,8 @@
         rx[s][j] = ok ? *reinterpret_cast<const float4 *>(X + ((int64_t)r + tdy * W + tdx) * ldx + xoff) : make_float4(0, 0, 0, 0);
         cpx[j] += TWS;
         while (cpx[j] >= W) { cpx[j] -= W; if (++cpy[j] == H) cpy[j] = 0; }
+      } else if (X16) {
+        rx16[s][j] = (r < me && xcol_ok) ? *reinterpret_cast<const uint2 *>(X16p + (int64_t)r * ldx + k0 + sc) : make_uint2(0u, 0u);
       } else {
         rx[s][j] = (r < me && xcol_ok) ? *reinterpret_cast<const float4 *>(X + (int64_t)r * ldx + k0 + sc) : make_float4(0, 0, 0, 0);
       }
@@ -688,9 +703,14 @@
 #pragma unroll
     for (int j = 0; j < 2; ++j) {
       const int r = sr + 8 * j;
-      const pdh2::SplitH y = pdh2::split4h(ry[s][j], sy), x = pdh2::split4h(rx[s][j], sx);
+      const pdh2::SplitH y = pdh2::split4h(ry[s][j], sy);
       *reinterpret_cast<uint2 *>(S(buf, 0, 0, r) + sc) = y.hi; *reinterpret_cast<uint2 *>(S(buf, 0, 1, r) + sc) = y.lo;
-      *reinterpret_cast<uint2 *>(S(buf, 1, 0, r) + sc) = x.hi; *reinterpret_cast<uint2 *>(S(buf, 1, 1, r) + sc) = x.lo;
+      if constexpr (X16) {
+        *reinterpret_cast<uint2 *>(S(buf, 1, 0, r) + sc) = pdh2::cvt4h_bf16(rx16[s][j], sx);
+      } else {
+        const pdh2::SplitH x = pdh2::split4h(rx[s][j], sx);
+        *reinterpret_cast<uint2 *>(S(buf, 1, 0, r) + sc) = x.hi; *reinterpret_cast<uint2 *>(S(buf, 1, 1, r) + sc) = x.lo;
+      }
       if (do_bias) { bsum.x += ry[s][j].x; bsum.y += ry[s][j].y; bsum.z += ry[s][j].z; bsum.w += ry[s][j].w; }
     }
   };
@@ -723,12 +743,14 @@
 #pragma unroll
       for (int p = 0; p < 2; ++p)
 #pragma unroll
-        for (int j = 0; j < 2; ++j) b[p][j] = frag_trw(S(par, 1, p, frow) + wk + (jp * 2 + j) * 32 + fcol);
+        for (int j = 0; j < 2; ++j) if (!X16 || p == 0) b[p][j] = frag_trw(S(par, 1, p, frow) + wk + (jp * 2 + j) * 32 + fcol);
 #define WTERM(PA, PB)                                                        \
   _Pragma("unroll") for (int i = 0; i < 2; ++i)                              \
       _Pragma("unroll") for (int j = 0; j < 2; ++j)                          \
         pdh2::mmah(acc[i][jp * 2 + j], __builtin_bit_cast(pdh2::h16x8, a[PA][i]), __builtin_bit_cast(pdh2::h16x8, b[PB][j]));
-      WTERM(1, 0) WTERM(0, 1) WTERM(0, 0)
+      WTERM(1, 0)
+      if constexpr (!X16) { WTERM(0, 1) }
+      WTERM(0, 0)
 #undef WTERM
     }
     if (st + 1 < steps) lstore(par ^ 1, par ^ 1);
@@ -737,6 +759,7 @@
   int st0 = 0;
   if (g_wgrad_fast && n0 + WTD <= N && k0 + WTD <= K && ((me - mb) % TWS) == 0 && steps >= 4 && (!CONV || W >= TWS)) {
     const float *py0 = dY + (int64_t)(mb + sr) * ldy + n0 + sc, *px0 = X + (int64_t)(mb + sr) * ldx + (CONV ? xoff : k0 + sc);
+    const unsigned short *px16 = X16p + (int64_t)(mb + sr) * ldx + k0 + sc;
     auto fstep = [&](int st, int par) {
       const int64_t m = (int64_t)(st + 2) * TWS;
 #pragma unroll
@@ -751,6 +774,8 @@
           const bool wrap = cpx[j] >= W;
           cpx[j] -= wrap ? W : 0;
           cpy[j] = wrap ? (cpy[j] + 1 == H ? 0 : cpy[j] + 1) : cpy[j];
+        } else if (X16) {
+          rx16[par][j] = *reinterpret_cast<const uint2 *>(px16 + (m + 8 * j) * ldx);
         } else {
           rx[par][j] = *reinterpret_cast<const float4 *>(px0 + (m + 8 * j) * ldx);
         }
@@ -761,25 +786,32 @@
 #pragma unroll
         for (int i = 0; i < 2; ++i) a[p][i] = frag_trw(S(par, 0, p, frow) + wn + i * 32 + fcol);
 #pragma unroll
-        for (int j = 0; j < 4; ++j) b[p][j] = frag_trw(S(par, 1, p, frow) + wk + j * 32 + fcol);
+        for (int j = 0; j < 4; ++j) if (!X16 || p == 0) b[p][j] = frag_trw(S(par, 1, p, frow) + wk + j * 32 + fcol);
       }
 #pragma unroll
       for (int j = 0; j < 2; ++j) {
         const int r = sr + 8 * j;
-        const pdh2::SplitH y = pdh2::split4h(ry[par ^ 1][j], sy), x = pdh2::split4h(rx[par ^ 1][j], sx);
+        const pdh2::SplitH y = pdh2::split4h(ry[par ^ 1][j], sy);
         *reinterpret_cast<uint2 *>(S(par ^ 1, 0, 0, r) + sc) = y.hi; *reinterpret_cast<uint2 *>(S(par ^ 1, 0, 1, r) + sc) = y.lo;
-        *reinterpret_cast<uint2 *>(S(par ^ 1, 1, 0, r) + sc) = x.hi; *reinterpret_cast<uint2 *>(S(par ^ 1, 1, 1, r) + sc) = x.lo;
+        if constexpr (X16) {
+          *reinterpret_cast<uint2 *>(S(par ^ 1, 1, 0, r) + sc) = pdh2::cvt4h_bf16(rx16[par ^ 1][j], sx);
+        } else {
+          const pdh2::SplitH x = pdh2::split4h(rx[par ^ 1][j], sx);
+          *reinterpret_cast<uint2 *>(S(par ^ 1, 1, 0, r) + sc) = x.hi; *reinterpret_cast<uint2 *>(S(par ^ 1, 1, 1, r) + sc) = x.lo;
+        }
         bsum.x += ry[par ^ 1][j].x; bsum.y += ry[par ^ 1][j].y; bsum.z += ry[par ^ 1][j].z; bsum.w += ry[par ^ 1][j].w;
       }
 #define WFTERM(PA, PB)                                                       \
   _Pragma("unroll") for (int i = 0; i < 2; ++i)                              \
       _Pragma("unroll") for (int j = 0; j < 4; ++j)                          \
         pdh2::mmah(acc[i][j], __builtin_bit_cast(pdh2::h16x8, a[PA][i]), __builtin_bit_cast(pdh2::h16x8, b[PB][j]));
-      WFTERM(1, 0) WFTERM(0, 1) WFTERM(0, 0)
+      WFTERM(1, 0)
+      if constexpr (!X16) { WFTERM(0, 1) }
+      WFTERM(0, 0)
 #undef WFTERM
-      __builtin_amdgcn_sched_group_barrier(0x100, 24, 0);
-#pragma unroll
-      for (int g = 0; g < 24; ++g) {
+      __builtin_amdgcn_sched_group_barrier(0x100, X16 ? 16 : 24, 0);
+#pragma unroll
+      for (int g = 0; g < (X16 ? 16 : 24); ++g) {
         __builtin_amdgcn_sched_group_barrier(0x008, 1, 0);
         __builtin_amdgcn_sched_group_barrier(0x002, 3, 0);
         if (g % 3 == 2) __builtin_amdgcn_sched_group_barrier(0x200, 1, 0);
@@ -831,14 +863,14 @@
   }
 }
 
-template <bool CONV>
+template <bool CONV, bool X16 = false>
 __global__ __launch_bounds__(512, 1) void gemm_wgrad_f16x2_wide(const float *__restrict__ dY, const float *__restrict__ X, float *__restrict__ dW,
                                                                 float *__restrict__ dB, float *__restrict__ ws, int M, int N, int K, int ldy, int ldx,
                                                                 int ldw, int tiles_k, int tiles, int m_chunk, int H, int W,
                                                                 const float *__restrict__ y_amax, const float *__restrict__ x_amax)
 {
-  wgrad_h2w_body<CONV>(dY, X, dW, dB, ws, M, N, K, ldy, ldx, ldw, tiles_k, tiles, m_chunk, H, W, xcd_chunk((int)blockIdx.x, (int)gridDim.x), 0,
-                       y_amax, x_amax);
+  wgrad_h2w_body<CONV, X16>(dY, X, dW, dB, ws, M, N, K, ldy, ldx, ldw, tiles_k, tiles, m_chunk, H, W, xcd_chunk((int)blockIdx.x, (int)gridDim.x), 0,
+                            y_amax, x_amax);
 }
 
 __device__ __forceinline__ void h2w_coord(int q, int t, int &row, int &col)
@@ -1132,8 +1164,9 @@
 
 static int wgrad_x3_launch(const float *dY, const float *X, float *dW, float *dB, float *ws, int64_t ws_floats, int M, int N, int K, int ldy,
                            int ldx, int ldw, hipStream_t st, const char *who, int convH = 0, int convW = 0, bool h2 = false,
-                           const float *y_amax = nullptr, const float *x_amax = nullptr)
-{
+                           const float *y_amax = nullptr, const float *x_amax = nullptr, bool x16 = false)
+{
+  if (x16 && (!h2 || convH)) return pd_set_error(PD_ERR_INVALID_ARG, "%s: the bf16-X form is the plain two-plane weight gradient", who);
   if (M < 0 || N < 0 || K < 0) return pd_set_error(PD_ERR_INVALID_ARG, "%s: negative size", who);
   if (N == 0 || K == 0 || M == 0) return PD_OK;
   if (!dW || !dY || !X) return pd_set_error(PD_ERR_INVALID_ARG, "%s: null pointer", who);
@@ -1164,9 +1197,10 @@
     if (!attr) {
       (void)hipFuncSetAttribute((const void *)gemm_wgrad_f16x2_wide<false>, hipFuncAttributeMaxDynamicSharedMemorySize, (int)lds);
       (void)hipFuncSetAttribute((const void *)gemm_wgrad_f16x2_wide<true>, hipFuncAttributeMaxDynamicSharedMemorySize, (int)lds);
+      (void)hipFuncSetAttribute((const void *)(gemm_wgrad_f16x2_wide<false, true>), hipFuncAttributeMaxDynamicSharedMemorySize, (int)lds);
       attr = true;
     }
-    auto kw = convH ? gemm_wgrad_f16x2_wide<true> : gemm_wgrad_f16x2_wide<false>;
+    auto kw = x16 ? gemm_wgrad_f16x2_wide<false, true> : convH ? gemm_wgrad_f16x2_wide<true> : gemm_wgrad_f16x2_wide<false>;
     hipLaunchKernelGGL(kw, dim3((unsigned)(wtiles * wsplits)), dim3(WNT), lds, st, dY, X, dW, dB, ws, M, N, K, ldy, ldx, ldw, wtk, wtiles, mc, convH, convW,
                        y_amax, x_amax);
     const int wgroups = wtiles * 128 >= 2048 ? 1 : wsplits >= 64 ? 8 : wsplits >= 16 ? 4 : 1;
@@ -1174,7 +1208,7 @@
     return pd_check_launch(who);
   }
   if (ws && (ws_floats < (int64_t)tiles * splits * BN * BM || splits < 2 || g_pd_dbg_x3 == 25)) ws = nullptr;
-  auto kfn = h2 ? (convH ? gemm_wgrad_f32x3_tr<0, true, true> : gemm_wgrad_f32x3_tr<0, false, true>)
+  auto kfn = x16 ? gemm_wgrad_f32x3_tr<0, false, true, true> : h2 ? (convH ? gemm_wgrad_f32x3_tr<0, true, true> : gemm_wgrad_f32x3_tr<0, false, true>)
                  : convH ? gemm_wgrad_f32x3_tr<0, true> : g_pd_dbg_x3 == 24 ? gemm_wgrad_f32x3_tr<2, false> : gemm_wgrad_f32x3_tr<0, false>;
   hipLaunchKernelGGL(kfn, dim3((unsigned)(tiles * splits)), dim3(256), 0, st, dY, X, dW, dB, ws, M, N, K, ldy, ldx, ldw, tk, tiles, m_chunk,
                      convH, convW, y_amax, x_amax);
@@ -1300,6 +1334,13 @@
                          true, y_amax, x_amax);
 }
 
+extern "C" int pd_gemm_wgrad_acc_f16x2_x16_ws(const float *dY, const void *X_bf16, float *dW, float *dB, const float *y_amax, const float *x_amax,
+                                              float *workspace, int64_t workspace_floats, int M, int N, int K, int ldy, int ldx, int ldw, void *stream_)
+{
+  return wgrad_x3_launch(dY, reinterpret_cast<const float *>(X_bf16), dW, dB, workspace, workspace_floats, M, N, K, ldy, ldx, ldw, (hipStream_t)stream_,
+                         "pd_gemm_wgrad_acc_f16x2_x16_ws", 0, 0, true, y_amax, x_amax, true);
+}
+
 extern "C" int pd_conv3x3_wgrad_nhwc_f16x2(const float *dY, const float *X, float *dWk, float *dB, const float *y_amax, const float *x_amax,
                                            float *workspace, int64_t workspace_floats, int B, int H, int W, int Ci, int Co, void *stream_)
 {
diff --git a/partdistillation_amd/functions/conv_x3.py b/partdistillation_amd/functions/conv_x3.py
--- a/partdistillation_amd/functions/conv_x3.py
+++ b/partdistillation_amd/functions/conv_x3.py
@@ -6,6 +6,7 @@
 
 H2 = __import__("os").environ.get("PD_H2_CONV", "1") != "0"
 H2_1X1 = __import__("os").environ.get("PD_H2_1X1", "1") != "0"
+A16 = __import__("os").environ.get("PD_H2_A16", "1") != "0"
 WGRAD_X3 = True
 
 
@@ -96,27 +97,36 @@
         ctx.has_bias = bias is not None
         ctx.x_bf16 = x.dtype == torch.bfloat16
         if H2 and H2_1X1 and x.is_contiguous(memory_format=torch.channels_last):
-            from .gemm import cast_rows_amax, gemm_tn_h2, row_amax
+            from .gemm import a16_supported, cast_rows_amax, gemm_tn_h2, gemm_tn_h2_a16, row_amax, row_amax_bf16, weight_operands
             B, ci, Hh, Ww = x.shape
             co = weight.shape[0]
-            if ctx.x_bf16:
-                x2, x_am = cast_rows_amax(x.permute(0, 2, 3, 1).reshape(-1, ci))
-                x = x2.view(B, Hh, Ww, ci).permute(0, 3, 1, 2)
+            w2 = weight.reshape(co, ci)
+            if A16 and w2.stride(1) == 1:
+                w_am, wt, wt_am = weight_operands(w2, transpose=ctx.needs_input_grad[0])
             else:
-                x_am = _pixel_amax(x)
-            w2 = weight.reshape(co, ci)
-            y = gemm_tn_h2(x.permute(0, 2, 3, 1).reshape(-1, ci), w2, bias, a_amax=x_am, b_amax=row_amax(w2))
-            ctx.save_for_backward(x, weight, x_am)
+                w_am, wt, wt_am = row_amax(w2), None, None
+            xr = x.permute(0, 2, 3, 1).reshape(-1, ci)
+            if ctx.x_bf16 and A16 and a16_supported(xr.shape[0], co, ci):
+                x_am = row_amax_bf16(xr)
+                y = gemm_tn_h2_a16(xr, w2, bias, a_amax=x_am, b_amax=w_am)
+            else:
+                if ctx.x_bf16:
+                    x2, x_am = cast_rows_amax(xr)
+                    x = x2.view(B, Hh, Ww, ci).permute(0, 3, 1, 2)
+                else:
+                    x_am = _pixel_amax(x)
+                y = gemm_tn_h2(x.permute(0, 2, 3, 1).reshape(-1, ci), w2, bias, a_amax=x_am, b_amax=w_am)
+            ctx.save_for_backward(x, weight, x_am, wt, wt_am)
             return y.view(B, Hh, Ww, co).permute(0, 3, 1, 2)
         if ctx.x_bf16:
             x = x.float()
-        ctx.save_for_backward(x, weight, None)
+        ctx.save_for_backward(x, weight, None, None, None)
         return torch.ops.aten.convolution(x, weight, bias, [1, 1], [0, 0], [1, 1], False, [0, 0], 1)
 
     @staticmethod
     def backward(ctx, dy):
         from .gemm import gemm_tn_h2, gemm_tn_h2_bf16out, gemm_wgrad_acc, row_amax
-        x, weight, x_am = ctx.saved_tensors
+        x, weight, x_am, wt, wt_am = ctx.saved_tensors
         dy = dy.contiguous(memory_format=torch.channels_last)
         co, ci = weight.shape[0], weight.shape[1]
         dx = dw = db = None
@@ -125,10 +135,12 @@
         dy_am = _pixel_amax(dy) if h2 else None
         if ctx.needs_input_grad[0]:
             if h2:
-                wt = weight.reshape(co, ci).t().contiguous()
+                if wt is None:
+                    wt = weight.reshape(co, ci).t().contiguous()
+                    wt_am = row_amax(wt)
                 B, _, Hh, Ww = x.shape
                 mm = gemm_tn_h2_bf16out if ctx.x_bf16 else gemm_tn_h2
-                dx = mm(rows(dy), wt, None, a_amax=dy_am, b_amax=row_amax(wt)).view(B, Hh, Ww, ci).permute(0, 3, 1, 2)
+                dx = mm(rows(dy), wt, None, a_amax=dy_am, b_amax=wt_am).view(B, Hh, Ww, ci).permute(0, 3, 1, 2)
             else:
                 dx = torch.ops.aten.convolution_backward(dy, x, weight, None, [1, 1], [0, 0], [1, 1], False, [0, 0], 1, [True, False, False])[0]
                 dx = dx.to(torch.bfloat16) if ctx.x_bf16 else dx
diff --git a/partdistillation_amd/functions/gemm.py b/partdistillation_amd/functions/gemm.py
--- a/partdistillation_amd/functions/gemm.py
+++ b/partdistillation_amd/functions/gemm.py
@@ -69,6 +69,51 @@
     am = torch.empty(x.shape[0], dtype=torch.float32, device=x.device)
     _lib.check(_lib.load().pd_cast_bf16_f32_amax(x.data_ptr(), x.shape[0], x.shape[1], y.data_ptr(), am.data_ptr(), _stream()))
     return y, am
+
+
+def row_amax_bf16(x):
+    assert x.is_cuda and x.dtype == torch.bfloat16 and x.dim() == 2 and x.stride(1) == 1 and x.shape[1] % 8 == 0 and x.stride(0) % 8 == 0
+    out = torch.empty(x.shape[0], dtype=torch.float32, device=x.device)
+    _lib.check(_lib.load().pd_row_amax_bf16(x.data_ptr(), x.shape[0], x.shape[1], x.stride(0), out.data_ptr(), _stream()))
+    return out
+
+
+def weight_operands(w, transpose=True):
+    assert w.is_cuda and w.dtype == torch.float32 and w.dim() == 2 and w.stride(1) == 1
+    co, ci = w.shape
+    buf = torch.empty(co + (ci * co + ci if transpose else 0), dtype=torch.float32, device=w.device)
+    w_am = buf[:co]
+    wt, wt_am = (buf[co:co + ci * co].view(ci, co), buf[co + ci * co:]) if transpose else (None, None)
+    _lib.check(_lib.load().pd_weight_operands_f32(w.data_ptr(), co, ci, w.stride(0), w_am.data_ptr(), wt.data_ptr() if transpose else None,
+                                                  wt_am.data_ptr() if transpose else None, _stream()))
+    return w_am, wt, wt_am
+
+
+def a16_supported(M, N, K):
+    return bool(_lib.load().pd_gemm_tn_f16x2_a16_supported(M, N, K))
+
+
+def gemm_tn_h2_a16(a, b, bias=None, a_amax=None, b_amax=None):
+    if not a.is_cuda:
+        raise RuntimeError("pd_gemm_tn_f16x2_a16 runs on the GPU only (no CPU fallback in partdistillation_amd)")
+    assert a.dtype == torch.bfloat16 and b.dtype == torch.float32 and a.stride(1) == 1 and b.stride(1) == 1 and b.shape[1] == a.shape[1]
+    M, K = a.shape
+    N = b.shape[0]
+    for v, n in ((a_amax, M), (b_amax, N)):
+        assert v is not None and v.dtype == torch.float32 and v.is_contiguous() and v.numel() == n
+    L = _lib.load()
+    c = torch.empty((M, N), dtype=torch.float32, device=a.device)
+    args = (a.data_ptr(), b.data_ptr(), bias.data_ptr() if bias is not None else None, c.data_ptr(), a_amax.data_ptr(), b_amax.data_ptr(), M, N, K,
+            a.stride(0), b.stride(0), N, _stream())
+    if not _TIMING["on"]:
+        _lib.check(L.pd_gemm_tn_f16x2_a16(*args))
+        return c
+    which = int(L.pd_gemm_tn_f16x2_a16_which(M, N, K))
+    label = ("gemm_rows_f16x2_k256<true, 0, true>" if which == 2 else "gemm_kpc_f16x2<true, 0, false, false, true>" if which == 5
+             else "gemm_tn_f16x2<128, 128, 64, 16, 0, false, 2, 1, true>")
+    with _timed_fwd(2.0 * M * N * K, label, 2.0 * M * K + 4.0 * (N * K + M * N)):
+        _lib.check(L.pd_gemm_tn_f16x2_a16(*args))
+    return c
 
 
 def gemm_tn_h2_bf16out(a, b, bias=None, a_amax=None, b_amax=None):
@@ -203,15 +248,16 @@
 def gemm_wgrad_acc(dy, x, dw, db=None, x3=None, h2=False, y_amax=None, x_amax=None):
     M, N = dy.shape
     K = x.shape[1]
+    x16 = h2 and x.dtype == torch.bfloat16
     assert dw.shape == (N, K) and dw.is_contiguous() and (db is None or db.numel() == N)
-    assert dy.dtype == torch.float32 and x.dtype == torch.float32 and dy.stride(1) == 1 and x.stride(1) == 1
+    assert dy.dtype == torch.float32 and (x.dtype == torch.float32 or x16) and dy.stride(1) == 1 and x.stride(1) == 1
     if _TIMING["on"]:
         a, b = torch.cuda.Event(enable_timing=True), torch.cuda.Event(enable_timing=True)
         a.record()
     L = _lib.load()
     if h2:
         ws = _wgrad_workspace(dy.device, int(L.pd_gemm_wgrad_f16x2_ws_floats(N, K)))
-        _lib.check(L.pd_gemm_wgrad_acc_f16x2_ws(dy.data_ptr(), x.data_ptr(), dw.data_ptr(), db.data_ptr() if db is not None else None,
+        _lib.check((L.pd_gemm_wgrad_acc_f16x2_x16_ws if x16 else L.pd_gemm_wgrad_acc_f16x2_ws)(dy.data_ptr(), x.data_ptr(), dw.data_ptr(), db.data_ptr() if db is not None else None,
                                                 y_amax.data_ptr() if y_amax is not None else None, x_amax.data_ptr() if x_amax is not None else None,
                                                 ws.data_ptr() if ws is not None else None, ws.numel() if ws is not None else 0,
                                                 M, N, K, dy.stride(0), x.stride(0), K, _stream()))
diff --git a/partdistillation_amd/lib.py b/partdistillation_amd/lib.py
--- a/partdistillation_amd/lib.py
+++ b/partdistillation_amd/lib.py
@@ -7,7 +7,7 @@
 CSRC = os.path.join(_HERE, "csrc")
 
 PD_F32, PD_F64, PD_BF16 = 0, 1, 2
-ABI_VERSION = 47
+ABI_VERSION = 48
 
 _c_int, _c_vp = ctypes.c_int, ctypes.c_void_p
 
@@ -39,6 +39,12 @@
     "pd_gemm_tn_f16x2_bf16out": (_c_int, [_c_vp] * 6 + [_c_int] * 6 + [_c_vp]),
     "pd_cast_bf16_f32_amax": (_c_int, [_c_vp, _c_int, _c_int, _c_vp, _c_vp, _c_vp]),
     "pd_row_amax_f32": (_c_int, [_c_vp, _c_int, _c_int, _c_int, _c_vp, _c_vp]),
+    "pd_row_amax_bf16": (_c_int, [_c_vp, _c_int, _c_int, _c_int, _c_vp, _c_vp]),
+    "pd_gemm_tn_f16x2_a16_supported": (_c_int, [_c_int] * 3),
+    "pd_gemm_tn_f16x2_a16_which": (_c_int, [_c_int] * 3),
+    "pd_gemm_tn_f16x2_a16": (_c_int, [_c_vp] * 6 + [_c_int] * 6 + [_c_vp]),
+    "pd_gemm_wgrad_acc_f16x2_x16_ws": (_c_int, [_c_vp] * 7 + [ctypes.c_int64] + [_c_int] * 6 + [_c_vp]),
+    "pd_weight_operands_f32": (_c_int, [_c_vp, _c_int, _c_int, _c_int, _c_vp, _c_vp, _c_vp, _c_vp]),
     "pd_gemm_tn_f32x3_relumask": (_c_int, [_c_vp] * 5 + [_c_int] * 6 + [_c_vp]),
     "pd_gemm_tn_f32x3_relu_bits": (_c_int, [_c_vp] * 5 + [_c_int] * 6 + [_c_vp]),
     "pd_gemm_tn_f32x3_relu_bits_words": (ctypes.c_int64, [_c_int] * 2),
```

Result: no change. 110.6, median of 6 (+0.5%).
